# rpng/open_vins

Measured on NVIDIA H100. Metric: msckf_updates_per_sec, higher is better.
Workload: dtype f64

## Files before the change

### open_vins_b200/csrc/chol_tiles.cuh

```cuda
#pragma once
#include "chol.cuh"
#ifdef CQ_PROBE
#include <cstdio>
#endif

#define CT_XP 12

__device__ __forceinline__ void ct_dmma(double &d0, double &d1, double a, double b) {
  asm volatile("mma.sync.aligned.m8n8k4.row.col.f64.f64.f64.f64 {%0,%1}, {%2}, {%3}, {%0,%1};" : "+d"(d0), "+d"(d1) : "d"(a), "d"(b));
}
__device__ __forceinline__ int ct_tri(int b) { return (b * (b + 1)) >> 1; }
__device__ __forceinline__ void ct_bar_group(int id, int nthreads) { asm volatile("bar.sync %0, %1;" ::"r"(id), "r"(nthreads) : "memory"); }
__device__ __forceinline__ size_t ct_idx(int i, int j) { return (size_t)(ct_tri(i >> 3) + (j >> 3)) * 64 + (i & 7) * 8 + (j & 7); }

struct CtView {
  double *T, *Xp0, *Xp1, *invd, *Linv0, *Linv1, *dummyT, *dummyX;
  int *flag;
};
__host__ __device__ inline size_t ct_view_doubles(int NRB) {
  return (size_t)((NRB * (NRB + 1)) / 2) * 64 + 2 * (size_t)NRB * 8 * CT_XP + (size_t)NRB * 8 + 128 + 64 + 2 * CT_XP;
}
__device__ __forceinline__ CtView ct_view_carve(double *base, int NRB, int *flag_word) {
  CtView v;
  v.T = base;
  v.Xp0 = v.T + (size_t)((NRB * (NRB + 1)) / 2) * 64;
  v.Xp1 = v.Xp0 + (size_t)NRB * 8 * CT_XP;
  v.invd = v.Xp1 + (size_t)NRB * 8 * CT_XP;
  v.Linv0 = v.invd + (size_t)NRB * 8;
  v.Linv1 = v.Linv0 + 64;
  v.dummyT = v.Linv1 + 64;
  v.dummyX = v.dummyT + 64;
  v.flag = flag_word;
  return v;
}

__device__ __forceinline__ void ct_diag8_frag(double &d0, double &d1, int nbk, double *invd, bool strict, double floor_d, int *flag) {
  const unsigned full = 0xffffffffu;
  const int lane = threadIdx.x & 31, g = lane >> 2, q = lane & 3;
  bool bad = false;
  double myinv = 0.0;
  const double inv_floor = (floor_d > 0.0) ? fast_rsqrt(floor_d) : 0.0;
  double pj = __shfl_sync(full, d0, 0);
#pragma unroll
  for (int j = 0; j < 8; j++) {
    const int jq = j >> 1;
    const double cur = (j & 1) ? d1 : d0;
    const double ag = __shfl_sync(full, cur, 4 * g + jq);
    const double ac0 = __shfl_sync(full, cur, 8 * q + jq);
    const double ac1 = __shfl_sync(full, cur, 8 * q + 4 + jq);
    double an = 0.0, dn = 0.0;
    if (j < 7) {
      an = __shfl_sync(full, cur, 4 * (j + 1) + jq);
      dn = __shfl_sync(full, ((j + 1) & 1) ? d1 : d0, 4 * (j + 1) + ((j + 1) >> 1));
    }
    const double y = fast_rsqrt(pj);
    const bool in = j < nbk;
    double d, iv;
    if (strict) {
      const bool pos = pj > 0.0;
      bad = bad || (in && !pos);
      d = pj;
      iv = (in && pos) ? y : 0.0;
    } else {
      const bool above = pj > floor_d;
      d = above ? pj : floor_d;
      iv = in ? (above ? y : inv_floor) : 0.0;
    }
    if (j < 7) {
      const double ln = an * iv;
      pj = fma(-ln, ln, dn);
    }
    if (lane == j)
      myinv = iv;
    if (q == jq) {
      if (j & 1)
        d1 = (g == j) ? d * iv : d1 * iv;
      else
        d0 = (g == j) ? d * iv : d0 * iv;
    }
    const double lg = ag * iv, lc0 = ac0 * iv, lc1 = ac1 * iv;
    if (2 * q > j)
      d0 = fma(-lg, lc0, d0);
    if (2 * q + 1 > j)
      d1 = fma(-lg, lc1, d1);
  }
  if (lane < 8)
    invd[lane] = myinv;
  if (bad && lane == 0)
    *flag = 1;
}

__device__ __forceinline__ void ct_linv8(const double *Lt, const double *invd, double *Linv) {
  const int lane = threadIdx.x & 31, cc = lane & 7;
  double mc[8];
#pragma unroll
  for (int j = 0; j < 8; j++) {
    double s0 = (j == cc) ? 1.0 : 0.0, s1 = 0.0;
#pragma unroll
    for (int t = 0; t < j; t++) {
      if (t & 1)
        s1 = fma(-Lt[j * 8 + t], mc[t], s1);
      else
        s0 = fma(-Lt[j * 8 + t], mc[t], s0);
    }
    mc[j] = (s0 + s1) * invd[j];
  }
  if (lane < 8) {
#pragma unroll
    for (int i = 0; i < 8; i++)
      Linv[i * 8 + cc] = (i >= cc) ? mc[i] : 0.0;
  }
}

__device__ __forceinline__ void ct_panel_tile(const CtView &sm, int i, int k, const double *Linv, double *Xb) {
  const int lane = threadIdx.x & 31, g = lane >> 2, q = lane & 3;
  double *t = sm.T + (size_t)(ct_tri(i) + k) * 64;
  const double a0 = t[g * 8 + q], a1 = t[g * 8 + q + 4];
  const double b0 = Linv[g * 8 + q], b1 = Linv[g * 8 + q + 4];
  double2 d = make_double2(0.0, 0.0);
  ct_dmma(d.x, d.y, a0, b0);
  ct_dmma(d.x, d.y, a1, b1);
  *reinterpret_cast<double2 *>(t + 2 * lane) = d;
  *reinterpret_cast<double2 *>(Xb + (size_t)(8 * i + g) * CT_XP + 2 * q) = d;
}

__device__ __forceinline__ void ct_panel_rows(double *T, double *Xp, const double *invd, int i0, int stride, int nrows, int k, int nbk) {
  if (i0 >= nrows)
    return;
  const double *Lk = T + (size_t)(ct_tri(k) + k) * 64;
  double L[8][8], iv[8];
#pragma unroll
  for (int c = 0; c < 8; c++) {
    iv[c] = (c < nbk) ? invd[8 * k + c] : 0.0;
#pragma unroll
    for (int t2 = 0; t2 < 4; t2++) {
      if (2 * t2 < c) {
        const double2 v = *reinterpret_cast<const double2 *>(Lk + c * 8 + 2 * t2);
        L[c][2 * t2] = v.x;
        L[c][2 * t2 + 1] = v.y;
      }
    }
  }
  for (int i = i0; i < nrows; i += stride) {
    double *src = T + (size_t)(ct_tri(i >> 3) + k) * 64 + (i & 7) * 8;
    double v[8], x[8];
    {
      const double2 v01 = *reinterpret_cast<const double2 *>(src), v23 = *reinterpret_cast<const double2 *>(src + 2);
      const double2 v45 = *reinterpret_cast<const double2 *>(src + 4), v67 = *reinterpret_cast<const double2 *>(src + 6);
      v[0] = v01.x, v[1] = v01.y, v[2] = v23.x, v[3] = v23.y, v[4] = v45.x, v[5] = v45.y, v[6] = v67.x, v[7] = v67.y;
    }
#pragma unroll
    for (int c = 0; c < 8; c++) {
      x[c] = (c < nbk) ? v[c] * iv[c] : 0.0;
#pragma unroll
      for (int t = c + 1; t < 8; t++)
        v[t] = fma(-x[c], L[t][c], v[t]);
    }
    if (nbk == 8) {
      *reinterpret_cast<double2 *>(src) = make_double2(x[0], x[1]);
      *reinterpret_cast<double2 *>(src + 2) = make_double2(x[2], x[3]);
      *reinterpret_cast<double2 *>(src + 4) = make_double2(x[4], x[5]);
      *reinterpret_cast<double2 *>(src + 6) = make_double2(x[6], x[7]);
    } else {
#pragma unroll
      for (int c = 0; c < 8; c++)
        if (c < nbk)
          src[c] = x[c];
    }
    double *xp = Xp + (size_t)i * CT_XP;
    *reinterpret_cast<double2 *>(xp) = make_double2(x[0], x[1]);
    *reinterpret_cast<double2 *>(xp + 2) = make_double2(x[2], x[3]);
    *reinterpret_cast<double2 *>(xp + 4) = make_double2(x[4], x[5]);
    *reinterpret_cast<double2 *>(xp + 6) = make_double2(x[6], x[7]);
  }
}

struct CtTileOps {
  double a0, a1, b0, b1;
  double2 c;
  double2 *cp;
};
__device__ __forceinline__ void ct_tile_load(CtTileOps &o, const CtView &sm, const double *Xp, int bi, int bj, int lane, bool valid) {
  const int g = lane >> 2, q = lane & 3;
  const double *xa = valid ? Xp + (size_t)(8 * bi + g) * CT_XP + q : sm.dummyX + q;
  const double *xb = valid ? Xp + (size_t)(8 * bj + g) * CT_XP + q : sm.dummyX + q;
  o.cp = reinterpret_cast<double2 *>((valid ? sm.T + (size_t)(ct_tri(bi) + bj) * 64 : sm.dummyT) + 2 * lane);
  o.a0 = -xa[0];
  o.a1 = -xa[4];
  o.b0 = xb[0];
  o.b1 = xb[4];
  o.c = *o.cp;
}
__device__ __forceinline__ void ct_tile_mma(CtTileOps &o) {
  ct_dmma(o.c.x, o.c.y, o.a0, o.b0);
  ct_dmma(o.c.x, o.c.y, o.a1, o.b1);
}
__device__ __forceinline__ void ct_tile_mma_store(CtTileOps &o) {
  ct_tile_mma(o);
  *o.cp = o.c;
}

#ifdef CQ_PROBE
#define CT_PROBE_T(v) v = clock64()
#else
#define CT_PROBE_T(v) do { } while (0)
#endif

__device__ __forceinline__ void ct_trail_row(const CtView &sm, const double *Xk, int bi, int j0, int jmax, int lane) {
  const int g = lane >> 2, q = lane & 3;
  const double *xa = Xk + (size_t)(8 * bi + g) * CT_XP + q;
  const double a0 = -xa[0], a1 = -xa[4];
  double *trow = sm.T + (size_t)ct_tri(bi) * 64 + 2 * lane;
  for (int bj = j0; bj <= jmax; bj += 2) {
    const bool two = bj + 1 <= jmax;
    const double *xb0 = Xk + (size_t)(8 * bj + g) * CT_XP + q;
    const double *xb1 = two ? xb0 + 8 * CT_XP : sm.dummyX + q;
    double2 *c0p = reinterpret_cast<double2 *>(trow + (size_t)bj * 64);
    double2 *c1p = two ? c0p + 32 : reinterpret_cast<double2 *>(sm.dummyT + 2 * lane);
    const double b00 = xb0[0], b01 = xb0[4], b10 = xb1[0], b11 = xb1[4];
    double2 c0 = *c0p, c1 = *c1p;
    ct_dmma(c0.x, c0.y, a0, b00);
    ct_dmma(c1.x, c1.y, a0, b10);
    ct_dmma(c0.x, c0.y, a1, b01);
    ct_dmma(c1.x, c1.y, a1, b11);
    *c0p = c0;
    *c1p = c1;
  }
}

template <int THREADS>
__device__ __forceinline__ void ct_chol_tiles(const CtView &sm, int n, int nrows, bool strict, double floor_d) {
  const int tid = threadIdx.x, lane = tid & 31, wid = tid >> 5;
  constexpr int NW = THREADS / 32, NH = NW - (NW + 3) / 4;
  static_assert(NH >= 1, "need at least one helper warp");
  const bool helper = (wid & 3) != 0;
  const int hr = wid - 1 - (wid >> 2);
  constexpr bool LINV = NW >= 8;
#ifdef CQ_PROBE
  long long p0 = 0, p1 = 0, p2 = 0, p3 = 0, p4 = 0, p5 = 0, acc[6] = {0, 0, 0, 0, 0, 0};
#endif
  const int NB = (n + 7) >> 3, NRB = (nrows + 7) >> 3;
  if (wid == 0) {
    double2 c = *reinterpret_cast<const double2 *>(sm.T + 2 * lane);
    ct_diag8_frag(c.x, c.y, min(8, n), sm.invd, strict, floor_d, sm.flag);
    *reinterpret_cast<double2 *>(sm.T + 2 * lane) = c;
    __syncwarp();
    if (LINV)
      asm volatile("bar.arrive 3, 64;" ::: "memory");
    ct_panel_rows(sm.T, sm.Xp0, sm.invd, lane < 8 ? 8 + lane : nrows, 1 << 30, nrows, 0, min(8, n));
  } else if (LINV && wid == 4) {
    asm volatile("bar.sync 3, 64;" ::: "memory");
    ct_linv8(sm.T, sm.invd, sm.Linv0);
  }
  __syncthreads();
  for (int k = 0; k < NB; k++) {
    const int par = k & 1;
    double *Xk = par ? sm.Xp1 : sm.Xp0, *Xn = par ? sm.Xp0 : sm.Xp1;
    const bool more = k + 1 < NB;
    CT_PROBE_T(p0);
#ifdef CQ_PROBE
    p1 = p2 = p3 = p4 = p0;
#endif
    if (wid == 0) {
      if (more) {
        const int k1 = k + 1, nbk1 = min(8, n - 8 * k1);
        CtTileOps o;
        ct_tile_load(o, sm, Xk, k1, k1, lane, true);
        ct_tile_mma(o);
        CT_PROBE_T(p1);
        ct_diag8_frag(o.c.x, o.c.y, nbk1, sm.invd + 8 * k1, strict, floor_d, sm.flag);
        *o.cp = o.c;
        __syncwarp();
        if (LINV)
          asm volatile("bar.arrive 3, 64;" ::: "memory");
        CT_PROBE_T(p2);
        asm volatile("bar.sync 2, %0;" ::"r"((NH + 1) * 32) : "memory");
        CT_PROBE_T(p3);
        ct_panel_rows(sm.T, Xn, sm.invd, lane < 8 ? 8 * (k + 2) + lane : nrows, 1 << 30, nrows, k1, nbk1);
        CT_PROBE_T(p4);
      }
    } else if (LINV && wid == 4) {
      if (more) {
        asm volatile("bar.sync 3, 64;" ::: "memory");
        ct_linv8(sm.T + (size_t)(ct_tri(k + 1) + k + 1) * 64, sm.invd + 8 * (k + 1), par ? sm.Linv0 : sm.Linv1);
      }
    } else if (helper) {
      if (LINV) {
        const double *Lk = par ? sm.Linv1 : sm.Linv0;
        for (int i = k + 2 + hr; i < NRB; i += NH)
          ct_panel_tile(sm, i, k, Lk, Xk);
      } else {
        ct_panel_rows(sm.T, Xk, sm.invd, 8 * (k + 2) + hr * 32 + lane, NH * 32, nrows, k, min(8, n - 8 * k));
      }
      if (NH > 1)
        ct_bar_group(1, NH * 32);
      else
        __syncwarp();
      CT_PROBE_T(p1);
      if (more) {
        for (int i = k + 2 + hr; i < NRB; i += 2 * NH) {
          CtTileOps o0, o1;
          ct_tile_load(o0, sm, Xk, i, k + 1, lane, true);
          ct_tile_load(o1, sm, Xk, i + NH, k + 1, lane, i + NH < NRB);
          ct_tile_mma_store(o0);
          ct_tile_mma_store(o1);
        }
        asm volatile("bar.arrive 2, %0;" ::"r"((NH + 1) * 32) : "memory");
        CT_PROBE_T(p2);
        const int R = NRB - (k + 2), jmaxc = NB - 1;
        for (int pr = hr; 2 * pr < R; pr += NH) {
          const int rb = R - 1 - pr;
          ct_trail_row(sm, Xk, k + 2 + rb, k + 2, min(k + 2 + rb, jmaxc), lane);
          if (rb != pr)
            ct_trail_row(sm, Xk, k + 2 + pr, k + 2, min(k + 2 + pr, jmaxc), lane);
        }
      }
      CT_PROBE_T(p3);
    }
    __syncthreads();
    CT_PROBE_T(p5);
#ifdef CQ_PROBE
    if (wid == 0) {
      acc[0] += p1 - p0, acc[1] += p2 - p1, acc[2] += p3 - p2, acc[3] += p4 - p3, acc[4] += p5 - p4;
    } else {
      acc[0] += p1 - p0, acc[1] += p2 - p1, acc[2] += p3 - p2, acc[3] += p5 - p3;
    }
    acc[5] += p5 - p0;
#endif
  }
#ifdef CQ_PROBE
  if (tid == 0)
    printf("chol n=%d W0 (cycles over %d steps): diag update %lld pivots %lld wait %lld rows below %lld step tail %lld | %lld\n", n, NB, acc[0], acc[1], acc[2], acc[3],
           acc[4], acc[5]);
  if (tid == 32 || tid == THREADS - 32)
    printf("chol n=%d helper warp %d: panel rows %lld column k+1 %lld trailing %lld wait %lld | %lld\n", n, wid, acc[0], acc[1], acc[2], acc[3], acc[5]);
#endif
}
```

### open_vins_b200/csrc/k_cholqr.cu

```cuda
#include "chol.cuh"
#include "chol_tiles.cuh"
#include "ovb_internal.cuh"
#include <math.h>
#include <cstdio>

#define CQ_MAXN 160
#define CQ_MAXB 20
#define CQ_MAXRB 22
#define CQ_GRAM_T 512
#define CQ_KB 32
#ifndef CQ_CHOL_T
#define CQ_CHOL_T 384
#endif
#define CQ_XP CT_XP
#define CQ_TRSM_T 640

namespace {

__device__ __forceinline__ void dmma(double &d0, double &d1, double a, double b) {
  asm volatile("mma.sync.aligned.m8n8k4.row.col.f64.f64.f64.f64 {%0,%1}, {%2}, {%3}, {%0,%1};" : "+d"(d0), "+d"(d1) : "d"(a), "d"(b));
}
__device__ __forceinline__ unsigned s_u32(const void *p) { return (unsigned)__cvta_generic_to_shared(p); }
__device__ __forceinline__ void cpa16(unsigned dst, const void *src, unsigned bytes) {
  asm volatile("cp.async.cg.shared.global [%0], [%1], 16, %2;" ::"r"(dst), "l"(src), "r"(bytes) : "memory");
}
__device__ __forceinline__ void cpa8(unsigned dst, const void *src, unsigned bytes) {
  asm volatile("cp.async.ca.shared.global [%0], [%1], 8, %2;" ::"r"(dst), "l"(src), "r"(bytes) : "memory");
}
__device__ __forceinline__ void cpa_commit() { asm volatile("cp.async.commit_group;" ::: "memory"); }
template <int N> __device__ __forceinline__ void cpa_wait() { asm volatile("cp.async.wait_group %0;" ::"n"(N) : "memory"); }
__device__ __forceinline__ void bar_group(int id, int nthreads) { asm volatile("bar.sync %0, %1;" ::"r"(id), "r"(nthreads) : "memory"); }
__device__ __forceinline__ int tri(int b) { return (b * (b + 1)) >> 1; }

__device__ __forceinline__ bool cq_tile_origin(int blk, int w, int BW, int nblk_side, int &ci, int &cj, int &offI, int &offJ, bool &diag) {
  int bI = 0, t = blk;
  while (t >= nblk_side - bI) {
    t -= nblk_side - bI;
    bI++;
  }
  const int bJ = bI + t;
  diag = (bI == bJ);
  int a, b;
  if (diag) {
    a = 0;
    int u = w;
    while (a < BW && u >= BW - a) {
      u -= BW - a;
      a++;
    }
    if (a >= BW)
      return false;
    b = a + u;
  } else {
    if (w >= BW * BW)
      return false;
    a = w / BW;
    b = w % BW;
  }
  offI = a * 32;
  offJ = (diag ? 0 : BW * 32) + b * 32;
  ci = (bI * BW + a) * 32;
  cj = (bJ * BW + b) * 32;
  return true;
}

template <int NT>
__device__ __forceinline__ void cq_issue_rows(double *buf, int pitch, const double *__restrict__ A, int ldA, int rc, int nrows, int r1, int nt, int cI0, int cJ0,
                                              int WI, int nrng) {
  const int units_per_row = nrng * WI / 2;
  for (int e = threadIdx.x; e < nrows * units_per_row; e += NT) {
    const int k = e / units_per_row, u = e - k * units_per_row;
    const int r = rc + k;
    const int dcol = 2 * u, col = (dcol < WI) ? cI0 + dcol : cJ0 + (dcol - WI);
    unsigned bytes = 0;
    if (r < r1)
      bytes = (col + 1 < nt) ? 16u : (col < nt ? 8u : 0u);
    const double *src = bytes ? (A + (size_t)r * ldA + col) : A;
    cpa16(s_u32(buf + (size_t)k * pitch + dcol), src, bytes);
  }
  cpa_commit();
}

__device__ __forceinline__ void cq_gram_kstep(double (&acc)[4][4][2], const double *row0, int pitch, int offI, int offJ, bool same, int g, int q) {
  const double *row = row0 + (size_t)q * pitch + g;
  double fa[4], fb[4];
#pragma unroll
  for (int b = 0; b < 4; b++)
    fa[b] = row[offI + 8 * b];
  if (same) {
#pragma unroll
    for (int b = 0; b < 4; b++)
      fb[b] = fa[b];
  } else {
#pragma unroll
    for (int b = 0; b < 4; b++)
      fb[b] = row[offJ + 8 * b];
  }
#pragma unroll
  for (int a = 0; a < 4; a++)
#pragma unroll
    for (int b = 0; b < 4; b++)
      dmma(acc[a][b][0], acc[a][b][1], fa[a], fb[b]);
}

}

__global__ void __launch_bounds__(CQ_GRAM_T) k_cq_gram(const double *__restrict__ A, int ldA, int m, int nt, int slab_rows, int BW, int nblk_side,
                                                      double *__restrict__ Gpart, int cs) {
  OVB_PDL_ENTER();
  extern __shared__ __align__(16) double gsm[];
  const int tid = threadIdx.x, lane = tid & 31, wid = tid >> 5, g = lane >> 2, q = lane & 3;
  int ci, cj, offI, offJ;
  bool diag;
  const bool active = cq_tile_origin(blockIdx.x, wid, BW, nblk_side, ci, cj, offI, offJ, diag);
  int bI = 0, tt = blockIdx.x;
  while (tt >= nblk_side - bI) {
    tt -= nblk_side - bI;
    bI++;
  }
  const int bJ = bI + tt;
  const int WI = BW * 32;
  const int nrng = (bI == bJ) ? 1 : 2;
  const int pitch = nrng * WI + 4;
  const int cI0 = bI * WI, cJ0 = bJ * WI;
  const int r0 = blockIdx.y * slab_rows, r1 = min(m, r0 + slab_rows);
  const int nchunks = (r1 > r0) ? (r1 - r0 + CQ_KB - 1) / CQ_KB : 0;
  double acc[4][4][2];
#pragma unroll
  for (int a = 0; a < 4; a++)
#pragma unroll
    for (int b = 0; b < 4; b++)
      acc[a][b][0] = acc[a][b][1] = 0.0;

  auto issue = [&](int c) { cq_issue_rows<CQ_GRAM_T>(gsm + (size_t)(c & 1) * CQ_KB * pitch, pitch, A, ldA, r0 + c * CQ_KB, CQ_KB, r1, nt, cI0, cJ0, WI, nrng); };
  if (nchunks > 0)
    issue(0);
  for (int c = 0; c < nchunks; c++) {
    if (c + 1 < nchunks) {
      issue(c + 1);
      cpa_wait<1>();
    } else {
      cpa_wait<0>();
    }
    __syncthreads();
    if (active) {
      const double *buf = gsm + (size_t)(c & 1) * CQ_KB * pitch;
#pragma unroll
      for (int ks = 0; ks < CQ_KB / 4; ks++)
        cq_gram_kstep(acc, buf + (size_t)4 * ks * pitch, pitch, offI, offJ, diag && offI == offJ, g, q);
    }
    __syncthreads();
  }
  if (cs <= 1) {
    if (active) {
      double *dst = Gpart + (((size_t)blockIdx.y * gridDim.x + blockIdx.x) * 16 + wid) * 1024;
#pragma unroll
      for (int a = 0; a < 4; a++)
#pragma unroll
        for (int b = 0; b < 4; b++)
          *reinterpret_cast<double2 *>(dst + (8 * a + g) * 32 + 8 * b + 2 * q) = make_double2(acc[a][b][0], acc[a][b][1]);
    }
    return;
  }
  double *stage = gsm;
  if (active) {
    double *dst = stage + (size_t)wid * 1024;
#pragma unroll
    for (int a = 0; a < 4; a++)
#pragma unroll
      for (int b = 0; b < 4; b++)
        *reinterpret_cast<double2 *>(dst + (8 * a + g) * 32 + 8 * b + 2 * q) = make_double2(acc[a][b][0], acc[a][b][1]);
  }
  asm volatile("barrier.cluster.arrive.release.aligned;" ::: "memory");
  asm volatile("barrier.cluster.wait.acquire.aligned;" ::: "memory");
  unsigned rank;
  asm volatile("mov.u32 %0, %%cluster_ctarank;" : "=r"(rank));
  if (active) {
    const int per = 1024 / cs;
    double *dst = Gpart + ((((size_t)blockIdx.y / cs) * gridDim.x + blockIdx.x) * 16 + wid) * 1024 + (size_t)rank * per;
    const unsigned base = s_u32(stage + (size_t)wid * 1024 + (size_t)rank * per);
    for (int e = lane; e < per; e += 32) {
      double sum = 0.0;
      for (int r = 0; r < cs; r++) {
        unsigned ra;
        double v;
        asm volatile("mapa.shared::cluster.u32 %0, %1, %2;" : "=r"(ra) : "r"(base + 8u * (unsigned)e), "r"((unsigned)r));
        asm volatile("ld.shared::cluster.f64 %0, [%1];" : "=d"(v) : "r"(ra) : "memory");
        sum += v;
      }
      dst[e] = sum;
    }
  }
  asm volatile("barrier.cluster.arrive.release.aligned;" ::: "memory");
  asm volatile("barrier.cluster.wait.acquire.aligned;" ::: "memory");
}

#define CQ_RED_T 1024
#define CQ_RED_CH 8
#define CQ_RED_GX (16 * CQ_RED_CH)
__global__ void __launch_bounds__(CQ_RED_T) k_cq_reduce(const double *__restrict__ Gpart, int nslab, int nblk, int BW, int nblk_side, int nt,
                                                       double *__restrict__ G, int ldG, int tiled) {
  OVB_PDL_ENTER();
  __shared__ double red[8][128];
  int ci, cj, offI, offJ;
  bool diag;
  const int w = blockIdx.x / CQ_RED_CH, ch = blockIdx.x % CQ_RED_CH, blk = blockIdx.y;
  if (!cq_tile_origin(blk, w, BW, nblk_side, ci, cj, offI, offJ, diag))
    return;
  if (ci >= nt || cj >= nt)
    return;
  const int el = threadIdx.x & 127, sg = threadIdx.x >> 7;
  const int e = ch * 128 + el;
  const double *src = Gpart + ((size_t)blk * 16 + w) * 1024 + e;
  const size_t stride = (size_t)nblk * 16 * 1024;
  double s0 = 0.0, s1 = 0.0;
  int sl = sg;
  for (; sl + 8 < nslab; sl += 16) {
    s0 += src[(size_t)sl * stride];
    s1 += src[(size_t)(sl + 8) * stride];
  }
  if (sl < nslab)
    s0 += src[(size_t)sl * stride];
  red[sg][el] = s0 + s1;
  __syncthreads();
  if (sg == 0) {
    const int i = ci + (e >> 5), j = cj + (e & 31);
    if (i < nt && j < nt && i <= j) {
      const double s = ((red[0][el] + red[1][el]) + (red[2][el] + red[3][el])) + ((red[4][el] + red[5][el]) + (red[6][el] + red[7][el]));
      if (tiled) {
        G[ct_idx(j, i)] = s;
        if ((i >> 3) == (j >> 3))
          G[(size_t)(tri(j >> 3) + (j >> 3)) * 64 + (i & 7) * 8 + (j & 7)] = s;
      } else {
        G[(size_t)i * ldG + j] = s;
        G[(size_t)j * ldG + i] = s;
      }
    }
  }
}

struct CqCholSmem {
  double T[(CQ_MAXRB * (CQ_MAXRB + 1) / 2) * 64];
  double Xp[2][CQ_MAXRB * 8 * CQ_XP];
  double invd[CQ_MAXRB * 8];
  double Linv[2][64];
  double red[32];
  double dummyT[64];
  double dummyX[2 * CQ_XP];
  int flag;
};

#define CQ_PK_INV ((CQ_MAXB * (CQ_MAXB + 1) / 2) * 64)
#define CQ_PK_DOUBLES (CQ_PK_INV + CQ_MAXB * 8)

namespace {

__device__ __forceinline__ void cq_chol_tiles(CqCholSmem &sm, int n, int nrows, bool strict, double floor_d) {
  CtView v;
  v.T = sm.T;
  v.Xp0 = sm.Xp[0];
  v.Xp1 = sm.Xp[1];
  v.invd = sm.invd;
  v.Linv0 = sm.Linv[0];
  v.Linv1 = sm.Linv[1];
  v.dummyT = sm.dummyT;
  v.dummyX = sm.dummyX;
  v.flag = &sm.flag;
  ct_chol_tiles<CQ_CHOL_T>(v, n, nrows, strict, floor_d);
}

__device__ void cq_load_tiles(CqCholSmem &sm, const double *__restrict__ G, size_t ldG, int n, int nrows, const double *__restrict__ rhs, int ld_rhs) {
  const int tid = threadIdx.x, lane = tid & 31, wid = tid >> 5;
  const int NB = (n + 7) >> 3, NRB = (nrows + 7) >> 3;
  for (int i = wid; i < 8 * NRB; i += CQ_CHOL_T / 32) {
    const double *row = (i >= n && rhs != nullptr) ? rhs + (size_t)(i - n) * ld_rhs : G + (size_t)i * ldG;
    const int jmax = min(i | 7, 8 * NB - 1);
    double *dst = sm.T + (size_t)tri(i >> 3) * 64 + (i & 7) * 8;
    for (int j = 2 * lane; j <= jmax; j += 64) {
      unsigned bytes = 0;
      if (i < nrows)
        bytes = (j + 1 < n) ? 16u : (j < n ? 8u : 0u);
      cpa16(s_u32(dst + (size_t)(j >> 3) * 64 + (j & 7)), bytes ? (const void *)(row + j) : (const void *)G, bytes);
    }
  }
  cpa_commit();
  for (int e = tid; e < 2 * CQ_MAXRB * 8 * CQ_XP; e += CQ_CHOL_T)
    (&sm.Xp[0][0])[e] = 0.0;
  if (tid < 64)
    sm.dummyT[tid] = 0.0;
  if (tid < 2 * CQ_XP)
    sm.dummyX[tid] = 0.0;
  if (tid == 0)
    sm.flag = 0;
  cpa_wait<0>();
}

__device__ __forceinline__ double cq_el(const double *T, int i, int j) { return T[(size_t)(tri(i >> 3) + (j >> 3)) * 64 + (i & 7) * 8 + (j & 7)]; }

}

__global__ void __launch_bounds__(CQ_CHOL_T) k_cq_chol_gram(const double *__restrict__ G, int ldG, int n, double shift_rel, double *__restrict__ Lpk, int tiled) {
  OVB_PDL_ENTER();
  extern __shared__ __align__(16) unsigned char cq_raw[];
  CqCholSmem &sm = *reinterpret_cast<CqCholSmem *>(cq_raw);
  const int tid = threadIdx.x, lane = tid & 31, wid = tid >> 5;
#ifdef CQ_PROBE
  const long long q0 = clock64();
#endif
  if (tiled) {
    __shared__ __align__(8) unsigned long long g_bar;
    const unsigned bar = s_u32(&g_bar);
    const int NB = (n + 7) >> 3;
    if (tid == 0) {
      asm volatile("mbarrier.init.shared::cta.b64 [%0], 1;" ::"r"(bar) : "memory");
      asm volatile("fence.mbarrier_init.release.cluster;" ::: "memory");
    }
    __syncthreads();
    if (tid == 0) {
      const unsigned bytes = (unsigned)(tri(NB) * 64 * sizeof(double));
      asm volatile("mbarrier.arrive.expect_tx.shared::cta.b64 _, [%0], %1;" ::"r"(bar), "r"(bytes) : "memory");
      asm volatile("cp.async.bulk.shared::cluster.global.mbarrier::complete_tx::bytes [%0], [%1], %2, [%3];" ::"r"(s_u32(sm.T)), "l"(G), "r"(bytes), "r"(bar)
                   : "memory");
    }
    for (int e = tid; e < 2 * CQ_MAXRB * 8 * CQ_XP; e += CQ_CHOL_T)
      (&sm.Xp[0][0])[e] = 0.0;
    if (tid < 64)
      sm.dummyT[tid] = 0.0;
    if (tid < 2 * CQ_XP)
      sm.dummyX[tid] = 0.0;
    if (tid == 0)
      sm.flag = 0;
    asm volatile("{\n\t.reg .pred p;\n\tCQ_GWAIT:\n\tmbarrier.try_wait.parity.shared::cta.b64 p, [%0], 0;\n\t@p bra CQ_GDONE;\n\tbra CQ_GWAIT;\n\tCQ_GDONE:\n\t}" ::"r"(bar)
                 : "memory");
    const int r0 = n - 8 * (NB - 1);
    if (r0 < 8) {
      double *last = sm.T + (size_t)tri(NB - 1) * 64;
      for (int e = tid; e < NB * 64; e += CQ_CHOL_T)
        if (((e >> 3) & 7) >= r0)
          last[e] = 0.0;
    }
  } else {
    cq_load_tiles(sm, G, (size_t)ldG, n, n, nullptr, 0);
  }
  __syncthreads();
  double mx = 0.0;
  for (int i = tid; i < n; i += CQ_CHOL_T) {
    const double d = sm.T[(size_t)(tri(i >> 3) + (i >> 3)) * 64 + (i & 7) * 9];
    mx = (d > mx) ? d : mx;
  }
#pragma unroll
  for (int o = 16; o > 0; o >>= 1) {
    const double y = __shfl_xor_sync(0xffffffffu, mx, o);
    mx = (y > mx) ? y : mx;
  }
  if (lane == 0)
    sm.red[wid] = mx;
  __syncthreads();
  mx = 0.0;
  for (int w = 0; w < CQ_CHOL_T / 32; w++)
    mx = (sm.red[w] > mx) ? sm.red[w] : mx;
  const double shift = shift_rel * mx;
  for (int i = tid; i < n; i += CQ_CHOL_T)
    sm.T[(size_t)(tri(i >> 3) + (i >> 3)) * 64 + (i & 7) * 9] += shift;
  __syncthreads();
#ifdef CQ_PROBE
  const long long q1 = clock64();
#endif
  cq_chol_tiles(sm, n, n, false, 0.25 * shift);
#ifdef CQ_PROBE
  const long long q2 = clock64();
#endif
  const int NB = (n + 7) >> 3;
  for (int e = 2 * tid; e < tri(NB) * 64; e += 2 * CQ_CHOL_T)
    *reinterpret_cast<double2 *>(Lpk + e) = *reinterpret_cast<const double2 *>(sm.T + e);
  for (int e = tid; e < CQ_MAXB * 8; e += CQ_CHOL_T)
    Lpk[CQ_PK_INV + e] = (e < n) ? sm.invd[e] : 1.0;
#ifdef CQ_PROBE
  if (tid == 0)
    printf("chol_gram n=%d: load %lld factor %lld store %lld cycles\n", n, q1 - q0, q2 - q1, clock64() - q2);
#endif
}

__global__ void __launch_bounds__(CQ_CHOL_T) k_cq_chol_ekf(double *__restrict__ S, int ldS, int r, const double *__restrict__ res, double *__restrict__ w,
                                                          double *__restrict__ invdiag, DevUpdateInfo *__restrict__ info, double *__restrict__ Lpk,
                                                          const double *__restrict__ floor_dev) {
  OVB_PDL_ENTER();
  extern __shared__ __align__(16) unsigned char cq_raw[];
  CqCholSmem &sm = *reinterpret_cast<CqCholSmem *>(cq_raw);
  const int tid = threadIdx.x, lane = tid & 31, wid = tid >> 5;
  const int nrows = r + (res != nullptr ? 1 : 0);
  cq_load_tiles(sm, S, (size_t)ldS, r, nrows, res, 0);
  __syncthreads();
  if (floor_dev != nullptr)
    cq_chol_tiles(sm, r, nrows, false, *floor_dev);
  else
    cq_chol_tiles(sm, r, nrows, true, 0.0);
  for (int i = wid; i < r; i += CQ_CHOL_T / 32)
    for (int j = lane; j <= i; j += 32)
      S[(size_t)i * ldS + j] = cq_el(sm.T, i, j);
  if (res != nullptr)
    for (int j = tid; j < r; j += CQ_CHOL_T)
      w[j] = cq_el(sm.T, r, j);
  if (invdiag != nullptr)
    for (int j = tid; j < r; j += CQ_CHOL_T)
      invdiag[j] = sm.invd[j];
  if (Lpk != nullptr) {
    const int NB = (r + 7) >> 3;
    for (int e = 2 * tid; e < tri(NB) * 64; e += 2 * CQ_CHOL_T)
      *reinterpret_cast<double2 *>(Lpk + e) = *reinterpret_cast<const double2 *>(sm.T + e);
    for (int e = tid; e < CQ_MAXB * 8; e += CQ_CHOL_T)
      Lpk[CQ_PK_INV + e] = (e < r) ? sm.invd[e] : 1.0;
  }
  if (tid == 0 && sm.flag && info != nullptr)
    info->not_spd = 1;
}

#define CQ_TRSM_NH 10
#define CQ_TRSM_SMEM (sizeof(double) * ((size_t)CQ_PK_DOUBLES + (size_t)(CQ_TRSM_T / 32) * CQ_TRSM_NH * 2 * 32))
template <int NH>
__device__ __forceinline__ void cq_trsm_half(double (&acc)[NH][2], int b0, const double *Lt, const double *Ri, double *xs, int lane) {
  const int g = lane >> 2, q = lane & 3;
#pragma unroll
  for (int jb = 0; jb < NH; jb++) {
    const int B = b0 + jb;
    const double *Ld = Lt + (size_t)(tri(B) + B) * 64;
    const double *ri = Ri + B * 8;
    double x[8];
#pragma unroll
    for (int qq = 0; qq < 4; qq++) {
      x[2 * qq] = __shfl_sync(0xffffffffu, acc[jb][0], (lane & ~3) | qq);
      x[2 * qq + 1] = __shfl_sync(0xffffffffu, acc[jb][1], (lane & ~3) | qq);
    }
#pragma unroll
    for (int c = 0; c < 8; c++) {
      x[c] *= ri[c];
#pragma unroll
      for (int c2 = c + 1; c2 < 8; c2++)
        x[c2] -= x[c] * Ld[c2 * 8 + c];
    }
    acc[jb][0] = (q == 0) ? x[0] : (q == 1) ? x[2] : (q == 2) ? x[4] : x[6];
    acc[jb][1] = (q == 0) ? x[1] : (q == 1) ? x[3] : (q == 2) ? x[5] : x[7];
    const double af0 = -((q == 0) ? x[0] : (q == 1) ? x[1] : (q == 2) ? x[2] : x[3]);
    const double af1 = -((q == 0) ? x[4] : (q == 1) ? x[5] : (q == 2) ? x[6] : x[7]);
    if (xs != nullptr) {
      xs[(2 * jb) * 32 + lane] = af0;
      xs[(2 * jb + 1) * 32 + lane] = af1;
    }
#pragma unroll
    for (int j = jb + 1; j < NH; j++) {
      const double *lf = Lt + (size_t)(tri(b0 + j) + B) * 64 + g * 8 + q;
      dmma(acc[j][0], acc[j][1], af0, lf[0]);
      dmma(acc[j][0], acc[j][1], af1, lf[4]);
    }
  }
}

template <int NH>
__device__ __forceinline__ void cq_trsm_load(double (&acc)[NH][2], const double *arow, bool row_ok, int b0, int nt, int q) {
#pragma unroll
  for (int jb = 0; jb < NH; jb++) {
    const int col = 8 * (b0 + jb) + 2 * q;
    acc[jb][0] = acc[jb][1] = 0.0;
    if (row_ok) {
      if (col + 1 < nt) {
        const double2 v = *reinterpret_cast<const double2 *>(arow + col);
        acc[jb][0] = v.x;
        acc[jb][1] = v.y;
      } else if (col < nt) {
        acc[jb][0] = arow[col];
      }
    }
  }
}
template <int NH>
__device__ __forceinline__ void cq_trsm_store(const double (&acc)[NH][2], double *arow, bool row_ok, int b0, int nt, int q) {
  if (!row_ok)
    return;
#pragma unroll
  for (int jb = 0; jb < NH; jb++) {
    const int col = 8 * (b0 + jb) + 2 * q;
    if (col + 1 < nt)
      *reinterpret_cast<double2 *>(arow + col) = make_double2(acc[jb][0], acc[jb][1]);
    else if (col < nt)
      arow[col] = acc[jb][0];
  }
}

template <int NBP, int NT>
__device__ __forceinline__ void cq_fetch_factor(double *Lt, double *Ri, const double *__restrict__ Lpk, int NB) {
  const int tid = threadIdx.x;
  __shared__ __align__(8) unsigned long long l_bar;
  const unsigned bar = s_u32(&l_bar);
  if (tid == 0) {
    asm volatile("mbarrier.init.shared::cta.b64 [%0], 1;" ::"r"(bar) : "memory");
    asm volatile("fence.mbarrier_init.release.cluster;" ::: "memory");
  }
  __syncthreads();
  if (tid == 0) {
    const unsigned bytesL = (unsigned)(tri(NB) * 64 * sizeof(double)), bytesR = (unsigned)(NB * 8 * sizeof(double));
    asm volatile("mbarrier.arrive.expect_tx.shared::cta.b64 _, [%0], %1;" ::"r"(bar), "r"(bytesL + bytesR) : "memory");
    asm volatile("cp.async.bulk.shared::cluster.global.mbarrier::complete_tx::bytes [%0], [%1], %2, [%3];" ::"r"(s_u32(Lt)), "l"(Lpk), "r"(bytesL), "r"(bar)
                 : "memory");
    asm volatile("cp.async.bulk.shared::cluster.global.mbarrier::complete_tx::bytes [%0], [%1], %2, [%3];" ::"r"(s_u32(Ri)), "l"(Lpk + CQ_PK_INV), "r"(bytesR),
                 "r"(bar)
                 : "memory");
  }
  for (int e = tri(NB) * 64 + tid; e < tri(NBP) * 64; e += NT)
    Lt[e] = 0.0;
  for (int e = NB * 8 + tid; e < NBP * 8; e += NT)
    Ri[e] = 1.0;
  asm volatile("{\n\t.reg .pred p;\n\tCQ_LWAIT:\n\tmbarrier.try_wait.parity.shared::cta.b64 p, [%0], 0;\n\t@p bra CQ_LDONE;\n\tbra CQ_LWAIT;\n\tCQ_LDONE:\n\t}" ::"r"(bar)
               : "memory");
  __syncthreads();
}

template <int NH1, int NH2>
__global__ void __launch_bounds__(CQ_TRSM_T) k_cq_trsm(double *__restrict__ A, int ldA, int m, int nt, const double *__restrict__ Lpk) {
  OVB_PDL_ENTER();
  extern __shared__ __align__(16) double tsm[];
  double *Lt = tsm;
  double *Ri = tsm + CQ_PK_INV;
  double *Xs = tsm + CQ_PK_DOUBLES;
  const int tid = threadIdx.x, lane = tid & 31, wid = tid >> 5, g = lane >> 2, q = lane & 3;
  cq_fetch_factor<NH1 + NH2, CQ_TRSM_T>(Lt, Ri, Lpk, (nt + 7) >> 3);
  double *xs = Xs + (size_t)wid * (CQ_TRSM_NH * 2 * 32);
  const int ngroups = (m + 7) >> 3;
  for (int rg = blockIdx.x + gridDim.x * wid; rg < ngroups; rg += gridDim.x * (CQ_TRSM_T / 32)) {
    const int row = 8 * rg + g;
    const bool row_ok = row < m;
    double *arow = A + (size_t)row * ldA;
#ifdef CQ_PROBE
    long long t0 = clock64(), t1, t2, t3 = 0, t4 = 0;
#endif
    {
      double acc[NH1][2];
      cq_trsm_load<NH1>(acc, arow, row_ok, 0, nt, q);
#ifdef CQ_PROBE
      t1 = clock64();
#endif
      cq_trsm_half<NH1>(acc, 0, Lt, Ri, NH2 > 0 ? xs : nullptr, lane);
#ifdef CQ_PROBE
      t2 = clock64();
#endif
      cq_trsm_store<NH1>(acc, arow, row_ok, 0, nt, q);
    }
    if constexpr (NH2 > 0) {
      double acc[NH2][2];
      cq_trsm_load<NH2>(acc, arow, row_ok, NH1, nt, q);
      __syncwarp();
#pragma unroll 2
      for (int jb = 0; jb < NH1; jb++) {
        const double af0 = xs[(2 * jb) * 32 + lane], af1 = xs[(2 * jb + 1) * 32 + lane];
#pragma unroll
        for (int j = 0; j < NH2; j++) {
          const double *lf = Lt + (size_t)(tri(NH1 + j) + jb) * 64 + g * 8 + q;
          dmma(acc[j][0], acc[j][1], af0, lf[0]);
          dmma(acc[j][0], acc[j][1], af1, lf[4]);
        }
      }
#ifdef CQ_PROBE
      t3 = clock64();
#endif
      cq_trsm_half<NH2>(acc, NH1, Lt, Ri, nullptr, lane);
#ifdef CQ_PROBE
      t4 = clock64();
#endif
      cq_trsm_store<NH2>(acc, arow, row_ok, NH1, nt, q);
      __syncwarp();
    }
#ifdef CQ_PROBE
    if (blockIdx.x == 0 && (tid == 0 || tid == 32 * 7) && rg < 40)
      printf("trsm rg=%d tid=%d: load %lld half1 %lld gemm+load %lld half2 %lld total %lld\n", rg, tid, t1 - t0, t2 - t1, t3 - t2, t4 - t3, clock64() - t0);
#endif
  }
}

static void cq_launch_trsm(ovb_ctx *ctx, int ctas, double *A, int ldA, int m, int nt, const double *Lpk) {
  const int NB = (nt + 7) / 8;
  const size_t smem = CQ_TRSM_SMEM;
  if (NB <= 5)
    ovb_launch(ctx, k_cq_trsm<5, 0>, dim3(ctas), dim3(CQ_TRSM_T), smem, A, ldA, m, nt, Lpk);
  else if (NB <= 10)
    ovb_launch(ctx, k_cq_trsm<10, 0>, dim3(ctas), dim3(CQ_TRSM_T), smem, A, ldA, m, nt, Lpk);
  else if (NB <= 15)
    ovb_launch(ctx, k_cq_trsm<10, 5>, dim3(ctas), dim3(CQ_TRSM_T), smem, A, ldA, m, nt, Lpk);
  else
    ovb_launch(ctx, k_cq_trsm<10, 10>, dim3(ctas), dim3(CQ_TRSM_T), smem, A, ldA, m, nt, Lpk);
}

#define CQ_SG_SMEM (226 * 1024)

__host__ __device__ __forceinline__ int cq_sg_pitch(int BW, int NBP) {
  const int w = (8 * NBP > 32 * BW) ? 8 * NBP : 32 * BW;
  return ((w + 15) & ~15) + 4;
}

template <int NH1, int NH2>
__device__ __forceinline__ void cq_solve_group(double *xrow, bool row_ok, const double *Lt, const double *Ri, int lane) {
  constexpr int NBP = NH1 + NH2;
  const int g = lane >> 2, q = lane & 3;
  {
    double acc[NH1][2];
    cq_trsm_load<NH1>(acc, xrow, row_ok, 0, 8 * NBP, q);
    cq_trsm_half<NH1>(acc, 0, Lt, Ri, nullptr, lane);
    cq_trsm_store<NH1>(acc, xrow, row_ok, 0, 8 * NBP, q);
  }
  if constexpr (NH2 > 0) {
    double acc[NH2][2];
    __syncwarp();
    cq_trsm_load<NH2>(acc, xrow, row_ok, NH1, 8 * NBP, q);
#pragma unroll 2
    for (int jb = 0; jb < NH1; jb++) {
      const double af0 = -xrow[8 * jb + q], af1 = -xrow[8 * jb + 4 + q];
#pragma unroll
      for (int j = 0; j < NH2; j++) {
        const double *lf = Lt + (size_t)(tri(NH1 + j) + jb) * 64 + g * 8 + q;
        dmma(acc[j][0], acc[j][1], af0, lf[0]);
        dmma(acc[j][0], acc[j][1], af1, lf[4]);
      }
    }
    cq_trsm_half<NH2>(acc, NH1, Lt, Ri, nullptr, lane);
    cq_trsm_store<NH2>(acc, xrow, row_ok, NH1, 8 * NBP, q);
  }
}

template <int NH1, int NH2>
__global__ void __launch_bounds__(CQ_GRAM_T) k_cq_solve_gram(const double *__restrict__ A, int ldA, int m, int nt, const double *__restrict__ Lpk, int slab_rows,
                                                            int cb, int ntail_max, int BW, double *__restrict__ Gpart, double *__restrict__ Qtail) {
  OVB_PDL_ENTER();
  extern __shared__ __align__(16) double ssm[];
  double *Lt = ssm;
  double *Ri = ssm + CQ_PK_INV;
  double *X = ssm + CQ_PK_DOUBLES;
  constexpr int NBP = NH1 + NH2;
  const int pitch = cq_sg_pitch(BW, NBP);
  const int r0 = blockIdx.x * slab_rows, r1 = min(m, r0 + slab_rows);
  double *tail = Qtail + (size_t)blockIdx.x * ntail_max * pitch;
  auto split_at = [&](int rc) { return r1 - rc > cb && r1 - rc <= 8 * (CQ_GRAM_T / 32); };
  auto nbuf_at = [&](int rc) { return split_at(rc) ? cb & ~7 : min(cb, (r1 - rc + 3) & ~3); };
  if (r0 < r1)
    cq_issue_rows<CQ_GRAM_T>(X, pitch, A, ldA, r0, nbuf_at(r0), r1, nt, 0, 0, pitch - 4, 1);
  cq_fetch_factor<NBP, CQ_GRAM_T>(Lt, Ri, Lpk, (nt + 7) >> 3);
  for (int rc = r0, nbuf = nbuf_at(r0), ntail = 0; rc < r1; rc += nbuf + ntail, nbuf = nbuf_at(rc)) {
    ntail = split_at(rc) ? (r1 - rc - nbuf + 3) & ~3 : 0;
    const int nact = nbuf + ntail;
    if (rc > r0)
      cq_issue_rows<CQ_GRAM_T>(X, pitch, A, ldA, rc, nbuf, r1, nt, 0, 0, pitch - 4, 1);
    for (int e = threadIdx.x; e < ntail * (pitch - 4); e += CQ_GRAM_T) {
      const int k = e / (pitch - 4), col = e - k * (pitch - 4), r = rc + nbuf + k;
      tail[(size_t)k * pitch + col] = (r < r1 && col < nt) ? A[(size_t)r * ldA + col] : 0.0;
    }
    cpa_wait<0>();
    __syncthreads();
    const int lane = threadIdx.x & 31, wid = threadIdx.x >> 5, g = lane >> 2, q = lane & 3, lr = 8 * wid + g;
    if (8 * wid < nbuf)
      cq_solve_group<NH1, NH2>(X + (size_t)min(lr, nbuf - 1) * pitch, lr < nbuf, Lt, Ri, lane);
    else if (8 * wid < nact)
      cq_solve_group<NH1, NH2>(tail + (size_t)min(lr - nbuf, ntail - 1) * pitch, lr < nact, Lt, Ri, lane);
    __syncthreads();
    int ci, cj, offI, offJ;
    bool diag;
    const bool active = cq_tile_origin(0, wid, BW, 1, ci, cj, offI, offJ, diag);
    double *part = Gpart + ((size_t)blockIdx.x * 16 + wid) * 1024 + g * 32 + 2 * q;
    if (active) {
      double acc[4][4][2];
#pragma unroll
      for (int a = 0; a < 4; a++)
#pragma unroll
        for (int b = 0; b < 4; b++) {
          const double2 v = rc > r0 ? *reinterpret_cast<const double2 *>(part + a * 256 + 8 * b) : make_double2(0.0, 0.0);
          acc[a][b][0] = v.x;
          acc[a][b][1] = v.y;
        }
#pragma unroll 1
      for (int k = 0; k < nact; k += 4)
        cq_gram_kstep(acc, k < nbuf ? X + (size_t)k * pitch : tail + (size_t)(k - nbuf) * pitch, pitch, offI, offJ, offI == offJ, g, q);
#pragma unroll
      for (int a = 0; a < 4; a++)
#pragma unroll
        for (int b = 0; b < 4; b++)
          *reinterpret_cast<double2 *>(part + a * 256 + 8 * b) = make_double2(acc[a][b][0], acc[a][b][1]);
    }
    __syncthreads();
  }
}

struct CqSgShape {
  int pitch, cb, ntail;
};
static CqSgShape cq_sg_shape(int nt, int BW, int slab_rows) {
  const int NB = (nt + 7) / 8, NBP = NB <= 5 ? 5 : NB <= 10 ? 10 : NB <= 15 ? 15 : 20;
  CqSgShape s;
  s.pitch = cq_sg_pitch(BW, NBP);
  const int round = slab_rows < 8 * (CQ_GRAM_T / 32) ? slab_rows : 8 * (CQ_GRAM_T / 32);
  const int fit = (int)((CQ_SG_SMEM - sizeof(double) * CQ_PK_DOUBLES) / (sizeof(double) * s.pitch)) & ~3;
  s.cb = fit < round ? fit : round;
  s.ntail = slab_rows > s.cb ? round - (s.cb & ~7) : 0;
  return s;
}
static size_t cq_solve_gram_scratch(int nslab, int nt, int BW, int slab_rows) {
  const CqSgShape s = cq_sg_shape(nt, BW, slab_rows);
  return (size_t)nslab * s.ntail * s.pitch;
}

template <int NH1, int NH2>
static void cq_launch_solve_gram_t(ovb_ctx *ctx, int nslab, const double *A, int ldA, int m, int nt, const double *Lpk, int slab_rows, int BW, double *Gpart,
                                   double *Qtail) {
  const CqSgShape s = cq_sg_shape(nt, BW, slab_rows);
  const size_t smem = sizeof(double) * (CQ_PK_DOUBLES + (size_t)s.cb * s.pitch);
  ovb_launch(ctx, k_cq_solve_gram<NH1, NH2>, dim3(nslab), dim3(CQ_GRAM_T), smem, A, ldA, m, nt, Lpk, slab_rows, s.cb, s.ntail, BW, Gpart, Qtail);
}
static void cq_launch_solve_gram(ovb_ctx *ctx, int nslab, const double *A, int ldA, int m, int nt, const double *Lpk, int slab_rows, int BW, double *Gpart,
                                 double *Qtail) {
  const int NB = (nt + 7) / 8;
  if (NB <= 5)
    cq_launch_solve_gram_t<5, 0>(ctx, nslab, A, ldA, m, nt, Lpk, slab_rows, BW, Gpart, Qtail);
  else if (NB <= 10)
    cq_launch_solve_gram_t<10, 0>(ctx, nslab, A, ldA, m, nt, Lpk, slab_rows, BW, Gpart, Qtail);
  else if (NB <= 15)
    cq_launch_solve_gram_t<10, 5>(ctx, nslab, A, ldA, m, nt, Lpk, slab_rows, BW, Gpart, Qtail);
  else
    cq_launch_solve_gram_t<10, 10>(ctx, nslab, A, ldA, m, nt, Lpk, slab_rows, BW, Gpart, Qtail);
}

__global__ void __launch_bounds__(256) k_cq_trmm(const double *__restrict__ L2, const double *__restrict__ L1, int nt, double *__restrict__ Rout, int ldR) {
  OVB_PDL_ENTER();
  __shared__ double As[16][CQ_MAXN + 1];
  __shared__ double Bs[CQ_MAXN][17];
  const int ti = blockIdx.y, tj = blockIdx.x;
  const int tid = threadIdx.x, tx = tid & 15, ty = tid >> 4;
  const int n = nt - 1;
  const int i = ti * 16 + ty, j = tj * 16 + tx;
  double acc = 0.0;
  if (tj >= ti) {
    const int k0 = ti * 16, k1 = min(nt, tj * 16 + 16);
    const int K = k1 - k0;
    for (int e = tid; e < 16 * K; e += 256) {
      const int a = e / K, k = e - a * K;
      const int ii = ti * 16 + a, kk = k0 + k;
      As[a][k] = (ii < nt && kk >= ii) ? L2[(size_t)(tri(kk >> 3) + (ii >> 3)) * 64 + (kk & 7) * 8 + (ii & 7)] : 0.0;
    }
    for (int e = tid; e < 16 * K; e += 256) {
      const int k = e >> 4, b = e & 15;
      const int kk = k0 + k, jj = tj * 16 + b;
      Bs[k][b] = (jj < nt && jj >= kk) ? L1[(size_t)(tri(jj >> 3) + (kk >> 3)) * 64 + (jj & 7) * 8 + (kk & 7)] : 0.0;
    }
    __syncthreads();
    double a0 = 0.0, a1 = 0.0, a2 = 0.0, a3 = 0.0;
    int k = 0;
    for (; k + 3 < K; k += 4) {
      a0 += As[ty][k] * Bs[k][tx];
      a1 += As[ty][k + 1] * Bs[k + 1][tx];
      a2 += As[ty][k + 2] * Bs[k + 2][tx];
      a3 += As[ty][k + 3] * Bs[k + 3][tx];
    }
    for (; k < K; k++)
      a0 += As[ty][k] * Bs[k][tx];
    acc = (a0 + a1) + (a2 + a3);
  }
  if (i < n && j < nt)
    Rout[(size_t)i * ldR + j] = (j >= i) ? acc : 0.0;
}

#define CQ_GN_T 256
__global__ void __launch_bounds__(CQ_GN_T) k_cq_gemm_nt(double *__restrict__ C, int ldc, const double *__restrict__ A, int lda, const double *__restrict__ B,
                                                       int ldb, int M, int N, int K, int lower_only) {
  OVB_PDL_ENTER();
  __shared__ __align__(16) double As[64][36];
  __shared__ __align__(16) double Bs[64][36];
  const int m0 = blockIdx.y * 64, n0 = blockIdx.x * 64;
  if (lower_only && n0 > m0 + 63)
    return;
  const int tid = threadIdx.x, lane = tid & 31, wid = tid >> 5, g = lane >> 2, q = lane & 3;
  const int wm = (wid >> 2) * 32, wn = (wid & 3) * 16;
  double acc[4][2][2];
#pragma unroll
  for (int a = 0; a < 4; a++)
#pragma unroll
    for (int b = 0; b < 2; b++)
      acc[a][b][0] = acc[a][b][1] = 0.0;
  for (int k0 = 0; k0 < K; k0 += 32) {
    for (int e = tid; e < 64 * 16; e += CQ_GN_T) {
      const int r = e >> 4, u = e & 15, k = k0 + 2 * u;
      unsigned ba = 0, bb = 0;
      if (m0 + r < M)
        ba = (k + 1 < K) ? 16u : (k < K ? 8u : 0u);
      if (n0 + r < N)
        bb = (k + 1 < K) ? 16u : (k < K ? 8u : 0u);
      cpa16(s_u32(&As[r][2 * u]), ba ? (const void *)(A + (size_t)(m0 + r) * lda + k) : (const void *)A, ba);
      cpa16(s_u32(&Bs[r][2 * u]), bb ? (const void *)(B + (size_t)(n0 + r) * ldb + k) : (const void *)B, bb);
    }
    cpa_commit();
    cpa_wait<0>();
    __syncthreads();
#pragma unroll
    for (int ks = 0; ks < 8; ks++) {
      double fa[4], fb[2];
#pragma unroll
      for (int a = 0; a < 4; a++)
        fa[a] = As[wm + 8 * a + g][4 * ks + q];
#pragma unroll
      for (int b = 0; b < 2; b++)
        fb[b] = Bs[wn + 8 * b + g][4 * ks + q];
#pragma unroll
      for (int a = 0; a < 4; a++)
#pragma unroll
        for (int b = 0; b < 2; b++)
          dmma(acc[a][b][0], acc[a][b][1], fa[a], fb[b]);
    }
    __syncthreads();
  }
#pragma unroll
  for (int a = 0; a < 4; a++)
#pragma unroll
    for (int b = 0; b < 2; b++) {
      const int i = m0 + wm + 8 * a + g, j = n0 + wn + 8 * b + 2 * q;
      if (i < M) {
        double *c = C + (size_t)i * ldc + j;
        if (j + 1 < N) {
          double2 v = *reinterpret_cast<double2 *>(c);
          v.x -= acc[a][b][0];
          v.y -= acc[a][b][1];
          *reinterpret_cast<double2 *>(c) = v;
        } else if (j < N) {
          c[0] -= acc[a][b][0];
        }
      }
    }
}

__global__ void __launch_bounds__(256) k_cq_shift(double *__restrict__ G, int ldG, int n, double shift_rel, double *__restrict__ floor_out) {
  OVB_PDL_ENTER();
  __shared__ double red[8];
  double mx = 0.0;
  for (int i = threadIdx.x; i < n; i += 256) {
    const double d = G[(size_t)i * ldG + i];
    mx = (d > mx) ? d : mx;
  }
#pragma unroll
  for (int o = 16; o > 0; o >>= 1) {
    const double y = __shfl_xor_sync(0xffffffffu, mx, o);
    mx = (y > mx) ? y : mx;
  }
  if ((threadIdx.x & 31) == 0)
    red[threadIdx.x >> 5] = mx;
  __syncthreads();
  mx = 0.0;
  for (int w = 0; w < 8; w++)
    mx = (red[w] > mx) ? red[w] : mx;
  const double shift = shift_rel * mx;
  for (int i = threadIdx.x; i < n; i += 256)
    G[(size_t)i * ldG + i] += shift;
  if (threadIdx.x == 0)
    *floor_out = 0.25 * shift;
}

__global__ void __launch_bounds__(256) k_cq_trmm_wide(const double *__restrict__ L2, const double *__restrict__ L1, int ldL, int nt, double *__restrict__ Rout,
                                                     int ldR) {
  OVB_PDL_ENTER();
  __shared__ double As[32][33];
  __shared__ double Bs[32][33];
  const int ti = blockIdx.y, tj = blockIdx.x;
  const int tid = threadIdx.x, tx = tid & 31, ty = tid >> 5;
  const int n = nt - 1;
  double acc[4] = {0, 0, 0, 0};
  if (tj >= ti) {
    for (int tk = ti; tk <= tj; tk++) {
      for (int e = tid; e < 1024; e += 256) {
        const int a = e >> 5, b = e & 31;
        const int k = tk * 32 + a, i = ti * 32 + b;
        As[a][b] = (k < nt && i < nt && k >= i) ? L2[(size_t)k * ldL + i] : 0.0;
        const int j = tj * 32 + a, k2 = tk * 32 + b;
        Bs[a][b] = (j < nt && k2 < nt && j >= k2) ? L1[(size_t)j * ldL + k2] : 0.0;
      }
      __syncthreads();
#pragma unroll 8
      for (int kk = 0; kk < 32; kk++) {
        const double b = Bs[tx][kk];
#pragma unroll
        for (int u = 0; u < 4; u++)
          acc[u] += As[kk][ty + 8 * u] * b;
      }
      __syncthreads();
    }
  }
#pragma unroll
  for (int u = 0; u < 4; u++) {
    const int i = ti * 32 + ty + 8 * u, j = tj * 32 + tx;
    if (i < n && j < nt)
      Rout[(size_t)i * ldR + j] = (j >= i) ? acc[u] : 0.0;
  }
}

#define CQ_GRAM_CS 4
static void cq_launch_gram(ovb_ctx *ctx, int nblk, int nslab_padded, size_t smem, const double *A, int ldA, int m, int nt, int slab_rows, int BW, int nblk_side,
                           double *Gpart, int cs) {
  cudaLaunchConfig_t cfg = {};
  cfg.gridDim = dim3(nblk, nslab_padded);
  cfg.blockDim = dim3(CQ_GRAM_T);
  cfg.dynamicSmemBytes = smem;
  cfg.stream = ctx->stream;
  cudaLaunchAttribute at[2];
  int na = 0;
  if (ctx->tsqr_pdl && !ctx->prof_on) {
    at[na].id = cudaLaunchAttributeProgrammaticStreamSerialization;
    at[na].val.programmaticStreamSerializationAllowed = 1;
    na++;
  }
  if (cs > 1) {
    at[na].id = cudaLaunchAttributeClusterDimension;
    at[na].val.clusterDim.x = 1;
    at[na].val.clusterDim.y = cs;
    at[na].val.clusterDim.z = 1;
    na++;
  }
  cfg.attrs = at;
  cfg.numAttrs = na;
  const bool prof = ctx->prof_on && ctx->prof_n < 96 && ctx->prof_ev[0] != nullptr;
  if (prof)
    cudaEventRecord(ctx->prof_ev[2 * ctx->prof_n], ctx->stream);
  cudaLaunchKernelEx(&cfg, k_cq_gram, A, ldA, m, nt, slab_rows, BW, nblk_side, Gpart, cs);
  if (prof) {
    cudaEventRecord(ctx->prof_ev[2 * ctx->prof_n + 1], ctx->stream);
    ctx->prof_fn[ctx->prof_n++] = (const void *)k_cq_gram;
  }
}

static bool cq_attrs(ovb_ctx *ctx) {
  if (!ctx->attr_done[4]) {
    cudaFuncSetAttribute(k_cq_gram, cudaFuncAttributeMaxDynamicSharedMemorySize, 160 * 1024);
    cudaFuncSetAttribute(k_cq_chol_gram, cudaFuncAttributeMaxDynamicSharedMemorySize, (int)sizeof(CqCholSmem));
    cudaFuncSetAttribute(k_cq_chol_ekf, cudaFuncAttributeMaxDynamicSharedMemorySize, (int)sizeof(CqCholSmem));
    cudaFuncSetAttribute(k_cq_trsm<5, 0>, cudaFuncAttributeMaxDynamicSharedMemorySize, (int)CQ_TRSM_SMEM);
    cudaFuncSetAttribute(k_cq_trsm<10, 0>, cudaFuncAttributeMaxDynamicSharedMemorySize, (int)CQ_TRSM_SMEM);
    cudaFuncSetAttribute(k_cq_trsm<10, 5>, cudaFuncAttributeMaxDynamicSharedMemorySize, (int)CQ_TRSM_SMEM);
    cudaFuncSetAttribute(k_cq_trsm<10, 10>, cudaFuncAttributeMaxDynamicSharedMemorySize, (int)CQ_TRSM_SMEM);
    cudaFuncSetAttribute(k_cq_solve_gram<5, 0>, cudaFuncAttributeMaxDynamicSharedMemorySize, CQ_SG_SMEM);
    cudaFuncSetAttribute(k_cq_solve_gram<10, 0>, cudaFuncAttributeMaxDynamicSharedMemorySize, CQ_SG_SMEM);
    cudaFuncSetAttribute(k_cq_solve_gram<10, 5>, cudaFuncAttributeMaxDynamicSharedMemorySize, CQ_SG_SMEM);
    cudaFuncSetAttribute(k_cq_solve_gram<10, 10>, cudaFuncAttributeMaxDynamicSharedMemorySize, CQ_SG_SMEM);
    ctx->attr_done[4] = 1;
  }
  return true;
}

int ovb_cholqr_max_cols(void) { return CQ_MAXN; }

static bool cq_ensure_G(ovb_ctx *ctx) {
  const int ldW = CQ_MAXN + 8;
  const size_t need_G = (size_t)4 * ldW * ldW;
  if (need_G > ctx->G_cap) {
    if (ctx->d_G)
      cudaFree(ctx->d_G);
    ctx->d_G = nullptr;
    if (cudaMalloc(&ctx->d_G, sizeof(double) * need_G) != cudaSuccess)
      return false;
    cudaMemsetAsync(ctx->d_G, 0, sizeof(double) * need_G, ctx->stream);
    ctx->G_cap = need_G;
  }
  return true;
}

bool launch_chol_ekf_dmma(ovb_ctx *ctx, double *S, int ldS, int r, const double *res, double *w, double *invdiag, double **Lpk_out) {
  if (Lpk_out)
    *Lpk_out = nullptr;
  if (r + 1 > CQ_MAXRB * 8 || r > CQ_MAXN || (ldS & 1))
    return false;
  cq_attrs(ctx);
  double *Lpk = nullptr;
  if (cq_ensure_G(ctx)) {
    const int ldW = CQ_MAXN + 8;
    Lpk = ctx->d_G + (size_t)3 * ldW * ldW;
  }
  ovb_launch(ctx, k_cq_chol_ekf, dim3(1), dim3(CQ_CHOL_T), sizeof(CqCholSmem), S, ldS, r, res, w, invdiag, ctx->d_info, Lpk, (const double *)nullptr);
  if (Lpk_out)
    *Lpk_out = Lpk;
  return true;
}

bool launch_trsm_rows(ovb_ctx *ctx, double *A, int ldA, int m, int nt, const double *Lpk) {
  if (nt > CQ_MAXN || (ldA & 1) || m < 1 || Lpk == nullptr)
    return false;
  cq_attrs(ctx);
  const int ngroups = (m + 7) / 8;
  int ctas = ngroups;
  if (ctas > ctx->sm_count)
    ctas = ctx->sm_count;
  cq_launch_trsm(ctx, ctas, A, ldA, m, nt, Lpk);
  return true;
}

#define CQ_WB 128
#define CQ_WMAX 520
#define CQ_WBLOCKS ((CQ_WMAX + CQ_WB - 1) / CQ_WB)
static bool cq_ensure_wide(ovb_ctx *ctx) {
  const size_t need = (size_t)2 * CQ_WMAX * CQ_WMAX + (size_t)2 * CQ_WBLOCKS * CQ_PK_DOUBLES + 64;
  if (need > ctx->cqw_cap) {
    if (ctx->d_cqw)
      cudaFree(ctx->d_cqw);
    ctx->d_cqw = nullptr;
    if (cudaMalloc(&ctx->d_cqw, sizeof(double) * need) != cudaSuccess)
      return false;
    ctx->cqw_cap = need;
  }
  return true;
}
static void cq_gemm_nt(ovb_ctx *ctx, double *C, int ldc, const double *A, int lda, const double *B, int ldb, int M, int N, int K, int lower_only) {
  if (M <= 0 || N <= 0 || K <= 0)
    return;
  ovb_launch(ctx, k_cq_gemm_nt, dim3((N + 63) / 64, (M + 63) / 64), dim3(CQ_GN_T), (size_t)0, C, ldc, A, lda, B, ldb, M, N, K, lower_only);
}
static void cq_trsm_any(ovb_ctx *ctx, double *A, int ldA, int m, int nt, const double *Lpk) {
  const int ngroups = (m + 7) / 8;
  int ctas = (ngroups + CQ_TRSM_T / 32 - 1) / (CQ_TRSM_T / 32);
  if (ngroups <= ctx->sm_count)
    ctas = ngroups;
  if (ctas > ctx->sm_count)
    ctas = ctx->sm_count;
  cq_launch_trsm(ctx, ctas, A, ldA, m, nt, Lpk);
}
static void cq_chol_blocked(ovb_ctx *ctx, double *S, int ld, int n, int extra, double *Lpk, const double *floor_dev, DevUpdateInfo *info) {
  for (int J = 0, b = 0; J < n; J += CQ_WB, b++) {
    const int nb = (n - J < CQ_WB) ? n - J : CQ_WB;
    double *Lb = Lpk + (size_t)b * CQ_PK_DOUBLES;
    ovb_launch(ctx, k_cq_chol_ekf, dim3(1), dim3(CQ_CHOL_T), sizeof(CqCholSmem), S + (size_t)J * ld + J, ld, nb, (const double *)nullptr, (double *)nullptr,
               (double *)nullptr, info, Lb, floor_dev);
    const int mrem = n + extra - (J + nb);
    if (mrem > 0) {
      double *panel = S + (size_t)(J + nb) * ld + J;
      cq_trsm_any(ctx, panel, ld, mrem, nb, Lb);
      const int ncols = n - (J + nb);
      cq_gemm_nt(ctx, S + (size_t)(J + nb) * ld + (J + nb), ld, panel, ld, panel, ld, mrem, ncols, nb, 1);
    }
  }
}
static void cq_trsm_blocked(ovb_ctx *ctx, double *X, int ldx, int m, int n, const double *S, int ld, const double *Lpk) {
  for (int J = 0, b = 0; J < n; J += CQ_WB, b++) {
    const int nb = (n - J < CQ_WB) ? n - J : CQ_WB;
    if (J > 0)
      cq_gemm_nt(ctx, X + J, ldx, X, ldx, S + (size_t)J * ld, ld, m, nb, J, 0);
    cq_trsm_any(ctx, X + J, ldx, m, nb, Lpk + (size_t)b * CQ_PK_DOUBLES);
  }
}

__global__ void k_cq_copy_row(const double *__restrict__ src, double *__restrict__ dst, int n) {
  OVB_PDL_ENTER();
  const int i = blockIdx.x * blockDim.x + threadIdx.x;
  if (i < n)
    dst[i] = src[i];
}
__global__ void k_cq_inv_diag(const double *__restrict__ S, int ld, int n, double *__restrict__ inv) {
  OVB_PDL_ENTER();
  const int i = blockIdx.x * blockDim.x + threadIdx.x;
  if (i < n) {
    const double d = S[(size_t)i * ld + i];
    inv[i] = d != 0.0 ? 1.0 / d : 0.0;
  }
}

bool launch_chol_solve_wide(ovb_ctx *ctx, double *S, int ldS, int r, double *w, double *invdiag, double *M, int ldM, int N, bool gate_only) {
  if (r > CQ_WMAX - 8 || (ldS & 1) || (ldM & 1) || r + 1 > ctx->cfg.max_state + 1)
    return false;
  cq_attrs(ctx);
  if (!cq_ensure_wide(ctx))
    return false;
  double *Lpk = ctx->d_cqw + (size_t)2 * CQ_WMAX * CQ_WMAX;
  ovb_launch(ctx, k_cq_copy_row, dim3((r + 127) / 128), dim3(128), (size_t)0, (const double *)w, S + (size_t)r * ldS, r);
  cq_chol_blocked(ctx, S, ldS, r, 1, Lpk, nullptr, ctx->d_info);
  ovb_launch(ctx, k_cq_copy_row, dim3((r + 127) / 128), dim3(128), (size_t)0, (const double *)(S + (size_t)r * ldS), w, r);
  ovb_launch(ctx, k_cq_inv_diag, dim3((r + 127) / 128), dim3(128), (size_t)0, (const double *)S, ldS, r, invdiag);
  if (!gate_only)
    cq_trsm_blocked(ctx, M, ldM, N, r, S, ldS, Lpk);
  return true;
}

static int cq_compress_wide(ovb_ctx *ctx, double *A, int m, int n, int ldA, double *Rout, int ldR) {
  const int nt = n + 1;
  if (nt > CQ_WMAX - 7 || !cq_ensure_wide(ctx))
    return -1;
  const int nT = (nt + 31) / 32, BW = 4, nblk_side = (nT + BW - 1) / BW, nblk = nblk_side * (nblk_side + 1) / 2;
  int nslab = ctx->sm_count / nblk;
  if (nslab < 1)
    nslab = 1;
  const int max_slabs = (m + CQ_KB - 1) / CQ_KB;
  if (nslab > max_slabs)
    nslab = max_slabs;
  int slab_rows = (((m + nslab - 1) / nslab) + 3) & ~3;
  nslab = (m + slab_rows - 1) / slab_rows;
  const size_t need_part = (size_t)nslab * nblk * 16 * 1024;
  if (need_part > ctx->Gpart_cap) {
    if (ctx->d_Gpart)
      cudaFree(ctx->d_Gpart);
    ctx->d_Gpart = nullptr;
    if (cudaMalloc(&ctx->d_Gpart, sizeof(double) * need_part) != cudaSuccess)
      return -1;
    ctx->Gpart_cap = need_part;
  }
  double *G1 = ctx->d_cqw, *G2 = G1 + (size_t)CQ_WMAX * CQ_WMAX, *Lpk1 = G2 + (size_t)CQ_WMAX * CQ_WMAX, *Lpk2 = Lpk1 + (size_t)CQ_WBLOCKS * CQ_PK_DOUBLES;
  double *floor_dev = Lpk2 + (size_t)CQ_WBLOCKS * CQ_PK_DOUBLES;
  const size_t gram_smem = sizeof(double) * 2 * CQ_KB * (size_t)(2 * BW * 32 + 4);
  int launches = 0;
  for (int pass = 0; pass < 2; pass++) {
    double *G = pass == 0 ? G1 : G2;
    cq_launch_gram(ctx, nblk, nslab, gram_smem, (const double *)A, ldA, m, nt, slab_rows, BW, nblk_side, ctx->d_Gpart, 1);
    ovb_launch(ctx, k_cq_reduce, dim3(CQ_RED_GX, nblk), dim3(CQ_RED_T), (size_t)0, (const double *)ctx->d_Gpart, nslab, nblk, BW, nblk_side, nt, G, (int)CQ_WMAX, 0);
    ovb_launch(ctx, k_cq_shift, dim3(1), dim3(256), (size_t)0, G, (int)CQ_WMAX, nt, pass == 0 ? 1e-11 : 1e-13, floor_dev + pass);
    cq_chol_blocked(ctx, G, CQ_WMAX, nt, 0, pass == 0 ? Lpk1 : Lpk2, floor_dev + pass, (DevUpdateInfo *)nullptr);
    if (pass == 0)
      cq_trsm_blocked(ctx, A, ldA, m, nt, G1, CQ_WMAX, Lpk1);
    launches += 3 + 3 * ((nt + CQ_WB - 1) / CQ_WB);
  }
  const int nT32 = (nt + 31) / 32;
  ovb_launch(ctx, k_cq_trmm_wide, dim3(nT32, nT32), dim3(256), (size_t)0, (const double *)G2, (const double *)G1, (int)CQ_WMAX, nt, Rout, ldR);
  ctx->n_launch += launches + 1;
  return launches + 1;
}

int launch_compress_cholqr2(ovb_ctx *ctx, double *A, int m, int n, int ldA, double *Rout, int ldR) {
  const int nt = n + 1;
  if ((ldA & 1) || m < 1)
    return -1;
  cq_attrs(ctx);
  if (nt > CQ_MAXN)
    return cq_compress_wide(ctx, A, m, n, ldA, Rout, ldR);
  const int nT = (nt + 31) / 32;
  const int BW = nT, nblk_side = 1, nblk = 1;
  int nslab = ctx->sm_count;
  const int max_slabs = (m + CQ_KB - 1) / CQ_KB;
  if (nslab > max_slabs)
    nslab = max_slabs;
  int slab_rows = (m + nslab - 1) / nslab;
  slab_rows = (slab_rows + 3) & ~3;
  nslab = (m + slab_rows - 1) / slab_rows;
  const int cs = (ctx->gram_cluster && nslab >= 2 * CQ_GRAM_CS) ? CQ_GRAM_CS : 1;
  const int nslab_pad = (nslab + cs - 1) / cs * cs, npart = nslab_pad / cs;
  const size_t part_doubles = (size_t)nslab_pad * nblk * 16 * 1024;
  const size_t need_part = part_doubles + cq_solve_gram_scratch(nslab, nt, BW, slab_rows);
  const int ldW = CQ_MAXN + 8;
  if (!cq_ensure_G(ctx))
    return -1;
  if (need_part > ctx->Gpart_cap) {
    const size_t cap = need_part + need_part / 2;
    if (ctx->d_Gpart)
      cudaFree(ctx->d_Gpart);
    ctx->d_Gpart = nullptr;
    ctx->Gpart_cap = 0;
    if (cudaMalloc(&ctx->d_Gpart, sizeof(double) * cap) != cudaSuccess)
      return -1;
    ctx->Gpart_cap = cap;
  }
  double *G = ctx->d_G, *L1 = G + (size_t)ldW * ldW, *L2 = L1 + (size_t)ldW * ldW;
  static_assert(CQ_PK_DOUBLES <= (CQ_MAXN + 8) * (CQ_MAXN + 8), "packed factor must fit its slot");
  size_t gram_smem = sizeof(double) * 2 * CQ_KB * (size_t)(BW * 32 + 4);
  if (cs > 1 && gram_smem < sizeof(double) * 16 * 1024)
    gram_smem = sizeof(double) * 16 * 1024;
  cq_launch_gram(ctx, nblk, nslab_pad, gram_smem, (const double *)A, ldA, m, nt, slab_rows, BW, nblk_side, ctx->d_Gpart, cs);
  ovb_launch(ctx, k_cq_reduce, dim3(CQ_RED_GX, nblk), dim3(CQ_RED_T), (size_t)0, (const double *)ctx->d_Gpart, npart, nblk, BW, nblk_side, nt, G, ldW, 1);
  ovb_launch(ctx, k_cq_chol_gram, dim3(1), dim3(CQ_CHOL_T), sizeof(CqCholSmem), (const double *)G, ldW, nt, 1e-11, L1, 1);
  cq_launch_solve_gram(ctx, nslab, (const double *)A, ldA, m, nt, (const double *)L1, slab_rows, BW, ctx->d_Gpart, ctx->d_Gpart + part_doubles);
  ovb_launch(ctx, k_cq_reduce, dim3(CQ_RED_GX, nblk), dim3(CQ_RED_T), (size_t)0, (const double *)ctx->d_Gpart, nslab, nblk, BW, nblk_side, nt, G, ldW, 1);
  ovb_launch(ctx, k_cq_chol_gram, dim3(1), dim3(CQ_CHOL_T), sizeof(CqCholSmem), (const double *)G, ldW, nt, 1e-13, L2, 1);
  const int nT16 = (nt + 15) / 16;
  ovb_launch(ctx, k_cq_trmm, dim3(nT16, nT16), dim3(256), (size_t)0, (const double *)L2, (const double *)L1, nt, Rout, ldR);
  ctx->n_launch += 7;
  return 7;
}
```

### open_vins_b200/csrc/k_ekf.cu

```cuda
#include "chol.cuh"
#include "ovb_internal.cuh"

#define EK_T 32

__global__ void __launch_bounds__(256) k_ekf_gemm(int mode, const double *__restrict__ P, int ldP, const double *__restrict__ H, int ldH,
                                                  const double *__restrict__ Min, int ldM, const DevUpdateInfo *__restrict__ info, int X, int Y,
                                                  int K, double *__restrict__ Cout, int ldC, double sigma2, const double *__restrict__ Rdiag) {
  OVB_PDL_ENTER();
  __shared__ double As[EK_T][EK_T + 1];
  __shared__ double Bs[EK_T][EK_T + 1];
  const int x0 = blockIdx.x * EK_T, y0 = blockIdx.y * EK_T;
  if (mode == 1 && y0 > x0 + EK_T - 1)
    return;
  const int tid = threadIdx.x, tx = tid & 31, ty = tid >> 5;
  double acc[4] = {0, 0, 0, 0};
  const int *cs = info->col_state;
  for (int j0 = 0; j0 < K; j0 += EK_T) {
    for (int e = tid; e < EK_T * EK_T; e += 256) {
      int jj = e >> 5, q = e & 31;
      int j = j0 + jj;
      double av = 0.0, bv = 0.0;
      if (j < K) {
        if (mode == 0) {
          int a = x0 + q;
// ... 79 lines not shown
                                                           int L_in_smem, const DevUpdateInfo *__restrict__ info) {
  OVB_PDL_ENTER();
  extern __shared__ __align__(16) double tsm[];
  const int lane = threadIdx.x & 31, wid = threadIdx.x >> 5;
  if (info->not_spd)
    return;
  const int ldl = r | 1;
  double *inv_s = tsm + (size_t)TR_ROWS * r;
  double *Ls = inv_s + r;
  for (int e = threadIdx.x; e < r; e += 32 * TR_ROWS)
    inv_s[e] = invdiag[e];
  if (L_in_smem)
    stage_lower_async<32 * TR_ROWS>(Ls, ldl, L, (size_t)ldL, r, r);
  else
    __syncthreads();
  const double *Lp = L_in_smem ? Ls : L;
  const int lp = L_in_smem ? ldl : ldL;
  const int a = blockIdx.x * TR_ROWS + wid;
  if (a >= N)
    return;
  double *y = tsm + (size_t)wid * r;
  for (int t = lane; t < r; t += 32)
    y[t] = M[(size_t)a * ldM + t];
  __syncwarp();
  for (int kb = 0; kb < r; kb += 8) {
    const int nbk = min(8, r - kb);
    double s[8];
#pragma unroll
    for (int c = 0; c < 8; c++)
      s[c] = 0.0;
    for (int t = lane; t < kb; t += 32) {
      const double yt = y[t];
#pragma unroll
      for (int c = 0; c < 8; c++)
        if (c < nbk)
          s[c] += Lp[(size_t)(kb + c) * lp + t] * yt;
    }
#pragma unroll
    for (int o = 16; o > 0; o >>= 1) {
#pragma unroll
      for (int c = 0; c < 8; c++)
        s[c] += __shfl_xor_sync(0xffffffffu, s[c], o);
    }
    double yn[8];
#pragma unroll
    for (int c = 0; c < 8; c++) {
      if (c < nbk) {
        const double *Lr = Lp + (size_t)(kb + c) * lp + kb;
        double v = y[kb + c] - s[c];
#pragma unroll
        for (int t = 0; t < 8; t++)
          if (t + 1 < c)
            v -= Lr[t] * yn[t];
        if (c > 0)
          v -= Lr[c - 1] * yn[c - 1];
        yn[c] = v * inv_s[kb + c];
      }
    }
    __syncwarp();
    if (lane < nbk) {
      double v = yn[0];
#pragma unroll
      for (int c = 1; c < 8; c++)
        v = (lane == c) ? yn[c] : v;
      y[kb + lane] = v;
    }
    __syncwarp();
  }
  for (int t = lane; t < r; t += 32)
    Yout[(size_t)a * ldY + t] = y[t];
}

__global__ void __launch_bounds__(256) k_ekf_downdate(double *__restrict__ P, int ldP, const double *__restrict__ Yin, int ldY, int N, int r,
                                                      const double *__restrict__ w, double *__restrict__ dx, DevUpdateInfo *__restrict__ info) {
  OVB_PDL_ENTER();
  __shared__ double As[EK_T][EK_T + 1];
  __shared__ double Bs[EK_T][EK_T + 1];
  const int a0 = blockIdx.x * EK_T, b0 = blockIdx.y * EK_T;
  if (b0 < a0)
    return;
  const int tid = threadIdx.x, tx = tid & 31, ty = tid >> 5;
  if (info->not_spd) {
    if (a0 == b0 && tid < EK_T && a0 + tid < N)
      dx[a0 + tid] = 0.0;
    return;
  }
  double acc[4] = {0, 0, 0, 0};
  double dxa = 0.0;
  for (int k0 = 0; k0 < r; k0 += EK_T) {
    for (int e = tid; e < EK_T * EK_T; e += 256) {
      int q = e >> 5, kk = e & 31;
      int k = k0 + kk;
      As[kk][q] = (k < r && a0 + q < N) ? Yin[(size_t)(a0 + q) * ldY + k] : 0.0;
      Bs[kk][q] = (k < r && b0 + q < N) ? Yin[(size_t)(b0 + q) * ldY + k] : 0.0;
    }
    __syncthreads();
#pragma unroll 8
    for (int kk = 0; kk < EK_T; kk++) {
      double b = Bs[kk][tx];
#pragma unroll
      for (int u = 0; u < 4; u++)
        acc[u] += As[kk][ty + 8 * u] * b;
    }
    if (a0 == b0 && tid < EK_T) {
      for (int kk = 0; kk < EK_T; kk++)
        if (k0 + kk < r)
          dxa += As[kk][tid] * w[k0 + kk];
    }
    __syncthreads();
  }
#pragma unroll
  for (int u = 0; u < 4; u++) {
    int a = a0 + ty + 8 * u, b = b0 + tx;
    if (a < N && b < N && b >= a) {
      double v = P[(size_t)a * ldP + b] - acc[u];
      P[(size_t)a * ldP + b] = v;
      P[(size_t)b * ldP + a] = v;
      if (a == b && v < 0.0)
        atomicMin(&info->neg_diag_index, a);
      if (!isfinite(v))
        info->nonfinite = 1;
    }
  }
  if (a0 == b0 && tid < EK_T && a0 + tid < N)
    dx[a0 + tid] = dxa;
}

#define EK1_KMAX 160
__device__ __forceinline__ void ek_cpa8(double *dst_smem, const double *src) {
  asm volatile("cp.async.ca.shared.global [%0], [%1], 8;" ::"r"((unsigned)__cvta_generic_to_shared(dst_smem)), "l"(src) : "memory");
}
__global__ void __launch_bounds__(256) k_ekf_gemm1(int mode, const double *__restrict__ P, int ldP, const double *__restrict__ H, int ldH,
                                                   const double *__restrict__ Min, int ldM, const DevUpdateInfo *__restrict__ info, int X, int Y,
                                                   int K, double *__restrict__ Cout, int ldC, double sigma2, const double *__restrict__ Rdiag) {
  OVB_PDL_ENTER();
  extern __shared__ __align__(16) double g1[];
  const int x0 = blockIdx.x * EK_T, y0 = blockIdx.y * EK_T;
  if (mode == 1 && y0 > x0 + EK_T - 1)
    return;
  const int tid = threadIdx.x, tx = tid & 31, ty = tid >> 5;
  const int *cs = info->col_state;
  const int pk = K | 1;
  double *Gs = g1, *Hs = g1 + (size_t)K * 33;
  const double *Gsrc = (mode == 0) ? P : Min;
  const int ldG = (mode == 0) ? ldP : ldM;
  const int g0 = (mode == 0) ? x0 : y0, gmax = (mode == 0) ? X : Y;
  const int h0 = (mode == 0) ? y0 : x0, hmax = (mode == 0) ? Y : X;
  __shared__ int cs_s[EK1_KMAX];
  for (int j = tid; j < K; j += 256)
    cs_s[j] = cs[j];
  __syncthreads();
  for (int e = tid; e < K * 32; e += 256) {
    const int j = e >> 5, a = e & 31;
    if (g0 + a < gmax)
      ek_cpa8(&Gs[j * 33 + a], &Gsrc[(size_t)cs_s[j] * ldG + g0 + a]);
    else
      Gs[j * 33 + a] = 0.0;
  }
  for (int i = ty; i < 32; i += 8)
    for (int j = tx; j < K; j += 32) {
      if (h0 + i < hmax)
        ek_cpa8(&Hs[i * pk + j], &H[(size_t)(h0 + i) * ldH + j]);
      else
        Hs[i * pk + j] = 0.0;
    }
  asm volatile("cp.async.commit_group;" ::: "memory");
  asm volatile("cp.async.wait_group 0;" ::: "memory");
  __syncthreads();
  double acc[4] = {0, 0, 0, 0};
  if (mode == 0) {
    for (int j = 0; j < K; j++) {
      const double gv = Gs[j * 33 + tx];
#pragma unroll
      for (int u = 0; u < 4; u++)
        acc[u] += gv * Hs[(ty + 8 * u) * pk + j];
    }
#pragma unroll
    for (int u = 0; u < 4; u++) {
      const int a = x0 + tx, i = y0 + ty + 8 * u;
      if (a < X && i < Y)
        Cout[(size_t)a * ldC + i] = acc[u];
    }
  } else {
    for (int j = 0; j < K; j++) {
      const double gv = Gs[j * 33 + tx];
#pragma unroll
      for (int u = 0; u < 4; u++)
        acc[u] += Hs[(ty + 8 * u) * pk + j] * gv;
    }
#pragma unroll
    for (int u = 0; u < 4; u++) {
      const int i = x0 + ty + 8 * u, k = y0 + tx;
      if (i < X && k < Y) {
        double v = acc[u];
        if (i == k)
          v += Rdiag ? Rdiag[i] : sigma2;
        Cout[(size_t)i * ldC + k] = v;
      }
    }
  }
}

__global__ void __launch_bounds__(256) k_ekf_downdate1(double *__restrict__ P, int ldP, const double *__restrict__ Yin, int ldY, int N, int r,
                                                       const double *__restrict__ w, double *__restrict__ dx, DevUpdateInfo *__restrict__ info) {
  OVB_PDL_ENTER();
  extern __shared__ __align__(16) double d1[];
  const int a0 = blockIdx.x * EK_T, b0 = blockIdx.y * EK_T;
  if (b0 < a0)
    return;
  const int tid = threadIdx.x, tx = tid & 31, ty = tid >> 5;
  if (info->not_spd) {
    if (a0 == b0 && tid < EK_T && a0 + tid < N)
      dx[a0 + tid] = 0.0;
    return;
  }
  const int pk = r | 1;
  double *As = d1, *Bs = d1 + (size_t)32 * pk, *ws = Bs + (size_t)32 * pk;
  for (int i = ty; i < 32; i += 8)
    for (int k = tx; k < r; k += 32) {
      if (a0 + i < N)
        ek_cpa8(&As[i * pk + k], &Yin[(size_t)(a0 + i) * ldY + k]);
      else
        As[i * pk + k] = 0.0;
      if (b0 + i < N)
        ek_cpa8(&Bs[i * pk + k], &Yin[(size_t)(b0 + i) * ldY + k]);
      else
        Bs[i * pk + k] = 0.0;
    }
  for (int k = tid; k < r; k += 256)
    ek_cpa8(&ws[k], &w[k]);
  asm volatile("cp.async.commit_group;" ::: "memory");
  asm volatile("cp.async.wait_group 0;" ::: "memory");
  __syncthreads();
  double acc[4] = {0, 0, 0, 0};
  for (int k = 0; k < r; k++) {
    const double bv = Bs[tx * pk + k];
#pragma unroll
    for (int u = 0; u < 4; u++)
      acc[u] += As[(ty + 8 * u) * pk + k] * bv;
  }
#pragma unroll
  for (int u = 0; u < 4; u++) {
    const int a = a0 + ty + 8 * u, b = b0 + tx;
    if (a < N && b < N && b >= a) {
      const double v = P[(size_t)a * ldP + b] - acc[u];
      P[(size_t)a * ldP + b] = v;
      P[(size_t)b * ldP + a] = v;
      if (a == b && v < 0.0)
        atomicMin(&info->neg_diag_index, a);
      if (!isfinite(v))
        info->nonfinite = 1;
    }
  }
  if (a0 == b0 && tid < EK_T && a0 + tid < N) {
    double s0 = 0.0, s1 = 0.0;
    int k = 0;
    for (; k + 1 < r; k += 2) {
      s0 += As[tid * pk + k] * ws[k];
      s1 += As[tid * pk + k + 1] * ws[k + 1];
    }
    if (k < r)
      s0 += As[tid * pk + k] * ws[k];
    dx[a0 + tid] = s0 + s1;
  }
}

__global__ void k_ekf_prep(DevUpdateInfo *info, const int *skip) {
  OVB_PDL_ENTER();
  info->neg_diag_index = 0x7fffffff;
  info->not_spd = (skip && *skip) ? 1 : 0;
  info->nonfinite = 0;
}

void launch_ekf_update(ovb_ctx *ctx, const double *H, int ldHm, int r, int n, bool gate_only, double sigma2, const double *Rdiag_dev,
                       const int *skip_dev) {
  const int N = ctx->N;
  const int ld = ctx->ldP;
  double *P = ctx->P[ctx->cur];
  ovb_launch(ctx, k_ekf_prep, dim3(1), dim3(1), (size_t)(0), ctx->d_info, skip_dev);
  if (r <= 0 || n <= 0)
    return;
  if (!ctx->attr_done[2]) {
    cudaFuncSetAttribute(k_ekf_chol, cudaFuncAttributeMaxDynamicSharedMemorySize, 200 * 1024);
    cudaFuncSetAttribute(k_ekf_trsm, cudaFuncAttributeMaxDynamicSharedMemorySize, 200 * 1024);
    cudaFuncSetAttribute(k_ekf_gemm1, cudaFuncAttributeMaxDynamicSharedMemorySize, 100 * 1024);
    cudaFuncSetAttribute(k_ekf_downdate1, cudaFuncAttributeMaxDynamicSharedMemorySize, 100 * 1024);
    ctx->attr_done[2] = 1;
  }
  const bool one_shot = ctx->ekf_chol_dmma && n <= EK1_KMAX && r <= EK1_KMAX;
  dim3 g0((N + EK_T - 1) / EK_T, (r + EK_T - 1) / EK_T);
  dim3 g1((r + EK_T - 1) / EK_T, (r + EK_T - 1) / EK_T);
  if (one_shot) {
    const size_t sm01 = sizeof(double) * ((size_t)n * 33 + (size_t)32 * (n | 1));
    ovb_launch(ctx, k_ekf_gemm1, dim3(g0), dim3(256), sm01, 0, P, ld, H, ldHm, nullptr, 0, ctx->d_info, N, r, n, ctx->d_M, ld, 0.0, nullptr);
    ovb_launch(ctx, k_ekf_gemm1, dim3(g1), dim3(256), sm01, 1, P, ld, H, ldHm, ctx->d_M, ld, ctx->d_info, r, r, n, ctx->d_S, ld, sigma2, Rdiag_dev);
  } else {
    ovb_launch(ctx, k_ekf_gemm, dim3(g0), dim3(256), (size_t)(0), 0, P, ld, H, ldHm, nullptr, 0, ctx->d_info, N, r, n, ctx->d_M, ld, 0.0, nullptr);
    ovb_launch(ctx, k_ekf_gemm, dim3(g1), dim3(256), (size_t)(0), 1, P, ld, H, ldHm, ctx->d_M, ld, ctx->d_info, r, r, n, ctx->d_S, ld, sigma2, Rdiag_dev);
  }
  size_t chol_bytes = sizeof(double) * (size_t)(r + 1) * (size_t)(r | 1);
  int use_smem = chol_bytes <= 200 * 1024;
  double *invdiag = ctx->d_w + ctx->cfg.max_state;
  double *Lpk = nullptr;
  const bool dmma_chol = ctx->ekf_chol_dmma && launch_chol_ekf_dmma(ctx, ctx->d_S, ld, r, ctx->d_w, ctx->d_w, invdiag, &Lpk);
  const bool wide = !dmma_chol && ctx->ekf_chol_dmma && r < ld && launch_chol_solve_wide(ctx, ctx->d_S, ld, r, ctx->d_w, invdiag, ctx->d_M, ld, N, gate_only);
  if (wide) {
    if (gate_only)
      return;
    dim3 g2w((N + EK_T - 1) / EK_T, (N + EK_T - 1) / EK_T);
    ovb_launch(ctx, k_ekf_downdate, dim3(g2w), dim3(256), (size_t)(0), P, ld, (const double *)ctx->d_M, ld, N, r, ctx->d_w, ctx->d_dx, ctx->d_info);
    return;
  }
  if (!dmma_chol)
    ovb_launch(ctx, k_ekf_chol, dim3(1), dim3(EKC_THREADS), (size_t)(use_smem ? chol_bytes : 0), ctx->d_S, ld, r, ctx->d_w, ctx->d_w, invdiag, ctx->d_info, use_smem);
  if (gate_only)
    return;
  const double *Yd = ctx->d_Y;
  if (dmma_chol && Lpk != nullptr && launch_trsm_rows(ctx, ctx->d_M, ld, N, r, Lpk)) {
    Yd = ctx->d_M;
  } else {
    size_t trsm_small = sizeof(double) * ((size_t)TR_ROWS * r + r);
    size_t trsm_full = trsm_small + sizeof(double) * (size_t)r * (size_t)(r | 1);
    int L_in_smem = trsm_full <= 200 * 1024;
    ovb_launch(ctx, k_ekf_trsm, dim3((N + TR_ROWS - 1) / TR_ROWS), dim3(32 * TR_ROWS), (size_t)(L_in_smem ? trsm_full : trsm_small), ctx->d_M, ld, ctx->d_S, ld, invdiag, N,
               r, ctx->d_Y, ld, L_in_smem, ctx->d_info);
  }
  dim3 g2((N + EK_T - 1) / EK_T, (N + EK_T - 1) / EK_T);
  if (one_shot) {
    const size_t smd = sizeof(double) * ((size_t)64 * (r | 1) + r);
    ovb_launch(ctx, k_ekf_downdate1, dim3(g2), dim3(256), smd, P, ld, Yd, ld, N, r, ctx->d_w, ctx->d_dx, ctx->d_info);
  } else {
    ovb_launch(ctx, k_ekf_downdate, dim3(g2), dim3(256), (size_t)(0), P, ld, Yd, ld, N, r, ctx->d_w, ctx->d_dx, ctx->d_info);
  }
}


__global__ void k_cov_init_augment(double *__restrict__ P, int ld, int N, int k, int n, const DevUpdateInfo *__restrict__ info,
                                   const double *__restrict__ Hx, const double *__restrict__ Hinv, double sigma2, const int *__restrict__ skip) {
  extern __shared__ double ism[];
  double *m = ism, *M = ism + (size_t)N * k;
  const int tid = threadIdx.x;
  if (skip && *skip)
    return;
  for (int a = tid; a < N; a += blockDim.x) {
    for (int i = 0; i < k; i++) {
      double acc = 0.0;
      for (int j = 0; j < n; j++)
        acc += P[(size_t)a * ld + info->col_state[j]] * Hx[i * n + j];
      m[a * k + i] = acc;
    }
  }
  __syncthreads();
  if (tid < k * k) {
    const int i = tid / k, i2 = tid % k;
    double acc = 0.0;
    for (int j = 0; j < n; j++)
      acc += Hx[i * n + j] * m[info->col_state[j] * k + i2];
    M[i * k + i2] = acc + (i == i2 ? sigma2 : 0.0);
  }
  __syncthreads();
  if (tid < k * k) {
    const int i = tid / k, i2 = tid % k;
    if (i2 < i)
      M[i * k + i2] = M[i2 * k + i];
  }
  __syncthreads();
  for (int a = tid; a < N; a += blockDim.x) {
    for (int q = 0; q < k; q++) {
      double acc = 0.0;
      for (int i = 0; i < k; i++)
        acc += m[a * k + i] * Hinv[q * k + i];
      P[(size_t)a * ld + N + q] = -acc;
      P[(size_t)(N + q) * ld + a] = -acc;
    }
  }
  if (tid < k * k) {
    const int q = tid / k, q2 = tid % k;
    double acc = 0.0;
    for (int i = 0; i < k; i++)
      for (int i2 = 0; i2 < k; i2++)
        acc += Hinv[q * k + i] * M[i * k + i2] * Hinv[q2 * k + i2];
    if (q <= q2) {
      P[(size_t)(N + q) * ld + N + q2] = acc;
      P[(size_t)(N + q2) * ld + N + q] = acc;
    }
  }
}

bool launch_cov_init_augment(ovb_ctx *ctx, int k, int n, const double *Hx_dev, const double *Hinv_dev, double sigma2, const int *skip_dev) {
  const int N = ctx->N;
  size_t smem = sizeof(double) * ((size_t)N * k + (size_t)k * k);
  if (smem > 200 * 1024)
    return false;
  if (!ctx->attr_done[5]) {
    cudaFuncSetAttribute(k_cov_init_augment, cudaFuncAttributeMaxDynamicSharedMemorySize, 200 * 1024);
    ctx->attr_done[5] = 1;
  }
  k_cov_init_augment<<<1, 256, smem, ctx->stream>>>(ctx->P[ctx->cur], ctx->ldP, N, k, n, ctx->d_info, Hx_dev, Hinv_dev, sigma2, skip_dev);
  return cudaGetLastError() == cudaSuccess;
}

__global__ void k_init_prep(const DevFeat *__restrict__ feat, DevInitSys *__restrict__ sys, DevUpdateInfo *__restrict__ info, int k, int n) {
  const int tid = threadIdx.x;
  const bool ok = feat->status == OVB_FEAT_OK;
  if (ok)
    for (int j = tid; j < n; j += blockDim.x)
      info->col_state[j] = sys->col_state[j];
  if (tid != 0)
    return;
  sys->status = feat->status;
  sys->chi2 = feat->chi2;
  int fail = sys->n != n ? 2 : 0;
  const int o = 3 - k;
  double A[9], Inv[9];
  for (int i = 0; i < k; i++)
    for (int j = 0; j < k; j++) {
      A[i * k + j] = sys->HL[(o + i) * 3 + o + j];
      Inv[i * k + j] = (i == j) ? 1.0 : 0.0;
    }
  for (int c0 = 0; c0 < k && !fail; c0++) {
    int piv = c0;
    for (int i = c0 + 1; i < k; i++)
      if (fabs(A[i * k + c0]) > fabs(A[piv * k + c0]))
        piv = i;
    if (!(fabs(A[piv * k + c0]) > 0.0)) {
      fail = 1;
      break;
    }
    if (piv != c0)
      for (int j = 0; j < k; j++) {
        double t = A[c0 * k + j];
        A[c0 * k + j] = A[piv * k + j];
        A[piv * k + j] = t;
        t = Inv[c0 * k + j];
        Inv[c0 * k + j] = Inv[piv * k + j];
        Inv[piv * k + j] = t;
      }
    const double d = A[c0 * k + c0];
    for (int j = 0; j < k; j++) {
      A[c0 * k + j] /= d;
      Inv[c0 * k + j] /= d;
    }
    for (int i = 0; i < k; i++) {
      if (i == c0)
        continue;
      const double f = A[i * k + c0];
      for (int j = 0; j < k; j++) {
        A[i * k + j] -= f * A[c0 * k + j];
        Inv[i * k + j] -= f * Inv[c0 * k + j];
      }
    }
  }
  for (int q = 0; q < 3; q++) {
    double acc = 0.0;
    if (q < k)
      for (int i = 0; i < k; i++)
        acc += Inv[q * k + i] * sys->res[o + i];
    sys->dx_new[q] = acc;
  }
  for (int i = 0; i < k * k; i++)
    sys->Hinv[i] = Inv[i];
  sys->fail = ok ? fail : 0;
  sys->skip = (!ok || fail) ? 1 : 0;
}

void launch_init_prep(ovb_ctx *ctx, int feat, int k, int n) {
  k_init_prep<<<1, 256, 0, ctx->stream>>>(ctx->d_feat + feat, ctx->d_init, ctx->d_info, k, n);
}

__global__ void k_cov_clone(double *P, int ld, int N, int old_off, int size, const int *neg_diag) {
  int idx = blockIdx.x * blockDim.x + threadIdx.x;
  int N2 = N + size;
  if (idx >= N2 * size || (neg_diag && *neg_diag != 0x7fffffff))
    return;
  int i = idx / size, j = idx % size;
  double v;
  if (i < N)
    v = P[(size_t)i * ld + old_off + j];
  else
    v = P[(size_t)(old_off + (i - N)) * ld + old_off + j];
  double vr = (i < N) ? P[(size_t)(old_off + j) * ld + i] : v;
  P[(size_t)i * ld + N + j] = v;
  if (i < N)
    P[(size_t)(N + j) * ld + i] = vr;
}
__global__ void k_cov_dt_cols(double *P, int ld, int N2, int new_off, int size, int dt_off, const double *dnc, const int *neg_diag) {
  int idx = blockIdx.x * blockDim.x + threadIdx.x;
  if (idx >= N2 * size || (neg_diag && *neg_diag != 0x7fffffff))
    return;
  int i = idx / size, j = idx % size;
  P[(size_t)i * ld + new_off + j] += P[(size_t)i * ld + dt_off] * dnc[j];
}
__global__ void k_cov_dt_rows(double *P, int ld, int N2, int new_off, int size, int dt_off, const double *dnc, const int *neg_diag) {
  int idx = blockIdx.x * blockDim.x + threadIdx.x;
  if (idx >= N2 * size || (neg_diag && *neg_diag != 0x7fffffff))
    return;
  int i = idx / N2, j = idx % N2;
  P[(size_t)(new_off + i) * ld + j] += dnc[i] * P[(size_t)dt_off * ld + j];
}

void launch_cov_clone(ovb_ctx *ctx, int old_off, int size, const double *dnc_dt_dev, int dt_off, const int *neg_diag_dev) {
  double *P = ctx->P[ctx->cur];
  int N = ctx->N, N2 = N + size;
  int tot = N2 * size;
  k_cov_clone<<<(tot + 255) / 256, 256, 0, ctx->stream>>>(P, ctx->ldP, N, old_off, size, neg_diag_dev);
  if (dnc_dt_dev) {
    k_cov_dt_cols<<<(tot + 255) / 256, 256, 0, ctx->stream>>>(P, ctx->ldP, N2, N, size, dt_off, dnc_dt_dev, neg_diag_dev);
    k_cov_dt_rows<<<(tot + 255) / 256, 256, 0, ctx->stream>>>(P, ctx->ldP, N2, N, size, dt_off, dnc_dt_dev, neg_diag_dev);
  }
}

__global__ void k_cov_marg(const double *Pin, double *Pout, int ld, int N, int off, int size) {
  int N2 = N - size;
  int i = blockIdx.y * blockDim.y + threadIdx.y, j = blockIdx.x * blockDim.x + threadIdx.x;
  if (i >= N2 || j >= N2)
    return;
  int si = i < off ? i : i + size, sj = j < off ? j : j + size;
  double v = (i >= off && j < off) ? Pin[(size_t)sj * ld + si] : Pin[(size_t)si * ld + sj];
  Pout[(size_t)i * ld + j] = v;
}

void launch_cov_marginalize(ovb_ctx *ctx, int off, int size) {
  int N2 = ctx->N - size;
  dim3 b(32, 8), g((N2 + 31) / 32, (N2 + 7) / 8);
  k_cov_marg<<<g, b, 0, ctx->stream>>>(ctx->P[ctx->cur], ctx->P[ctx->cur ^ 1], ctx->ldP, ctx->N, off, size);
}

__global__ void k_prop_C(const double *P, int ld, int N, int p, int q, const int *old_idx, const double *Phi, double *Cbuf, int ldC) {
  int idx = blockIdx.x * blockDim.x + threadIdx.x;
  if (idx >= N * p)
    return;
  int a = idx / p, j = idx % p;
  double acc = 0.0;
  for (int k = 0; k < q; k++)
    acc += P[(size_t)a * ld + old_idx[k]] * Phi[(size_t)j * q + k];
  Cbuf[(size_t)a * ldC + j] = acc;
}
__global__ void k_prop_PCP(const double *Cbuf, int ldC, int p, int q, const int *old_idx, const double *Phi, const double *Q, double *Sbuf,
                           int ldS) {
  int idx = blockIdx.x * blockDim.x + threadIdx.x;
  if (idx >= p * p)
    return;
  int i = idx / p, j = idx % p;
  double acc = (i <= j) ? Q[(size_t)i * p + j] : Q[(size_t)j * p + i];
  for (int k = 0; k < q; k++)
    acc += Phi[(size_t)i * q + k] * Cbuf[(size_t)old_idx[k] * ldC + j];
  Sbuf[(size_t)i * ldS + j] = acc;
}
__global__ void k_prop_write(double *P, int ld, int N, int new_off, int p, const double *Cbuf, int ldC, const double *Sbuf, int ldS,
                             DevUpdateInfo *info) {
  int idx = blockIdx.x * blockDim.x + threadIdx.x;
  if (idx >= N * p)
    return;
  int a = idx / p, j = idx % p;
  if (a >= new_off && a < new_off + p) {
    double v = Sbuf[(size_t)(a - new_off) * ldS + j];
    P[(size_t)a * ld + new_off + j] = v;
    if (a - new_off == j && v < 0.0)
      atomicMin(&info->neg_diag_index, a);
  } else {
    double v = Cbuf[(size_t)a * ldC + j];
    P[(size_t)a * ld + new_off + j] = v;
    P[(size_t)(new_off + j) * ld + a] = v;
  }
}

void launch_cov_propagate(ovb_ctx *ctx, int new_off, int p, int q, const int *old_idx_dev, const double *Phi_dev, const double *Q_dev) {
  double *P = ctx->P[ctx->cur];
  int N = ctx->N, ld = ctx->ldP;
  ovb_launch(ctx, k_ekf_prep, dim3(1), dim3(1), (size_t)(0), ctx->d_info, (const int *)nullptr);
  k_prop_C<<<(N * p + 255) / 256, 256, 0, ctx->stream>>>(P, ld, N, p, q, old_idx_dev, Phi_dev, ctx->d_M, ld);
  k_prop_PCP<<<(p * p + 255) / 256, 256, 0, ctx->stream>>>(ctx->d_M, ld, p, q, old_idx_dev, Phi_dev, Q_dev, ctx->d_S, ld);
  k_prop_write<<<(N * p + 255) / 256, 256, 0, ctx->stream>>>(P, ld, N, new_off, p, ctx->d_M, ld, ctx->d_S, ld, ctx->d_info);
}

#define PA_THREADS 1024

__device__ __forceinline__ void pa_stage(double *dst, const double *src, int count, int tid) {
  for (int e = tid; e < count; e += PA_THREADS) {
    const unsigned d = (unsigned)__cvta_generic_to_shared(dst + e);
    asm volatile("cp.async.ca.shared.global [%0], [%1], 8;" ::"r"(d), "l"(src + e) : "memory");
  }
}

__global__ void __launch_bounds__(PA_THREADS) k_prop_accumulate(int n, int steps, const double *__restrict__ F, const double *__restrict__ G,
                                                                const double *__restrict__ qc, double *__restrict__ Phi_out,
                                                                double *__restrict__ Q_out) {
  extern __shared__ double pa_sm[];
  const int tid = threadIdx.x, nn = n * n, rec = nn + 12 * n + 4, npairs = n * (n + 1) / 2;
  double *Phi = pa_sm, *Phi2 = Phi + nn, *Q = Phi2 + nn, *T = Q + nn, *stg = T + nn;
  unsigned char *pi = (unsigned char *)(stg + 2 * rec), *pj = pi + npairs;
  for (int e = tid; e < nn; e += PA_THREADS) {
    Phi[e] = (e / n == e % n) ? 1.0 : 0.0;
    Q[e] = 0.0;
  }
  if (tid < n)
    for (int j = tid, t = tid * n - tid * (tid - 1) / 2; j < n; j++, t++)
      pi[t] = (unsigned char)tid, pj[t] = (unsigned char)j;
  auto stage = [&](int s) {
    double *r = stg + (s & 1) * rec;
    pa_stage(r, F + (size_t)s * nn, nn, tid);
    pa_stage(r + nn, G + (size_t)s * 12 * n, 12 * n, tid);
    pa_stage(r + nn + 12 * n, qc + (size_t)s * 4, 4, tid);
    asm volatile("cp.async.commit_group;" ::: "memory");
  };
  if (steps > 0)
    stage(0);
  for (int s = 0; s < steps; s++) {
    asm volatile("cp.async.wait_all;" ::: "memory");
    __syncthreads();
    if (s + 1 < steps)
      stage(s + 1);
    const double *f = stg + (s & 1) * rec, *g = f + nn, *w = g + 12 * n;
    for (int e = tid; e < 2 * nn; e += PA_THREADS) {
      const bool phi = e >= nn;
      const int ee = phi ? e - nn : e, i = ee / n, j = ee % n;
      const double *B = phi ? Phi : Q;
      double acc = 0.0;
      for (int k = 0; k < n; k++)
        acc = __dadd_rn(acc, __dmul_rn(f[i * n + k], B[k * n + j]));
      (phi ? Phi2 : T)[ee] = acc;
// ... 45 lines not shown
```

### open_vins_b200/csrc/ovb_api.cu

```cuda
#include "ovb_internal.cuh"
#include <chrono>
#include <algorithm>
#include <cmath>
#include <cstdio>
#include <cstdlib>
#include <cstring>
#include <new>
#include <vector>

static const double g_chi2_table[OVB_CHI2_TABLE_LEN] = {
#include "chi2_table.inc"
};

unsigned char *ovb_feat_order_ptr(ovb_ctx *ctx) { return ctx->d_feat_order; }

static size_t align_up(size_t v, size_t a) { return (v + a - 1) / a * a; }

extern "C" {

static ovb_status ensure_stage(ovb_ctx *ctx, size_t doubles);

int ovb_abi_version(void) { return OVB_ABI_VERSION; }

double ovb_chi2_quantile95(int dof) {
  if (dof < 1)
    return 0.0;
  if (dof >= OVB_CHI2_TABLE_LEN)
    dof = OVB_CHI2_TABLE_LEN - 1;
  return g_chi2_table[dof];
}

void ovb_opts_default(ovb_opts *o) {
  memset(o, 0, sizeof(*o));
  o->triangulate_1d = 0;
  o->refine_features = 1;
  o->max_runs = 5;
  o->init_lamda = 1e-3;
  o->max_lamda = 1e10;
  o->min_dx = 1e-6;
  o->min_dcost = 1e-6;
  o->lam_mult = 10;
  o->min_dist = 0.10;
  o->max_dist = 60;
  o->max_baseline = 40;
  o->max_cond_number = 10000;
  o->sigma_pix = 1;
  o->chi2_multipler = 5;
  o->do_fej = 1;
  o->feat_rep = OVB_REP_GLOBAL_3D;
  o->do_calib_camera_pose = 0;
  o->do_calib_camera_intrinsics = 0;
  o->col_order = OVB_COLS_CANONICAL;
  o->compress = OVB_COMPRESS_CHOLQR2;
}

const char *ovb_last_error(const ovb_ctx *ctx) { return ctx ? ctx->err : "null context"; }

ovb_status ovb_create(const ovb_config *cfg, ovb_ctx **out) {
  if (!cfg || !out)
    return OVB_ERR_ARG;
  *out = nullptr;
  ovb_ctx *ctx = new (std::nothrow) ovb_ctx();
  if (!ctx)
    return OVB_ERR_CAPACITY;
  memset(ctx, 0, sizeof(*ctx));
  ctx->cfg = *cfg;
  if (ctx->cfg.max_state < 32)
    ctx->cfg.max_state = 32;
  if (ctx->cfg.max_feats < 1)
    ctx->cfg.max_feats = 1;
  if (ctx->cfg.max_meas < 2)
    ctx->cfg.max_meas = 2;
  ctx->device = cfg->device;
  int ndev = 0;
  if (cudaGetDeviceCount(&ndev) != cudaSuccess || ndev <= 0 || cfg->device >= ndev) {
    delete ctx;
    return OVB_ERR_CUDA;
  }
#define CK(call)                                                                                                      \
  do {                                                                                                                \
    cudaError_t e_ = (call);                                                                                          \
    if (e_ != cudaSuccess) {                                                                                          \
      fprintf(stderr, "ovb_create: %s failed: %s\n", #call, cudaGetErrorString(e_));                                  \
      ovb_destroy(ctx);                                                                                               \
      return OVB_ERR_CUDA;                                                                                            \
    }                                                                                                                 \
  } while (0)
  CK(cudaSetDevice(ctx->device));
  cudaDeviceProp prop;
  CK(cudaGetDeviceProperties(&prop, ctx->device));
  ctx->sm_count = prop.multiProcessorCount;
  {
    const char *e = getenv("OVB_TSQR_CLUSTER");
    ctx->tsqr_cluster = e ? atoi(e) : 1;
    const char *e2 = getenv("OVB_TSQR_PDL");
    ctx->tsqr_pdl = e2 ? atoi(e2) : 1;
    const char *e3 = getenv("OVB_FEAT_CLASSES");
    ctx->feat_classes = e3 ? atoi(e3) : 1;
    const char *e4 = getenv("OVB_EKF_CHOL_DMMA");
    ctx->ekf_chol_dmma = e4 ? atoi(e4) : 1;
    const char *e5 = getenv("OVB_GRAM_CLUSTER");
    ctx->gram_cluster = e5 ? atoi(e5) : 0;
  }
  CK(cudaStreamCreateWithFlags(&ctx->stream, cudaStreamNonBlocking));
  ctx->own_stream = 1;
  CK(cudaStreamCreateWithFlags(&ctx->side_stream, cudaStreamNonBlocking));
  CK(cudaStreamCreateWithFlags(&ctx->side_stream2, cudaStreamNonBlocking));
  CK(cudaEventCreateWithFlags(&ctx->ev_join2, cudaEventDisableTiming));
  CK(cudaEventCreateWithFlags(&ctx->ev_fork, cudaEventDisableTiming));
  CK(cudaEventCreateWithFlags(&ctx->ev_join, cudaEventDisableTiming));
  for (int i = 0; i < 8; i++)
    CK(cudaEventCreate(&ctx->ev[i]));
  const int ms = ctx->cfg.max_state;
  ctx->ldP = ms;
  ctx->N = 0;
  ctx->cur = 0;
  CK(cudaMalloc(&ctx->P[0], sizeof(double) * (size_t)ms * ms));
  CK(cudaMalloc(&ctx->P[1], sizeof(double) * (size_t)ms * ms));
  CK(cudaMemset(ctx->P[0], 0, sizeof(double) * (size_t)ms * ms));
  CK(cudaMemset(ctx->P[1], 0, sizeof(double) * (size_t)ms * ms));
  ctx->off_opts = align_up(sizeof(DevFrame), 256);
  ctx->off_feat = ctx->off_opts + align_up(sizeof(DevOpts), 256);
  ctx->off_blob = ctx->off_feat + align_up(sizeof(DevFeat) * (size_t)ctx->cfg.max_feats, 256);
  ctx->blob_cap = align_up((size_t)ctx->cfg.max_meas * (1 + 2 + 8 + 8) + (size_t)ctx->cfg.max_feats * OVB_MAX_CAMS + 64, 256);
  ctx->arena_bytes = ctx->off_blob + ctx->blob_cap;
  CK(cudaMalloc(&ctx->d_arena, ctx->arena_bytes));
  CK(cudaMallocHost(&ctx->h_arena, ctx->arena_bytes));
  ctx->d_frame = (DevFrame *)ctx->d_arena;
  ctx->d_opts = (DevOpts *)(ctx->d_arena + ctx->off_opts);
  ctx->d_feat = (DevFeat *)(ctx->d_arena + ctx->off_feat);
  ctx->d_blob = ctx->d_arena + ctx->off_blob;
  ctx->h_frame = (DevFrame *)ctx->h_arena;
  ctx->h_opts = (DevOpts *)(ctx->h_arena + ctx->off_opts);
  ctx->h_feat = (DevFeat *)(ctx->h_arena + ctx->off_feat);
  ctx->h_blob = ctx->h_arena + ctx->off_blob;
  CK(cudaMalloc(&ctx->d_cc, sizeof(DevCamPoses)));
  CK(cudaMalloc(&ctx->d_feat_order, (size_t)ctx->cfg.max_feats * (OVB_MAX_VARS + 1)));
  ctx->info_bytes = align_up(sizeof(DevUpdateInfo), 256);
  CK(cudaMalloc(&ctx->d_info, ctx->info_bytes + sizeof(double) * (size_t)ms));
  ctx->d_dx = (double *)((char *)ctx->d_info + ctx->info_bytes);
  CK(cudaMallocHost(&ctx->h_info, ctx->info_bytes + sizeof(double) * (size_t)ms));
  ctx->h_dx = (double *)((char *)ctx->h_info + ctx->info_bytes);
  CK(cudaMalloc(&ctx->d_chi2_table, sizeof(g_chi2_table)));
  CK(cudaMemcpy(ctx->d_chi2_table, g_chi2_table, sizeof(g_chi2_table), cudaMemcpyHostToDevice));
  ctx->max_rows = ctx->cfg.max_rows > 0 ? ctx->cfg.max_rows : 2 * ctx->cfg.max_meas;
  if (ctx->max_rows < 2 * ctx->cfg.max_meas)
    ctx->max_rows = 2 * ctx->cfg.max_meas;
  int ldcap = std::min(OVB_MAX_COLS, ms) + 8;
  ctx->Hs_cap = (size_t)ctx->max_rows * ldcap;
  CK(cudaMalloc(&ctx->d_Hs, sizeof(double) * ctx->Hs_cap));
  ctx->h_stage = nullptr;
  ctx->stage_cap = 0;
  ctx->W_cap = ((size_t)ctx->max_rows / OVB_CR + 2 + (size_t)ctx->sm_count) * OVB_NB * OVB_NB + 4096;
  CK(cudaMalloc(&ctx->d_W[0], sizeof(double) * ctx->W_cap));
  CK(cudaMalloc(&ctx->d_W[1], sizeof(double) * ctx->W_cap));
  size_t rsz = (size_t)(ms + 8) * (ms + 8);
  CK(cudaMalloc(&ctx->d_R, sizeof(double) * rsz));
  CK(cudaMalloc(&ctx->d_R2, sizeof(double) * rsz));
  CK(cudaMalloc(&ctx->d_M, sizeof(double) * (size_t)ms * ms));
  CK(cudaMalloc(&ctx->d_S, sizeof(double) * (size_t)(ms + 1) * ms));
  CK(cudaMalloc(&ctx->d_Y, sizeof(double) * (size_t)ms * ms));
  CK(cudaMalloc(&ctx->d_w, sizeof(double) * (size_t)ms * 4));
  ctx->scratch_per_cta = (size_t)(2 * OVB_BIG_MAX_MEAS + 1) * (2 * OVB_BIG_MAX_MEAS + 1);
  ctx->scratch_ctas = 2 * ctx->sm_count;
  CK(cudaMalloc(&ctx->d_scratch, sizeof(double) * ctx->scratch_per_cta * ctx->scratch_ctas));
  ctx->dump_cap = 0;
  ctx->d_dump = nullptr;
  ctx->imu_cap = (size_t)OVB_PROP_STEPS_RESERVE * (39 * 39 + 12 * 39 + 4) + 64 + 39;
  CK(cudaMalloc(&ctx->d_imu, sizeof(double) * ctx->imu_cap));
  CK(cudaMallocHost(&ctx->h_imu, sizeof(double) * ctx->imu_cap));
#undef CK
  *out = ctx;
  return OVB_OK;
}

void ovb_destroy(ovb_ctx *ctx) {
  if (ctx)
    for (int i = 0; i < 2 * 96; i++)
      if (ctx->prof_ev[i])
        cudaEventDestroy(ctx->prof_ev[i]);
  if (!ctx)
    return;
  cudaSetDevice(ctx->device);
  if (ctx->stream)
    cudaStreamSynchronize(ctx->stream);
  void *dev[] = {ctx->P[0],   ctx->P[1], ctx->d_arena, ctx->d_cc, ctx->d_feat_order, ctx->d_info, ctx->d_chi2_table, ctx->d_Hs, ctx->d_W[0],
                 ctx->d_W[1], ctx->d_R,  ctx->d_R2,    ctx->d_M,  ctx->d_S,          ctx->d_Y,    ctx->d_w,          ctx->d_scratch,
                 ctx->d_long, ctx->d_dump, ctx->P_snap, ctx->d_flush, ctx->d_Gpart, ctx->d_G, ctx->d_cqw, ctx->d_grp, ctx->d_grp_acc, ctx->d_init, ctx->d_imu};
  for (void *p : dev)
    if (p)
      cudaFree(p);
  void *host[] = {ctx->h_arena, ctx->h_info, ctx->h_stage, ctx->h_grp, ctx->h_init, ctx->h_imu};
  for (void *p : host)
    if (p)
      cudaFreeHost(p);
  for (int i = 0; i < 8; i++)
    if (ctx->ev[i])
      cudaEventDestroy(ctx->ev[i]);
  if (ctx->ev_fork)
    cudaEventDestroy(ctx->ev_fork);
  if (ctx->ev_join)
    cudaEventDestroy(ctx->ev_join);
  if (ctx->ev_join2)
    cudaEventDestroy(ctx->ev_join2);
  if (ctx->side_stream2)
    cudaStreamDestroy(ctx->side_stream2);
  if (ctx->side_stream)
    cudaStreamDestroy(ctx->side_stream);
  if (ctx->stream && ctx->own_stream)
    cudaStreamDestroy(ctx->stream);
  delete ctx;
}

int ovb_cov_dim(const ovb_ctx *ctx) { return ctx ? ctx->N : 0; }

ovb_status ovb_cov_set(ovb_ctx *ctx, const double *P, int N) {
  if (!ctx || !P || N < 1)
    return OVB_ERR_ARG;
  if (N > ctx->cfg.max_state) {
    snprintf(ctx->err, sizeof(ctx->err), "ovb_cov_set: N=%d exceeds max_state=%d", N, ctx->cfg.max_state);
    return OVB_ERR_CAPACITY;
  }
  OVB_CUDA_CHECK(ctx, cudaSetDevice(ctx->device));
  OVB_CUDA_CHECK(ctx, cudaMemcpy2DAsync(ctx->P[ctx->cur], sizeof(double) * ctx->ldP, P, sizeof(double) * N, sizeof(double) * N, N,
                                        cudaMemcpyHostToDevice, ctx->stream));
  OVB_CUDA_CHECK(ctx, cudaStreamSynchronize(ctx->stream));
  ctx->N = N;
  return OVB_OK;
}

ovb_status ovb_cov_get(ovb_ctx *ctx, double *P, int N) {
  if (!ctx || !P || N != ctx->N)
    return OVB_ERR_ARG;
  OVB_CUDA_CHECK(ctx, cudaSetDevice(ctx->device));
  OVB_CUDA_CHECK(ctx, cudaMemcpy2DAsync(P, sizeof(double) * N, ctx->P[ctx->cur], sizeof(double) * ctx->ldP, sizeof(double) * N, N,
                                        cudaMemcpyDeviceToHost, ctx->stream));
  OVB_CUDA_CHECK(ctx, cudaStreamSynchronize(ctx->stream));
  return OVB_OK;
}

ovb_status ovb_cov_get_marginal(ovb_ctx *ctx, const int *off, const int *sz, int nvar, double *out) {
  if (!ctx || !off || !sz || !out || nvar < 1)
    return OVB_ERR_ARG;
  int n = 0;
  for (int i = 0; i < nvar; i++) {
    if (off[i] < 0 || sz[i] < 1 || off[i] + sz[i] > ctx->N)
      return OVB_ERR_ARG;
    n += sz[i];
  }
  OVB_CUDA_CHECK(ctx, cudaSetDevice(ctx->device));
  int ii = 0;
  for (int i = 0; i < nvar; i++) {
    int kk = 0;
    for (int k = 0; k < nvar; k++) {
      OVB_CUDA_CHECK(ctx, cudaMemcpy2DAsync(out + (size_t)ii * n + kk, sizeof(double) * n,
                                            ctx->P[ctx->cur] + (size_t)off[i] * ctx->ldP + off[k], sizeof(double) * ctx->ldP,
                                            sizeof(double) * sz[k], sz[i], cudaMemcpyDeviceToHost, ctx->stream));
      kk += sz[k];
    }
    ii += sz[i];
  }
  OVB_CUDA_CHECK(ctx, cudaStreamSynchronize(ctx->stream));
  return OVB_OK;
}

ovb_status ovb_cov_clone(ovb_ctx *ctx, int old_off, int size, const double *dnc_dt, int dt_off) {
  if (!ctx || size < 1 || old_off < 0 || old_off + size > ctx->N)
    return OVB_ERR_ARG;
  if (ctx->N + size > ctx->cfg.max_state) {
    snprintf(ctx->err, sizeof(ctx->err), "ovb_cov_clone: N+size=%d exceeds max_state=%d", ctx->N + size, ctx->cfg.max_state);
    return OVB_ERR_CAPACITY;
  }
  if (dnc_dt && (dt_off < 0 || dt_off >= ctx->N || size > 64))
    return OVB_ERR_ARG;
  OVB_CUDA_CHECK(ctx, cudaSetDevice(ctx->device));
  const double *dnc_dev = nullptr;
  if (dnc_dt) {
    memcpy(ctx->h_dx, dnc_dt, sizeof(double) * size);
    OVB_CUDA_CHECK(ctx, cudaMemcpyAsync(ctx->d_w, ctx->h_dx, sizeof(double) * size, cudaMemcpyHostToDevice, ctx->stream));
    dnc_dev = ctx->d_w;
  }
  launch_cov_clone(ctx, old_off, size, dnc_dev, dt_off);
  OVB_CUDA_CHECK(ctx, cudaGetLastError());
  OVB_CUDA_CHECK(ctx, cudaStreamSynchronize(ctx->stream));
  ctx->N += size;
  return OVB_OK;
}

ovb_status ovb_cov_marginalize(ovb_ctx *ctx, int off, int size) {
  if (!ctx || size < 1 || off < 0 || off + size > ctx->N)
    return OVB_ERR_ARG;
  OVB_CUDA_CHECK(ctx, cudaSetDevice(ctx->device));
  launch_cov_marginalize(ctx, off, size);
  OVB_CUDA_CHECK(ctx, cudaGetLastError());
  OVB_CUDA_CHECK(ctx, cudaStreamSynchronize(ctx->stream));
  ctx->cur ^= 1;
  ctx->N -= size;
  return OVB_OK;
}

ovb_status ovb_cov_propagate(ovb_ctx *ctx, int new_off, int p, const int *old_off, const int *old_sz, int nold, const double *Phi,
                             const double *Q) {
  if (!ctx || !old_off || !old_sz || !Phi || !Q || p < 1 || nold < 1 || new_off < 0 || new_off + p > ctx->N)
    return OVB_ERR_ARG;
  int q = 0;
  for (int i = 0; i < nold; i++) {
    if (old_off[i] < 0 || old_sz[i] < 1 || old_off[i] + old_sz[i] > ctx->N)
      return OVB_ERR_ARG;
    q += old_sz[i];
  }
  if (q > ctx->cfg.max_state || p > ctx->cfg.max_state || (size_t)p * q + (size_t)p * p > ctx->Hs_cap)
    return OVB_ERR_CAPACITY;
  OVB_CUDA_CHECK(ctx, cudaSetDevice(ctx->device));
  {
    ovb_status es = ensure_stage(ctx, (size_t)p * q + (size_t)p * p + (size_t)q + 16);
    if (es != OVB_OK)
      return es;
  }
  double *hs = ctx->h_stage;
  memcpy(hs, Phi, sizeof(double) * (size_t)p * q);
  memcpy(hs + (size_t)p * q, Q, sizeof(double) * (size_t)p * p);
  int *hidx = (int *)(hs + (size_t)p * q + (size_t)p * p);
  int c = 0;
  for (int i = 0; i < nold; i++)
    for (int k = 0; k < old_sz[i]; k++)
      hidx[c++] = old_off[i] + k;
  size_t bytes = sizeof(double) * ((size_t)p * q + (size_t)p * p) + sizeof(int) * q;
  OVB_CUDA_CHECK(ctx, cudaMemcpyAsync(ctx->d_Hs, hs, bytes, cudaMemcpyHostToDevice, ctx->stream));
  const double *Phi_dev = ctx->d_Hs;
  const double *Q_dev = ctx->d_Hs + (size_t)p * q;
  const int *idx_dev = (const int *)(ctx->d_Hs + (size_t)p * q + (size_t)p * p);
  launch_cov_propagate(ctx, new_off, p, q, idx_dev, Phi_dev, Q_dev);
  OVB_CUDA_CHECK(ctx, cudaGetLastError());
  OVB_CUDA_CHECK(ctx, cudaMemcpyAsync(ctx->h_info, ctx->d_info, sizeof(DevUpdateInfo), cudaMemcpyDeviceToHost, ctx->stream));
  OVB_CUDA_CHECK(ctx, cudaStreamSynchronize(ctx->stream));
  if (ctx->h_info->neg_diag_index != 0x7fffffff) {
    snprintf(ctx->err, sizeof(ctx->err), "EKFPropagation: diagonal at %d is negative", ctx->h_info->neg_diag_index);
    return OVB_ERR_NEG_DIAG;
  }
  return OVB_OK;
}

ovb_status ovb_cov_propagate_imu(ovb_ctx *ctx, int n, int steps, const double *F, const double *G, const double *qc, int new_off, const int *old_off,
                                 const int *old_sz, int nold, int clone_off, int clone_size, const double *dnc_dt, int dt_off, double *Phi_out,
                                 double *Q_out) {
  if (!ctx)
    return OVB_ERR_ARG;
  if (n > OVB_PROP_MAX_N) {
    snprintf(ctx->err, sizeof(ctx->err), "ovb_cov_propagate_imu: n=%d exceeds %d", n, OVB_PROP_MAX_N);
    return OVB_ERR_CAPACITY;
  }
  if (n < 1 || steps < 0 || (steps > 0 && (!F || !G || !qc)) || !old_off || !old_sz || nold < 1 || new_off < 0 || new_off + n > ctx->N)
    return OVB_ERR_ARG;
  int q = 0;
  for (int i = 0; i < nold; i++) {
    if (old_off[i] < 0 || old_sz[i] < 1 || old_off[i] + old_sz[i] > ctx->N)
      return OVB_ERR_ARG;
    q += old_sz[i];
  }
  if (q != n)
    return OVB_ERR_ARG;
  if (clone_size < 1 || clone_off < 0 || clone_off + clone_size > ctx->N || (dnc_dt && (dt_off < 0 || dt_off >= ctx->N || clone_size > 64)))
    return OVB_ERR_ARG;
  if (ctx->N + clone_size > ctx->cfg.max_state) {
    snprintf(ctx->err, sizeof(ctx->err), "ovb_cov_propagate_imu: N+clone_size=%d exceeds max_state=%d", ctx->N + clone_size, ctx->cfg.max_state);
    return OVB_ERR_CAPACITY;
  }
  const size_t nn = (size_t)n * n;
  if (2 * nn > ctx->Hs_cap)
    return OVB_ERR_CAPACITY;
  OVB_CUDA_CHECK(ctx, cudaSetDevice(ctx->device));
  const size_t oF = 0, oG = oF + (size_t)steps * nn, oq = oG + (size_t)steps * 12 * n, od = oq + (size_t)steps * 4,
               oi = od + (dnc_dt ? (size_t)clone_size : 0), in_doubles = oi + ((size_t)n + 1) / 2;
  const size_t need = std::max(in_doubles, 2 * nn);
  if (need > ctx->imu_cap) {
    const size_t cap = need + need / 2;
    cudaFree(ctx->d_imu);
    cudaFreeHost(ctx->h_imu);
    ctx->d_imu = nullptr, ctx->h_imu = nullptr, ctx->imu_cap = 0;
    OVB_CUDA_CHECK(ctx, cudaMalloc(&ctx->d_imu, sizeof(double) * cap));
    OVB_CUDA_CHECK(ctx, cudaMallocHost(&ctx->h_imu, sizeof(double) * cap));
    ctx->imu_cap = cap;
  }
  double *hs = ctx->h_imu;
  if (steps > 0) {
    memcpy(hs + oF, F, sizeof(double) * (size_t)steps * nn);
    memcpy(hs + oG, G, sizeof(double) * (size_t)steps * 12 * n);
    memcpy(hs + oq, qc, sizeof(double) * (size_t)steps * 4);
  }
  if (dnc_dt)
    memcpy(hs + od, dnc_dt, sizeof(double) * clone_size);
  int *hidx = (int *)(hs + oi);
  for (int i = 0, c = 0; i < nold; i++)
    for (int k = 0; k < old_sz[i]; k++)
      hidx[c++] = old_off[i] + k;
  OVB_CUDA_CHECK(ctx, cudaMemcpyAsync(ctx->d_imu, hs, sizeof(double) * in_doubles, cudaMemcpyHostToDevice, ctx->stream));
  double *Phi_dev = ctx->d_Hs, *Q_dev = ctx->d_Hs + nn;
  if (!launch_prop_accumulate(ctx, n, steps, ctx->d_imu + oF, ctx->d_imu + oG, ctx->d_imu + oq, Phi_dev, Q_dev)) {
    snprintf(ctx->err, sizeof(ctx->err), "ovb_cov_propagate_imu: k_prop_accumulate launch failed: %s", cudaGetErrorString(cudaGetLastError()));
    OVB_CUDA_CHECK(ctx, cudaStreamSynchronize(ctx->stream));
    return OVB_ERR_CUDA;
  }
  launch_cov_propagate(ctx, new_off, n, n, (const int *)(ctx->d_imu + oi), Phi_dev, Q_dev);
  launch_cov_clone(ctx, clone_off, clone_size, dnc_dt ? ctx->d_imu + od : nullptr, dt_off, &ctx->d_info->neg_diag_index);
  OVB_CUDA_CHECK(ctx, cudaGetLastError());
  OVB_CUDA_CHECK(ctx, cudaMemcpyAsync(&ctx->h_info->neg_diag_index, &ctx->d_info->neg_diag_index, sizeof(int), cudaMemcpyDeviceToHost, ctx->stream));
  if (Phi_out || Q_out)
    OVB_CUDA_CHECK(ctx, cudaMemcpyAsync(hs, Phi_dev, sizeof(double) * 2 * nn, cudaMemcpyDeviceToHost, ctx->stream));
  OVB_CUDA_CHECK(ctx, cudaStreamSynchronize(ctx->stream));
  if (Phi_out)
    memcpy(Phi_out, hs, sizeof(double) * nn);
  if (Q_out)
    memcpy(Q_out, hs + nn, sizeof(double) * nn);
  if (ctx->h_info->neg_diag_index != 0x7fffffff) {
    snprintf(ctx->err, sizeof(ctx->err), "EKFPropagation: diagonal at %d is negative", ctx->h_info->neg_diag_index);
    return OVB_ERR_NEG_DIAG;
  }
  ctx->N += clone_size;
  return OVB_OK;
}

struct Packed {
  int n_feats, n_meas, m_total, ldH, n_all;
  int n_groups;
  BlobView bv;
};

static ovb_status ensure_groups(ovb_ctx *ctx, int n) {
  if (n > 1) {
    if (!ctx->P_snap)
      OVB_CUDA_CHECK(ctx, cudaMalloc(&ctx->P_snap, sizeof(double) * (size_t)ctx->ldP * ctx->ldP));
    if (!ctx->d_grp_acc)
      OVB_CUDA_CHECK(ctx, cudaMalloc(&ctx->d_grp_acc, sizeof(double) * ((size_t)ctx->cfg.max_state + 4)));
  }
  if (n <= ctx->grp_cap)
    return OVB_OK;
  if (ctx->d_grp)
    cudaFree(ctx->d_grp);
  if (ctx->h_grp)
    cudaFreeHost(ctx->h_grp);
  ctx->d_grp = nullptr;
  ctx->h_grp = nullptr;
  ctx->grp_cap = 0;
  const int cap = std::max(n, 4);
  OVB_CUDA_CHECK(ctx, cudaMalloc(&ctx->d_grp, sizeof(DevGroup) * (size_t)cap));
  OVB_CUDA_CHECK(ctx, cudaMallocHost(&ctx->h_grp, sizeof(DevGroup) * (size_t)cap));
  ctx->grp_cap = cap;
  return OVB_OK;
}

static int slam_lm_width(int rep) { return rep == OVB_REP_ANCHORED_INVERSE_DEPTH_SINGLE ? 1 : 3; }

static ovb_status build_groups(ovb_ctx *ctx, int F, int rows_total, Packed *pk) {
  const DevFrame *hf = ctx->h_frame;
  const int room = OVB_MAX_COLS - hf->n_all;
  std::vector<int> f0;
  for (int f = 0, acc = 0; f < F; f++) {
    const int w = slam_lm_width(ctx->h_feat[f].rep);
    if (f == 0 || acc + w > room) {
      f0.push_back(f);
      acc = 0;
    }
    acc += w;
  }
  const int G = (int)f0.size();
  f0.push_back(F);
  if (room < 3 || G > 0xffff) {
    snprintf(ctx->err, sizeof(ctx->err), "SLAM batch of %d landmarks: %d column groups", F, G);
    return OVB_ERR_CAPACITY;
  }
  ovb_status st = ensure_groups(ctx, G);
  if (st != OVB_OK)
    return st;
  int widest = 0;
  std::vector<std::pair<int, int>> lms;
  for (int g = 0; g < G; g++) {
    DevGroup &gr = ctx->h_grp[g];
    gr.f0 = f0[g];
    gr.f1 = f0[g + 1];
    gr.row0 = ctx->h_feat[gr.f0].row0;
    gr.rows = (gr.f1 < F ? ctx->h_feat[gr.f1].row0 : rows_total) - gr.row0;
    lms.clear();
    for (int f = gr.f0; f < gr.f1; f++)
      lms.push_back({ctx->h_feat[f].lm_off, f});
    std::sort(lms.begin(), lms.end());
    int col = 0, n_ent = 0;
    size_t l = 0;
    for (int s = 0; s < hf->n_slots || l < lms.size();) {
      if (l < lms.size() && (s == hf->n_slots || lms[l].first < hf->slot_off[s])) {
        const int f = lms[l++].second;
        gr.ent[n_ent++] = -1 - f;
// ... 1609 lines not shown
```

### open_vins_b200/csrc/ovb_internal.cuh

```cuda
#pragma once
#include "../../include/ovb200.h"
#include <cuda_runtime.h>
#include <stdint.h>

#define OVB_BIG_MAX_MEAS 128
#define OVB_MAX_COLS 512
#define OVB_NB 16
#define OVB_CR 256
#define OVB_PROP_MAX_N 64
#define OVB_PROP_STEPS_RESERVE 64

struct DevFrame {
  int n_clones, n_cams;
  int n_slots;
  int n_all;
  double clone_R[OVB_MAX_CLONES][9];
  double clone_p[OVB_MAX_CLONES][3];
  double clone_R_fej[OVB_MAX_CLONES][9];
  double clone_p_fej[OVB_MAX_CLONES][3];
  double cam_R[OVB_MAX_CAMS][9];
  double cam_p[OVB_MAX_CAMS][3];
  double cam_intr[OVB_MAX_CAMS][8];
  int cam_model[OVB_MAX_CAMS];
  int slot_off[OVB_MAX_VARS];
  int slot_size[OVB_MAX_VARS];
  int slot_col[OVB_MAX_VARS];
  int clone_slot[OVB_MAX_CLONES];
  int cam_ext_slot[OVB_MAX_CAMS];
  int cam_intr_slot[OVB_MAX_CAMS];
  const struct DevGroup *groups;
  int lm_w;
};

struct DevGroup {
  int f0, f1;
  int row0, rows;
  int n_cols;
  int n_ent;
  int ent[OVB_MAX_VARS + OVB_MAX_COLS];
  int col_state[OVB_MAX_COLS];
  short col_frame[OVB_MAX_COLS];
};

struct DevCamPoses {
  double cc_R[OVB_MAX_CAMS][OVB_MAX_CLONES][9];
  double cc_p[OVB_MAX_CAMS][OVB_MAX_CLONES][3];
};

struct DevOpts {
  ovb_opts o;
  double sigma_pix_sq;
  int rep;
};

struct DevFeat {
  int m0, m1;
  int row0;
  int key0, key1;
  int status;
  int anchor_cam, anchor_clone;
  int sched;
  int rep;
  double p_FinA[3], p_FinG[3];
  double chi2;
  double p_FinG_fej[3];
  double sigma_sq;
  double chi2_mult;
  int lm_off;
  unsigned short lm_col, grp;
};

struct DevUpdateInfo {
  int n_used;
  int n_feats_used;
  int rows_stacked;
  int n_order;
  int order_slot[OVB_MAX_VARS];
  int col_state[OVB_MAX_COLS];
  int col_canon[OVB_MAX_COLS];
  int neg_diag_index;
  int not_spd;
  int nonfinite;
};

struct DevInitSys {
  int status;
  int skip;
  int fail;
  int pad;
  double chi2;
  double dx_new[3];
  int n;
  int col_state[OVB_MAX_COLS];
  double HL[9];
  double res[3];
  double HR[3 * OVB_MAX_COLS];
  double Hinv[9];
};
#define OVB_INIT_HEAD_BYTES (4 * sizeof(int) + 4 * sizeof(double))

struct BlobView {
  const uint8_t *cam;
  const uint16_t *clone;
  const float *uv;
  const float *uvn;
  const uint8_t *keys;
};

struct ovb_ctx {
  ovb_config cfg;
  int device;
  cudaStream_t stream;
  int own_stream;
  cudaStream_t side_stream;
  cudaStream_t side_stream2;
  cudaEvent_t ev_fork, ev_join, ev_join2;
  int feat_classes;
  cudaEvent_t ev[8];
  char err[256];
  int N, ldP;
  double *P[2];
  int cur;
  unsigned char *d_arena, *h_arena;
  size_t arena_bytes, off_opts, off_feat, off_blob;
  DevFrame *d_frame;
  DevOpts *d_opts;
  DevFeat *d_feat;
  unsigned char *d_blob;
  DevFrame *h_frame;
  DevOpts *h_opts;
  DevFeat *h_feat;
  unsigned char *h_blob;
  size_t blob_cap;
  DevCamPoses *d_cc;
  unsigned char *d_feat_order;
  DevUpdateInfo *d_info;
  DevUpdateInfo *h_info;
  double *h_dx;
  double *h_stage;
  size_t stage_cap;
  double *d_chi2_table;
  double *d_Hs;
  size_t Hs_cap;
  double *d_W[2];
  size_t W_cap;
  double *d_R;
  double *d_R2;
  double *d_M;
  double *d_S;
  double *d_Y;
  double *d_w;
  double *d_dx;
  double *d_scratch;
  size_t scratch_per_cta;
  int scratch_ctas;
  double *d_long;
  size_t long_cap;
  double *d_dump;
  size_t dump_cap;
  int dump_rows;
  int max_rows;
  int sm_count;
  size_t info_bytes;
  int attr_done[8];
  int tsqr_pdl;
  int tsqr_cluster;
  int gram_cluster;
  int ekf_chol_dmma;
  mutable float stage_ms[6];
  mutable int stage_pending;
  double host_us[4];
  int replay_enabled, last_pk_valid;
  int last_n_feats, last_m_total, last_ldH, last_n_all, last_col_order;
  BlobView last_bv;
  double *P_snap;
  void *d_flush;
  DevGroup *d_grp, *h_grp;
  int grp_cap;
  double *d_grp_acc;
  int slam_unbounded;
  int n_launch, n_launch_tsqr_level;
  double *d_Gpart, *d_G;
  size_t Gpart_cap, G_cap;
  double *d_cqw;
  size_t cqw_cap;
  size_t last_h2d_bytes, last_d2h_bytes;
  DevInitSys *d_init, *h_init;
  int64_t init_counters[4];
  double *d_imu, *h_imu;
  size_t imu_cap;
  int prof_on, prof_n;
  cudaEvent_t prof_ev[2 * 96];
  const void *prof_fn[96];
};

#define OVB_CUDA_CHECK(ctx, call)                                                                                     \
  do {                                                                                                                \
    cudaError_t e_ = (call);                                                                                          \
    if (e_ != cudaSuccess) {                                                                                          \
      snprintf((ctx)->err, sizeof((ctx)->err), "%s:%d %s: %s", __FILE__, __LINE__, #call, cudaGetErrorString(e_));    \
      return OVB_ERR_CUDA;                                                                                            \
    }                                                                                                                 \
  } while (0)

void launch_cam_poses(ovb_ctx *ctx);
void launch_triangulate(ovb_ctx *ctx, int n_feats, BlobView bv);
void launch_feature_system(ovb_ctx *ctx, int n_feats, BlobView bv, int ldH, int mode);
ovb_status feature_scratch_reserve(ovb_ctx *ctx, int n_feats, bool slam, bool init = false);
void launch_feature_init(ovb_ctx *ctx, int sched, BlobView bv, int ldH);
void launch_init_prep(ovb_ctx *ctx, int feat, int k, int n);
void launch_column_map(ovb_ctx *ctx, int n_feats, BlobView bv, int rows_drop = 3);
void launch_column_map_slam(ovb_ctx *ctx, int n_feats, bool full_map);
void launch_tsqr(ovb_ctx *ctx, double *A, int m, int n, int ldA, double *Rout, int ldR);
int launch_compress_gram(ovb_ctx *ctx, const double *A, int m, int n, int ldA, double *Rout, int ldR);
int launch_compress_cholqr2(ovb_ctx *ctx, double *A, int m, int n, int ldA, double *Rout, int ldR);
bool launch_chol_ekf_dmma(ovb_ctx *ctx, double *S, int ldS, int r, const double *res, double *w, double *invdiag, double **Lpk_out);
bool launch_trsm_rows(ovb_ctx *ctx, double *A, int ldA, int m, int nt, const double *Lpk);
bool launch_chol_solve_wide(ovb_ctx *ctx, double *S, int ldS, int r, double *w, double *invdiag, double *M, int ldM, int N, bool gate_only);
void launch_reorder_R(ovb_ctx *ctx, const double *Rin, int n_all, int ldRin, double *Rout, int ldRout);
void launch_ekf_update(ovb_ctx *ctx, const double *H, int ldHm, int r, int n, bool gate_only, double sigma2, const double *Rdiag_dev,
                       const int *skip_dev = nullptr);
bool launch_cov_init_augment(ovb_ctx *ctx, int k, int n, const double *Hx_dev, const double *Hinv_dev, double sigma2,
                             const int *skip_dev = nullptr);
void launch_cov_clone(ovb_ctx *ctx, int old_off, int size, const double *dnc_dt_dev, int dt_off, const int *neg_diag_dev = nullptr);
void launch_cov_marginalize(ovb_ctx *ctx, int off, int size);
void launch_cov_propagate(ovb_ctx *ctx, int new_off, int p, int q, const int *old_idx_dev, const double *Phi_dev, const double *Q_dev);
bool launch_prop_accumulate(ovb_ctx *ctx, int n, int steps, const double *F_dev, const double *G_dev, const double *qc_dev, double *Phi_dev,
                            double *Q_dev);

#define OVB_PDL_ENTER()                                                     \
  do {                                                                      \
    asm volatile("griddepcontrol.launch_dependents;" ::: "memory");         \
    asm volatile("griddepcontrol.wait;" ::: "memory");                      \
  } while (0)

#ifdef __CUDACC__
template <typename... KArgs, typename... Args>
static inline void ovb_launch(ovb_ctx *ctx, void (*kern)(KArgs...), dim3 grid, dim3 block, size_t smem, Args &&...args) {
  cudaLaunchConfig_t cfg = {};
  cfg.gridDim = grid;
  cfg.blockDim = block;
  cfg.dynamicSmemBytes = smem;
  cfg.stream = ctx->stream;
  cudaLaunchAttribute at[1];
  at[0].id = cudaLaunchAttributeProgrammaticStreamSerialization;
  at[0].val.programmaticStreamSerializationAllowed = 1;
  cfg.attrs = at;
  cfg.numAttrs = (ctx->tsqr_pdl && !ctx->prof_on) ? 1 : 0;
  const bool prof = ctx->prof_on && ctx->prof_n < 96 && ctx->prof_ev[0] != nullptr;
  if (prof)
    cudaEventRecord(ctx->prof_ev[2 * ctx->prof_n], ctx->stream);
  cudaLaunchKernelEx(&cfg, kern, static_cast<KArgs>(args)...);
  if (prof) {
    cudaEventRecord(ctx->prof_ev[2 * ctx->prof_n + 1], ctx->stream);
    ctx->prof_fn[ctx->prof_n++] = (const void *)kern;
  }
}
#endif
```

Baseline: 2328.

## Stream Cholesky factor columns to dependent TRSM kernels via global epoch counter

The single-CTA Cholesky kernels now publish each finished block column of the packed factor to global memory from a spare warp and bump an epoch-tagged release counter. The downstream TRSM and solve-gram kernels launch early through PDL, dedicate one warp to polling that counter, and issue bulk async copies into shared memory guarded by per-column mbarriers. Compute warps wait only on the column they need, so the triangular solve overlaps with the factorization instead of waiting for the whole kernel to finish. The cost is cross-kernel spin polling with a timeout fallback, one fewer compute warp in the consumer, extra global stores, and a risk of deadlock or ordering bugs if the producer and consumer are not co-resident.

```diff
diff --git a/open_vins_b200/csrc/chol_tiles.cuh b/open_vins_b200/csrc/chol_tiles.cuh
--- a/open_vins_b200/csrc/chol_tiles.cuh
+++ b/open_vins_b200/csrc/chol_tiles.cuh
@@ -228,8 +228,11 @@
   }
 }
 
-template <int THREADS>
-__device__ __forceinline__ void ct_chol_tiles(const CtView &sm, int n, int nrows, bool strict, double floor_d) {
+struct CtNoPublish {
+  __device__ __forceinline__ void column(const CtView &, int) const {}
+};
+template <int THREADS, typename PUB = CtNoPublish>
+__device__ __forceinline__ void ct_chol_tiles(const CtView &sm, int n, int nrows, bool strict, double floor_d, const PUB &pub = PUB()) {
   const int tid = threadIdx.x, lane = tid & 31, wid = tid >> 5;
   constexpr int NW = THREADS / 32, NH = NW - (NW + 3) / 4;
   static_assert(NH >= 1, "need at least one helper warp");
@@ -316,6 +319,8 @@
         }
       }
       CT_PROBE_T(p3);
+    } else if (wid == 8 && k > 0) {
+      pub.column(sm, k - 1);
     }
     __syncthreads();
     CT_PROBE_T(p5);
diff --git a/open_vins_b200/csrc/k_cholqr.cu b/open_vins_b200/csrc/k_cholqr.cu
--- a/open_vins_b200/csrc/k_cholqr.cu
+++ b/open_vins_b200/csrc/k_cholqr.cu
@@ -31,6 +31,21 @@
 template <int N> __device__ __forceinline__ void cpa_wait() { asm volatile("cp.async.wait_group %0;" ::"n"(N) : "memory"); }
 __device__ __forceinline__ void bar_group(int id, int nthreads) { asm volatile("bar.sync %0, %1;" ::"r"(id), "r"(nthreads) : "memory"); }
 __device__ __forceinline__ int tri(int b) { return (b * (b + 1)) >> 1; }
+
+__device__ __forceinline__ void cq_pub_store(unsigned long long *ctr, unsigned long long v) {
+  asm volatile("st.release.gpu.global.u64 [%0], %1;" ::"l"(ctr), "l"(v) : "memory");
+}
+__device__ __forceinline__ unsigned long long cq_pub_load(const unsigned long long *ctr) {
+  unsigned long long v;
+  asm volatile("ld.acquire.gpu.global.u64 %0, [%1];" : "=l"(v) : "l"(ctr) : "memory");
+  return v;
+}
+__device__ __forceinline__ void cq_fence_proxy() { asm volatile("fence.proxy.async.global;" ::: "memory"); }
+__device__ __forceinline__ void cq_mbar_init(unsigned bar) { asm volatile("mbarrier.init.shared::cta.b64 [%0], 1;" ::"r"(bar) : "memory"); }
+__device__ __forceinline__ void cq_mbar_arrive(unsigned bar) { asm volatile("mbarrier.arrive.shared::cta.b64 _, [%0];" ::"r"(bar) : "memory"); }
+__device__ __forceinline__ void cq_mbar_wait(unsigned bar) {
+  asm volatile("{\n\t.reg .pred p;\n\tCQ_MWAIT:\n\tmbarrier.try_wait.parity.shared::cta.b64 p, [%0], 0;\n\t@!p bra CQ_MWAIT;\n\t}" ::"r"(bar) : "memory");
+}
 
 __device__ __forceinline__ bool cq_tile_origin(int blk, int w, int BW, int nblk_side, int &ci, int &cj, int &offI, int &offJ, bool &diag) {
   int bI = 0, t = blk;
@@ -255,7 +270,40 @@
 
 namespace {
 
-__device__ __forceinline__ void cq_chol_tiles(CqCholSmem &sm, int n, int nrows, bool strict, double floor_d) {
+struct CqPublish {
+  double *Lpk;
+  unsigned long long *ctr, epoch;
+  int n;
+  __device__ __forceinline__ void column(const CtView &sm, int k) const {
+    if (ctr == nullptr)
+      return;
+    const int lane = threadIdx.x & 31, NB = (n + 7) >> 3;
+    for (int i = k; i < NB; i++) {
+      const size_t o = (size_t)(ct_tri(i) + k) * 64 + 2 * lane;
+      *reinterpret_cast<double2 *>(Lpk + o) = *reinterpret_cast<const double2 *>(sm.T + o);
+    }
+    if (lane < 8)
+      Lpk[CQ_PK_INV + 8 * k + lane] = (8 * k + lane < n) ? sm.invd[8 * k + lane] : 1.0;
+    cq_fence_proxy();
+    __threadfence();
+    __syncwarp();
+    if (lane == 0)
+      cq_pub_store(ctr, (epoch << 6) | (unsigned long long)(k + 2));
+  }
+  __device__ __forceinline__ int first_tile_el() const { return ctr ? (tri((n + 7) >> 3) - 1) * 64 : 0; }
+  __device__ __forceinline__ int first_pivot() const { return ctr ? 8 * (((n + 7) >> 3) - 1) : 0; }
+  __device__ __forceinline__ void finish() const {
+    if (ctr == nullptr)
+      return;
+    cq_fence_proxy();
+    __threadfence();
+    __syncthreads();
+    if (threadIdx.x == 0)
+      cq_pub_store(ctr, (epoch << 6) | (unsigned long long)(((n + 7) >> 3) + 1));
+  }
+};
+
+__device__ __forceinline__ void cq_chol_tiles(CqCholSmem &sm, int n, int nrows, bool strict, double floor_d, const CqPublish &pub) {
   CtView v;
   v.T = sm.T;
   v.Xp0 = sm.Xp[0];
@@ -266,7 +314,7 @@
   v.dummyT = sm.dummyT;
   v.dummyX = sm.dummyX;
   v.flag = &sm.flag;
-  ct_chol_tiles<CQ_CHOL_T>(v, n, nrows, strict, floor_d);
+  ct_chol_tiles<CQ_CHOL_T>(v, n, nrows, strict, floor_d, pub);
 }
 
 __device__ void cq_load_tiles(CqCholSmem &sm, const double *__restrict__ G, size_t ldG, int n, int nrows, const double *__restrict__ rhs, int ld_rhs) {
@@ -299,8 +347,12 @@
 
 }
 
-__global__ void __launch_bounds__(CQ_CHOL_T) k_cq_chol_gram(const double *__restrict__ G, int ldG, int n, double shift_rel, double *__restrict__ Lpk, int tiled) {
+__global__ void __launch_bounds__(CQ_CHOL_T) k_cq_chol_gram(const double *__restrict__ G, int ldG, int n, double shift_rel, double *__restrict__ Lpk, int tiled,
+                                                           unsigned long long *pub_ctr, unsigned long long epoch) {
   OVB_PDL_ENTER();
+  if (pub_ctr != nullptr && threadIdx.x == 0)
+    cq_pub_store(pub_ctr, (epoch << 6) | 1ull);
+  const CqPublish pub{Lpk, pub_ctr, epoch, n};
   extern __shared__ __align__(16) unsigned char cq_raw[];
   CqCholSmem &sm = *reinterpret_cast<CqCholSmem *>(cq_raw);
   const int tid = threadIdx.x, lane = tid & 31, wid = tid >> 5;
@@ -366,15 +418,16 @@
 #ifdef CQ_PROBE
   const long long q1 = clock64();
 #endif
-  cq_chol_tiles(sm, n, n, false, 0.25 * shift);
+  cq_chol_tiles(sm, n, n, false, 0.25 * shift, pub);
 #ifdef CQ_PROBE
   const long long q2 = clock64();
 #endif
   const int NB = (n + 7) >> 3;
-  for (int e = 2 * tid; e < tri(NB) * 64; e += 2 * CQ_CHOL_T)
+  for (int e = pub.first_tile_el() + 2 * tid; e < tri(NB) * 64; e += 2 * CQ_CHOL_T)
     *reinterpret_cast<double2 *>(Lpk + e) = *reinterpret_cast<const double2 *>(sm.T + e);
-  for (int e = tid; e < CQ_MAXB * 8; e += CQ_CHOL_T)
+  for (int e = pub.first_pivot() + tid; e < CQ_MAXB * 8; e += CQ_CHOL_T)
     Lpk[CQ_PK_INV + e] = (e < n) ? sm.invd[e] : 1.0;
+  pub.finish();
 #ifdef CQ_PROBE
   if (tid == 0)
     printf("chol_gram n=%d: load %lld factor %lld store %lld cycles\n", n, q1 - q0, q2 - q1, clock64() - q2);
@@ -383,8 +436,11 @@
 
 __global__ void __launch_bounds__(CQ_CHOL_T) k_cq_chol_ekf(double *__restrict__ S, int ldS, int r, const double *__restrict__ res, double *__restrict__ w,
                                                           double *__restrict__ invdiag, DevUpdateInfo *__restrict__ info, double *__restrict__ Lpk,
-                                                          const double *__restrict__ floor_dev) {
+                                                          const double *__restrict__ floor_dev, unsigned long long *pub_ctr, unsigned long long epoch) {
   OVB_PDL_ENTER();
+  if (pub_ctr != nullptr && threadIdx.x == 0)
+    cq_pub_store(pub_ctr, (epoch << 6) | 1ull);
+  const CqPublish pub{Lpk, pub_ctr, epoch, r};
   extern __shared__ __align__(16) unsigned char cq_raw[];
   CqCholSmem &sm = *reinterpret_cast<CqCholSmem *>(cq_raw);
   const int tid = threadIdx.x, lane = tid & 31, wid = tid >> 5;
@@ -392,9 +448,17 @@
   cq_load_tiles(sm, S, (size_t)ldS, r, nrows, res, 0);
   __syncthreads();
   if (floor_dev != nullptr)
-    cq_chol_tiles(sm, r, nrows, false, *floor_dev);
+    cq_chol_tiles(sm, r, nrows, false, *floor_dev, pub);
   else
-    cq_chol_tiles(sm, r, nrows, true, 0.0);
+    cq_chol_tiles(sm, r, nrows, true, 0.0, pub);
+  if (Lpk != nullptr) {
+    const int NB = (r + 7) >> 3;
+    for (int e = pub.first_tile_el() + 2 * tid; e < tri(NB) * 64; e += 2 * CQ_CHOL_T)
+      *reinterpret_cast<double2 *>(Lpk + e) = *reinterpret_cast<const double2 *>(sm.T + e);
+    for (int e = pub.first_pivot() + tid; e < CQ_MAXB * 8; e += CQ_CHOL_T)
+      Lpk[CQ_PK_INV + e] = (e < r) ? sm.invd[e] : 1.0;
+    pub.finish();
+  }
   for (int i = wid; i < r; i += CQ_CHOL_T / 32)
     for (int j = lane; j <= i; j += 32)
       S[(size_t)i * ldS + j] = cq_el(sm.T, i, j);
@@ -404,25 +468,20 @@
   if (invdiag != nullptr)
     for (int j = tid; j < r; j += CQ_CHOL_T)
       invdiag[j] = sm.invd[j];
-  if (Lpk != nullptr) {
-    const int NB = (r + 7) >> 3;
-    for (int e = 2 * tid; e < tri(NB) * 64; e += 2 * CQ_CHOL_T)
-      *reinterpret_cast<double2 *>(Lpk + e) = *reinterpret_cast<const double2 *>(sm.T + e);
-    for (int e = tid; e < CQ_MAXB * 8; e += CQ_CHOL_T)
-      Lpk[CQ_PK_INV + e] = (e < r) ? sm.invd[e] : 1.0;
-  }
   if (tid == 0 && sm.flag && info != nullptr)
     info->not_spd = 1;
 }
 
 #define CQ_TRSM_NH 10
 #define CQ_TRSM_SMEM (sizeof(double) * ((size_t)CQ_PK_DOUBLES + (size_t)(CQ_TRSM_T / 32) * CQ_TRSM_NH * 2 * 32))
-template <int NH>
-__device__ __forceinline__ void cq_trsm_half(double (&acc)[NH][2], int b0, const double *Lt, const double *Ri, double *xs, int lane) {
+template <int NH, bool WAIT = false>
+__device__ __forceinline__ void cq_trsm_half(double (&acc)[NH][2], int b0, const double *Lt, const double *Ri, double *xs, int lane, unsigned cbar = 0) {
   const int g = lane >> 2, q = lane & 3;
 #pragma unroll
   for (int jb = 0; jb < NH; jb++) {
     const int B = b0 + jb;
+    if constexpr (WAIT)
+      cq_mbar_wait(cbar + 8 * B);
     const double *Ld = Lt + (size_t)(tri(B) + B) * 64;
     const double *ri = Ri + B * 8;
     double x[8];
@@ -514,18 +573,91 @@
   __syncthreads();
 }
 
-template <int NH1, int NH2>
-__global__ void __launch_bounds__(CQ_TRSM_T) k_cq_trsm(double *__restrict__ A, int ldA, int m, int nt, const double *__restrict__ Lpk) {
-  OVB_PDL_ENTER();
+template <int NBP, int NT>
+__device__ __forceinline__ void cq_stream_init(unsigned long long *bars, double *Lt, double *Ri, int NB) {
+  const int tid = threadIdx.x;
+  if (tid == 0) {
+    for (int j = 0; j <= NBP; j++)
+      cq_mbar_init(s_u32(bars + j));
+    asm volatile("fence.mbarrier_init.release.cluster;" ::: "memory");
+  }
+  for (int e = tri(NB) * 64 + tid; e < tri(NBP) * 64; e += NT)
+    Lt[e] = 0.0;
+  for (int e = NB * 8 + tid; e < NBP * 8; e += NT)
+    Ri[e] = 1.0;
+  __syncthreads();
+}
+
+#define CQ_STREAM_POLL_NS 20000000ull
+
+__device__ void cq_stream_fetch(unsigned long long *bars, double *Lt, double *Ri, const double *__restrict__ Lpk, int NB, int NBP,
+                                const unsigned long long *ctr, unsigned long long epoch) {
+  const unsigned long long base = epoch << 6;
+  unsigned long long t0, t;
+  asm volatile("mov.u64 %0, %%globaltimer;" : "=l"(t0));
+  bool poll = true;
+  auto reach = [&](int s) {
+    while (poll && cq_pub_load(ctr) < (base | (unsigned long long)s)) {
+      asm volatile("mov.u64 %0, %%globaltimer;" : "=l"(t));
+      if (t - t0 > CQ_STREAM_POLL_NS) {
+        asm volatile("griddepcontrol.wait;" ::: "memory");
+        poll = false;
+      } else {
+        __nanosleep(64);
+      }
+    }
+  };
+  reach(1);
+  cq_mbar_arrive(s_u32(bars));
+  for (int j = NB; j < NBP; j++)
+    cq_mbar_arrive(s_u32(bars + 1 + j));
+  for (int j = 0; j < NB; j++) {
+    reach(j + 2);
+    cq_fence_proxy();
+    const unsigned bar = s_u32(bars + 1 + j);
+    asm volatile("mbarrier.arrive.expect_tx.shared::cta.b64 _, [%0], %1;" ::"r"(bar), "r"((unsigned)((NB - j) * 64 + 8) * 8u) : "memory");
+    for (int i = j; i < NB; i++) {
+      const size_t o = (size_t)(tri(i) + j) * 64;
+      asm volatile("cp.async.bulk.shared::cluster.global.mbarrier::complete_tx::bytes [%0], [%1], 512, [%2];" ::"r"(s_u32(Lt + o)), "l"(Lpk + o), "r"(bar)
+                   : "memory");
+    }
+    asm volatile("cp.async.bulk.shared::cluster.global.mbarrier::complete_tx::bytes [%0], [%1], 64, [%2];" ::"r"(s_u32(Ri + 8 * j)), "l"(Lpk + CQ_PK_INV + 8 * j),
+                 "r"(bar)
+                 : "memory");
+  }
+  asm volatile("griddepcontrol.wait;" ::: "memory");
+  for (int j = 0; j < NB; j++)
+    cq_mbar_wait(s_u32(bars + 1 + j));
+}
+
+template <int NH1, int NH2, bool STREAM>
+__device__ __forceinline__ void cq_trsm_rows(double *__restrict__ A, int ldA, int m, int nt, const double *__restrict__ Lpk,
+                                             const unsigned long long *__restrict__ pub_ctr, unsigned long long epoch) {
   extern __shared__ __align__(16) double tsm[];
   double *Lt = tsm;
   double *Ri = tsm + CQ_PK_INV;
   double *Xs = tsm + CQ_PK_DOUBLES;
   const int tid = threadIdx.x, lane = tid & 31, wid = tid >> 5, g = lane >> 2, q = lane & 3;
-  cq_fetch_factor<NH1 + NH2, CQ_TRSM_T>(Lt, Ri, Lpk, (nt + 7) >> 3);
+  unsigned cbar = 0;
+  if constexpr (STREAM) {
+    asm volatile("griddepcontrol.launch_dependents;" ::: "memory");
+    __shared__ __align__(8) unsigned long long bars[CQ_MAXB + 1];
+    cq_stream_init<NH1 + NH2, CQ_TRSM_T>(bars, Lt, Ri, (nt + 7) >> 3);
+    if (wid == CQ_TRSM_T / 32 - 1) {
+      if (lane == 0)
+        cq_stream_fetch(bars, Lt, Ri, Lpk, (nt + 7) >> 3, NH1 + NH2, pub_ctr, epoch);
+      return;
+    }
+    cq_mbar_wait(s_u32(bars));
+    cbar = s_u32(bars + 1);
+  } else {
+    OVB_PDL_ENTER();
+    cq_fetch_factor<NH1 + NH2, CQ_TRSM_T>(Lt, Ri, Lpk, (nt + 7) >> 3);
+  }
   double *xs = Xs + (size_t)wid * (CQ_TRSM_NH * 2 * 32);
   const int ngroups = (m + 7) >> 3;
-  for (int rg = blockIdx.x + gridDim.x * wid; rg < ngroups; rg += gridDim.x * (CQ_TRSM_T / 32)) {
+  constexpr int NSW = CQ_TRSM_T / 32 - (STREAM ? 1 : 0);
+  for (int rg = blockIdx.x + gridDim.x * wid; rg < ngroups; rg += gridDim.x * NSW) {
     const int row = 8 * rg + g;
     const bool row_ok = row < m;
     double *arow = A + (size_t)row * ldA;
@@ -538,7 +670,7 @@
 #ifdef CQ_PROBE
       t1 = clock64();
 #endif
-      cq_trsm_half<NH1>(acc, 0, Lt, Ri, NH2 > 0 ? xs : nullptr, lane);
+      cq_trsm_half<NH1, STREAM>(acc, 0, Lt, Ri, NH2 > 0 ? xs : nullptr, lane, cbar);
 #ifdef CQ_PROBE
       t2 = clock64();
 #endif
@@ -561,7 +693,7 @@
 #ifdef CQ_PROBE
       t3 = clock64();
 #endif
-      cq_trsm_half<NH2>(acc, NH1, Lt, Ri, nullptr, lane);
+      cq_trsm_half<NH2, STREAM>(acc, NH1, Lt, Ri, nullptr, lane, cbar);
 #ifdef CQ_PROBE
       t4 = clock64();
 #endif
@@ -574,18 +706,45 @@
 #endif
   }
 }
-
-static void cq_launch_trsm(ovb_ctx *ctx, int ctas, double *A, int ldA, int m, int nt, const double *Lpk) {
+template <int NH1, int NH2>
+__global__ void __launch_bounds__(CQ_TRSM_T) k_cq_trsm(double *__restrict__ A, int ldA, int m, int nt, const double *__restrict__ Lpk) {
+  cq_trsm_rows<NH1, NH2, false>(A, ldA, m, nt, Lpk, nullptr, 0);
+}
+template <int NH1, int NH2>
+__global__ void __launch_bounds__(CQ_TRSM_T) k_cq_trsm(double *__restrict__ A, int ldA, int m, int nt, const double *__restrict__ Lpk,
+                                                      const unsigned long long *__restrict__ pub_ctr, unsigned long long epoch) {
+  cq_trsm_rows<NH1, NH2, true>(A, ldA, m, nt, Lpk, pub_ctr, epoch);
+}
+using CqTrsmKernel = void (*)(double *, int, int, int, const double *);
+using CqTrsmStreamKernel = void (*)(double *, int, int, int, const double *, const unsigned long long *, unsigned long long);
+
+template <bool STREAM>
+static void cq_launch_trsm_t(ovb_ctx *ctx, int ctas, double *A, int ldA, int m, int nt, const double *Lpk, const unsigned long long *pub_ctr,
+                             unsigned long long epoch) {
   const int NB = (nt + 7) / 8;
   const size_t smem = CQ_TRSM_SMEM;
+  const dim3 grid(ctas), block(CQ_TRSM_T);
+  auto go = [&](auto plain, auto streaming) {
+    if constexpr (STREAM)
+      ovb_launch(ctx, streaming, grid, block, smem, A, ldA, m, nt, Lpk, pub_ctr, epoch);
+    else
+      ovb_launch(ctx, plain, grid, block, smem, A, ldA, m, nt, Lpk);
+  };
   if (NB <= 5)
-    ovb_launch(ctx, k_cq_trsm<5, 0>, dim3(ctas), dim3(CQ_TRSM_T), smem, A, ldA, m, nt, Lpk);
+    go((CqTrsmKernel)k_cq_trsm<5, 0>, (CqTrsmStreamKernel)k_cq_trsm<5, 0>);
   else if (NB <= 10)
-    ovb_launch(ctx, k_cq_trsm<10, 0>, dim3(ctas), dim3(CQ_TRSM_T), smem, A, ldA, m, nt, Lpk);
+    go((CqTrsmKernel)k_cq_trsm<10, 0>, (CqTrsmStreamKernel)k_cq_trsm<10, 0>);
   else if (NB <= 15)
-    ovb_launch(ctx, k_cq_trsm<10, 5>, dim3(ctas), dim3(CQ_TRSM_T), smem, A, ldA, m, nt, Lpk);
+    go((CqTrsmKernel)k_cq_trsm<10, 5>, (CqTrsmStreamKernel)k_cq_trsm<10, 5>);
   else
-    ovb_launch(ctx, k_cq_trsm<10, 10>, dim3(ctas), dim3(CQ_TRSM_T), smem, A, ldA, m, nt, Lpk);
+    go((CqTrsmKernel)k_cq_trsm<10, 10>, (CqTrsmStreamKernel)k_cq_trsm<10, 10>);
+}
+static void cq_launch_trsm(ovb_ctx *ctx, int ctas, double *A, int ldA, int m, int nt, const double *Lpk, const unsigned long long *pub_ctr = nullptr,
+                           unsigned long long epoch = 0) {
+  if (pub_ctr != nullptr)
+    cq_launch_trsm_t<true>(ctx, ctas, A, ldA, m, nt, Lpk, pub_ctr, epoch);
+  else
+    cq_launch_trsm_t<false>(ctx, ctas, A, ldA, m, nt, Lpk, pub_ctr, epoch);
 }
 
 #define CQ_SG_SMEM (226 * 1024)
@@ -596,13 +755,13 @@
 }
 
 template <int NH1, int NH2>
-__device__ __forceinline__ void cq_solve_group(double *xrow, bool row_ok, const double *Lt, const double *Ri, int lane) {
+__device__ __forceinline__ void cq_solve_group(double *xrow, bool row_ok, const double *Lt, const double *Ri, int lane, unsigned cbar) {
   constexpr int NBP = NH1 + NH2;
   const int g = lane >> 2, q = lane & 3;
   {
     double acc[NH1][2];
     cq_trsm_load<NH1>(acc, xrow, row_ok, 0, 8 * NBP, q);
-    cq_trsm_half<NH1>(acc, 0, Lt, Ri, nullptr, lane);
+    cq_trsm_half<NH1, true>(acc, 0, Lt, Ri, nullptr, lane, cbar);
     cq_trsm_store<NH1>(acc, xrow, row_ok, 0, 8 * NBP, q);
   }
   if constexpr (NH2 > 0) {
@@ -619,15 +778,16 @@
         dmma(acc[j][0], acc[j][1], af1, lf[4]);
       }
     }
-    cq_trsm_half<NH2>(acc, NH1, Lt, Ri, nullptr, lane);
+    cq_trsm_half<NH2, true>(acc, NH1, Lt, Ri, nullptr, lane, cbar);
     cq_trsm_store<NH2>(acc, xrow, row_ok, NH1, 8 * NBP, q);
   }
 }
 
 template <int NH1, int NH2>
 __global__ void __launch_bounds__(CQ_GRAM_T) k_cq_solve_gram(const double *__restrict__ A, int ldA, int m, int nt, const double *__restrict__ Lpk, int slab_rows,
-                                                            int cb, int ntail_max, int BW, double *__restrict__ Gpart, double *__restrict__ Qtail) {
-  OVB_PDL_ENTER();
+                                                          int cb, int ntail_max, int BW, double *__restrict__ Gpart, double *__restrict__ Qtail,
+                                                          const unsigned long long *__restrict__ pub_ctr, unsigned long long epoch) {
+  asm volatile("griddepcontrol.launch_dependents;" ::: "memory");
   extern __shared__ __align__(16) double ssm[];
   double *Lt = ssm;
   double *Ri = ssm + CQ_PK_INV;
@@ -638,26 +798,46 @@
   double *tail = Qtail + (size_t)blockIdx.x * ntail_max * pitch;
   auto split_at = [&](int rc) { return r1 - rc > cb && r1 - rc <= 8 * (CQ_GRAM_T / 32); };
   auto nbuf_at = [&](int rc) { return split_at(rc) ? cb & ~7 : min(cb, (r1 - rc + 3) & ~3); };
-  if (r0 < r1)
-    cq_issue_rows<CQ_GRAM_T>(X, pitch, A, ldA, r0, nbuf_at(r0), r1, nt, 0, 0, pitch - 4, 1);
-  cq_fetch_factor<NBP, CQ_GRAM_T>(Lt, Ri, Lpk, (nt + 7) >> 3);
+  constexpr int NF = CQ_GRAM_T - 32;
+  const int lane = threadIdx.x & 31, wid = threadIdx.x >> 5, g = lane >> 2, q = lane & 3, lr = 8 * wid + g;
+  const bool fetcher = threadIdx.x >= NF;
+  __shared__ __align__(8) unsigned long long bars[CQ_MAXB + 1];
+  cq_stream_init<NBP, CQ_GRAM_T>(bars, Lt, Ri, (nt + 7) >> 3);
+  const unsigned cbar = s_u32(bars + 1);
+  if (fetcher) {
+    if (lane == 0)
+      cq_stream_fetch(bars, Lt, Ri, Lpk, (nt + 7) >> 3, NBP, pub_ctr, epoch);
+    __syncwarp();
+  } else {
+    cq_mbar_wait(s_u32(bars));
+    if (r0 < r1)
+      cq_issue_rows<NF>(X, pitch, A, ldA, r0, nbuf_at(r0), r1, nt, 0, 0, pitch - 4, 1);
+  }
   for (int rc = r0, nbuf = nbuf_at(r0), ntail = 0; rc < r1; rc += nbuf + ntail, nbuf = nbuf_at(rc)) {
     ntail = split_at(rc) ? (r1 - rc - nbuf + 3) & ~3 : 0;
     const int nact = nbuf + ntail;
-    if (rc > r0)
+    const bool first = rc == r0;
+    if (!first)
       cq_issue_rows<CQ_GRAM_T>(X, pitch, A, ldA, rc, nbuf, r1, nt, 0, 0, pitch - 4, 1);
-    for (int e = threadIdx.x; e < ntail * (pitch - 4); e += CQ_GRAM_T) {
-      const int k = e / (pitch - 4), col = e - k * (pitch - 4), r = rc + nbuf + k;
-      tail[(size_t)k * pitch + col] = (r < r1 && col < nt) ? A[(size_t)r * ldA + col] : 0.0;
-    }
+    if (!(first && fetcher))
+      for (int e = threadIdx.x; e < ntail * (pitch - 4); e += first ? NF : CQ_GRAM_T) {
+        const int k = e / (pitch - 4), col = e - k * (pitch - 4), r = rc + nbuf + k;
+        tail[(size_t)k * pitch + col] = (r < r1 && col < nt) ? A[(size_t)r * ldA + col] : 0.0;
+      }
     cpa_wait<0>();
-    __syncthreads();
-    const int lane = threadIdx.x & 31, wid = threadIdx.x >> 5, g = lane >> 2, q = lane & 3, lr = 8 * wid + g;
+    if (!first) {
+      bar_group(1, CQ_GRAM_T);
+    } else if (fetcher) {
+      asm volatile("bar.sync 3, %0;" ::"n"(CQ_GRAM_T) : "memory");
+    } else {
+      asm volatile("bar.arrive 3, %0;" ::"n"(CQ_GRAM_T) : "memory");
+      bar_group(2, NF);
+    }
     if (8 * wid < nbuf)
-      cq_solve_group<NH1, NH2>(X + (size_t)min(lr, nbuf - 1) * pitch, lr < nbuf, Lt, Ri, lane);
+      cq_solve_group<NH1, NH2>(X + (size_t)min(lr, nbuf - 1) * pitch, lr < nbuf, Lt, Ri, lane, cbar);
     else if (8 * wid < nact)
-      cq_solve_group<NH1, NH2>(tail + (size_t)min(lr - nbuf, ntail - 1) * pitch, lr < nact, Lt, Ri, lane);
-    __syncthreads();
+      cq_solve_group<NH1, NH2>(tail + (size_t)min(lr - nbuf, ntail - 1) * pitch, lr < nact, Lt, Ri, lane, cbar);
+    bar_group(1, CQ_GRAM_T);
     int ci, cj, offI, offJ;
     bool diag;
     const bool active = cq_tile_origin(0, wid, BW, 1, ci, cj, offI, offJ, diag);
@@ -681,7 +861,7 @@
         for (int b = 0; b < 4; b++)
           *reinterpret_cast<double2 *>(part + a * 256 + 8 * b) = make_double2(acc[a][b][0], acc[a][b][1]);
     }
-    __syncthreads();
+    bar_group(1, CQ_GRAM_T);
   }
 }
 
@@ -705,22 +885,22 @@
 
 template <int NH1, int NH2>
 static void cq_launch_solve_gram_t(ovb_ctx *ctx, int nslab, const double *A, int ldA, int m, int nt, const double *Lpk, int slab_rows, int BW, double *Gpart,
-                                   double *Qtail) {
+                                   double *Qtail, const unsigned long long *pub_ctr, unsigned long long epoch) {
   const CqSgShape s = cq_sg_shape(nt, BW, slab_rows);
   const size_t smem = sizeof(double) * (CQ_PK_DOUBLES + (size_t)s.cb * s.pitch);
-  ovb_launch(ctx, k_cq_solve_gram<NH1, NH2>, dim3(nslab), dim3(CQ_GRAM_T), smem, A, ldA, m, nt, Lpk, slab_rows, s.cb, s.ntail, BW, Gpart, Qtail);
+  ovb_launch(ctx, k_cq_solve_gram<NH1, NH2>, dim3(nslab), dim3(CQ_GRAM_T), smem, A, ldA, m, nt, Lpk, slab_rows, s.cb, s.ntail, BW, Gpart, Qtail, pub_ctr, epoch);
 }
 static void cq_launch_solve_gram(ovb_ctx *ctx, int nslab, const double *A, int ldA, int m, int nt, const double *Lpk, int slab_rows, int BW, double *Gpart,
-                                 double *Qtail) {
+                                 double *Qtail, const unsigned long long *pub_ctr, unsigned long long epoch) {
   const int NB = (nt + 7) / 8;
   if (NB <= 5)
-    cq_launch_solve_gram_t<5, 0>(ctx, nslab, A, ldA, m, nt, Lpk, slab_rows, BW, Gpart, Qtail);
+    cq_launch_solve_gram_t<5, 0>(ctx, nslab, A, ldA, m, nt, Lpk, slab_rows, BW, Gpart, Qtail, pub_ctr, epoch);
   else if (NB <= 10)
-    cq_launch_solve_gram_t<10, 0>(ctx, nslab, A, ldA, m, nt, Lpk, slab_rows, BW, Gpart, Qtail);
+    cq_launch_solve_gram_t<10, 0>(ctx, nslab, A, ldA, m, nt, Lpk, slab_rows, BW, Gpart, Qtail, pub_ctr, epoch);
   else if (NB <= 15)
-    cq_launch_solve_gram_t<10, 5>(ctx, nslab, A, ldA, m, nt, Lpk, slab_rows, BW, Gpart, Qtail);
+    cq_launch_solve_gram_t<10, 5>(ctx, nslab, A, ldA, m, nt, Lpk, slab_rows, BW, Gpart, Qtail, pub_ctr, epoch);
   else
-    cq_launch_solve_gram_t<10, 10>(ctx, nslab, A, ldA, m, nt, Lpk, slab_rows, BW, Gpart, Qtail);
+    cq_launch_solve_gram_t<10, 10>(ctx, nslab, A, ldA, m, nt, Lpk, slab_rows, BW, Gpart, Qtail, pub_ctr, epoch);
 }
 
 __global__ void __launch_bounds__(256) k_cq_trmm(const double *__restrict__ L2, const double *__restrict__ L1, int nt, double *__restrict__ Rout, int ldR) {
@@ -931,10 +1111,14 @@
     cudaFuncSetAttribute(k_cq_gram, cudaFuncAttributeMaxDynamicSharedMemorySize, 160 * 1024);
     cudaFuncSetAttribute(k_cq_chol_gram, cudaFuncAttributeMaxDynamicSharedMemorySize, (int)sizeof(CqCholSmem));
     cudaFuncSetAttribute(k_cq_chol_ekf, cudaFuncAttributeMaxDynamicSharedMemorySize, (int)sizeof(CqCholSmem));
-    cudaFuncSetAttribute(k_cq_trsm<5, 0>, cudaFuncAttributeMaxDynamicSharedMemorySize, (int)CQ_TRSM_SMEM);
-    cudaFuncSetAttribute(k_cq_trsm<10, 0>, cudaFuncAttributeMaxDynamicSharedMemorySize, (int)CQ_TRSM_SMEM);
-    cudaFuncSetAttribute(k_cq_trsm<10, 5>, cudaFuncAttributeMaxDynamicSharedMemorySize, (int)CQ_TRSM_SMEM);
-    cudaFuncSetAttribute(k_cq_trsm<10, 10>, cudaFuncAttributeMaxDynamicSharedMemorySize, (int)CQ_TRSM_SMEM);
+    cudaFuncSetAttribute((CqTrsmKernel)k_cq_trsm<5, 0>, cudaFuncAttributeMaxDynamicSharedMemorySize, (int)CQ_TRSM_SMEM);
+    cudaFuncSetAttribute((CqTrsmStreamKernel)k_cq_trsm<5, 0>, cudaFuncAttributeMaxDynamicSharedMemorySize, (int)CQ_TRSM_SMEM);
+    cudaFuncSetAttribute((CqTrsmKernel)k_cq_trsm<10, 0>, cudaFuncAttributeMaxDynamicSharedMemorySize, (int)CQ_TRSM_SMEM);
+    cudaFuncSetAttribute((CqTrsmStreamKernel)k_cq_trsm<10, 0>, cudaFuncAttributeMaxDynamicSharedMemorySize, (int)CQ_TRSM_SMEM);
+    cudaFuncSetAttribute((CqTrsmKernel)k_cq_trsm<10, 5>, cudaFuncAttributeMaxDynamicSharedMemorySize, (int)CQ_TRSM_SMEM);
+    cudaFuncSetAttribute((CqTrsmStreamKernel)k_cq_trsm<10, 5>, cudaFuncAttributeMaxDynamicSharedMemorySize, (int)CQ_TRSM_SMEM);
+    cudaFuncSetAttribute((CqTrsmKernel)k_cq_trsm<10, 10>, cudaFuncAttributeMaxDynamicSharedMemorySize, (int)CQ_TRSM_SMEM);
+    cudaFuncSetAttribute((CqTrsmStreamKernel)k_cq_trsm<10, 10>, cudaFuncAttributeMaxDynamicSharedMemorySize, (int)CQ_TRSM_SMEM);
     cudaFuncSetAttribute(k_cq_solve_gram<5, 0>, cudaFuncAttributeMaxDynamicSharedMemorySize, CQ_SG_SMEM);
     cudaFuncSetAttribute(k_cq_solve_gram<10, 0>, cudaFuncAttributeMaxDynamicSharedMemorySize, CQ_SG_SMEM);
     cudaFuncSetAttribute(k_cq_solve_gram<10, 5>, cudaFuncAttributeMaxDynamicSharedMemorySize, CQ_SG_SMEM);
@@ -961,9 +1145,12 @@
   return true;
 }
 
-bool launch_chol_ekf_dmma(ovb_ctx *ctx, double *S, int ldS, int r, const double *res, double *w, double *invdiag, double **Lpk_out) {
+bool launch_chol_ekf_dmma(ovb_ctx *ctx, double *S, int ldS, int r, const double *res, double *w, double *invdiag, double **Lpk_out,
+                          unsigned long long *epoch_out) {
   if (Lpk_out)
     *Lpk_out = nullptr;
+  if (epoch_out)
+    *epoch_out = 0;
   if (r + 1 > CQ_MAXRB * 8 || r > CQ_MAXN || (ldS & 1))
     return false;
   cq_attrs(ctx);
@@ -972,13 +1159,17 @@
     const int ldW = CQ_MAXN + 8;
     Lpk = ctx->d_G + (size_t)3 * ldW * ldW;
   }
-  ovb_launch(ctx, k_cq_chol_ekf, dim3(1), dim3(CQ_CHOL_T), sizeof(CqCholSmem), S, ldS, r, res, w, invdiag, ctx->d_info, Lpk, (const double *)nullptr);
+  const unsigned long long epoch = (epoch_out != nullptr && Lpk != nullptr) ? ++ctx->pub_epoch : 0;
+  ovb_launch(ctx, k_cq_chol_ekf, dim3(1), dim3(CQ_CHOL_T), sizeof(CqCholSmem), S, ldS, r, res, w, invdiag, ctx->d_info, Lpk, (const double *)nullptr,
+             epoch ? ctx->d_pub : (unsigned long long *)nullptr, epoch);
   if (Lpk_out)
     *Lpk_out = Lpk;
+  if (epoch_out)
+    *epoch_out = epoch;
   return true;
 }
 
-bool launch_trsm_rows(ovb_ctx *ctx, double *A, int ldA, int m, int nt, const double *Lpk) {
+bool launch_trsm_rows(ovb_ctx *ctx, double *A, int ldA, int m, int nt, const double *Lpk, unsigned long long epoch) {
   if (nt > CQ_MAXN || (ldA & 1) || m < 1 || Lpk == nullptr)
     return false;
   cq_attrs(ctx);
@@ -986,7 +1177,7 @@
   int ctas = ngroups;
   if (ctas > ctx->sm_count)
     ctas = ctx->sm_count;
-  cq_launch_trsm(ctx, ctas, A, ldA, m, nt, Lpk);
+  cq_launch_trsm(ctx, ctas, A, ldA, m, nt, Lpk, epoch ? ctx->d_pub : nullptr, epoch);
   return true;
 }
 
@@ -1024,7 +1215,7 @@
     const int nb = (n - J < CQ_WB) ? n - J : CQ_WB;
     double *Lb = Lpk + (size_t)b * CQ_PK_DOUBLES;
     ovb_launch(ctx, k_cq_chol_ekf, dim3(1), dim3(CQ_CHOL_T), sizeof(CqCholSmem), S + (size_t)J * ld + J, ld, nb, (const double *)nullptr, (double *)nullptr,
-               (double *)nullptr, info, Lb, floor_dev);
+               (double *)nullptr, info, Lb, floor_dev, (unsigned long long *)nullptr, 0ull);
     const int mrem = n + extra - (J + nb);
     if (mrem > 0) {
       double *panel = S + (size_t)(J + nb) * ld + J;
@@ -1156,10 +1347,11 @@
     gram_smem = sizeof(double) * 16 * 1024;
   cq_launch_gram(ctx, nblk, nslab_pad, gram_smem, (const double *)A, ldA, m, nt, slab_rows, BW, nblk_side, ctx->d_Gpart, cs);
   ovb_launch(ctx, k_cq_reduce, dim3(CQ_RED_GX, nblk), dim3(CQ_RED_T), (size_t)0, (const double *)ctx->d_Gpart, npart, nblk, BW, nblk_side, nt, G, ldW, 1);
-  ovb_launch(ctx, k_cq_chol_gram, dim3(1), dim3(CQ_CHOL_T), sizeof(CqCholSmem), (const double *)G, ldW, nt, 1e-11, L1, 1);
-  cq_launch_solve_gram(ctx, nslab, (const double *)A, ldA, m, nt, (const double *)L1, slab_rows, BW, ctx->d_Gpart, ctx->d_Gpart + part_doubles);
+  const unsigned long long epoch = ++ctx->pub_epoch;
+  ovb_launch(ctx, k_cq_chol_gram, dim3(1), dim3(CQ_CHOL_T), sizeof(CqCholSmem), (const double *)G, ldW, nt, 1e-11, L1, 1, ctx->d_pub, epoch);
+  cq_launch_solve_gram(ctx, nslab, (const double *)A, ldA, m, nt, (const double *)L1, slab_rows, BW, ctx->d_Gpart, ctx->d_Gpart + part_doubles, ctx->d_pub, epoch);
   ovb_launch(ctx, k_cq_reduce, dim3(CQ_RED_GX, nblk), dim3(CQ_RED_T), (size_t)0, (const double *)ctx->d_Gpart, nslab, nblk, BW, nblk_side, nt, G, ldW, 1);
-  ovb_launch(ctx, k_cq_chol_gram, dim3(1), dim3(CQ_CHOL_T), sizeof(CqCholSmem), (const double *)G, ldW, nt, 1e-13, L2, 1);
+  ovb_launch(ctx, k_cq_chol_gram, dim3(1), dim3(CQ_CHOL_T), sizeof(CqCholSmem), (const double *)G, ldW, nt, 1e-13, L2, 1, (unsigned long long *)nullptr, 0ull);
   const int nT16 = (nt + 15) / 16;
   ovb_launch(ctx, k_cq_trmm, dim3(nT16, nT16), dim3(256), (size_t)0, (const double *)L2, (const double *)L1, nt, Rout, ldR);
   ctx->n_launch += 7;
diff --git a/open_vins_b200/csrc/k_ekf.cu b/open_vins_b200/csrc/k_ekf.cu
--- a/open_vins_b200/csrc/k_ekf.cu
+++ b/open_vins_b200/csrc/k_ekf.cu
@@ -405,7 +405,8 @@
   int use_smem = chol_bytes <= 200 * 1024;
   double *invdiag = ctx->d_w + ctx->cfg.max_state;
   double *Lpk = nullptr;
-  const bool dmma_chol = ctx->ekf_chol_dmma && launch_chol_ekf_dmma(ctx, ctx->d_S, ld, r, ctx->d_w, ctx->d_w, invdiag, &Lpk);
+  unsigned long long epoch = 0;
+  const bool dmma_chol = ctx->ekf_chol_dmma && launch_chol_ekf_dmma(ctx, ctx->d_S, ld, r, ctx->d_w, ctx->d_w, invdiag, &Lpk, gate_only ? nullptr : &epoch);
   const bool wide = !dmma_chol && ctx->ekf_chol_dmma && r < ld && launch_chol_solve_wide(ctx, ctx->d_S, ld, r, ctx->d_w, invdiag, ctx->d_M, ld, N, gate_only);
   if (wide) {
     if (gate_only)
@@ -419,7 +420,7 @@
   if (gate_only)
     return;
   const double *Yd = ctx->d_Y;
-  if (dmma_chol && Lpk != nullptr && launch_trsm_rows(ctx, ctx->d_M, ld, N, r, Lpk)) {
+  if (dmma_chol && Lpk != nullptr && launch_trsm_rows(ctx, ctx->d_M, ld, N, r, Lpk, epoch)) {
     Yd = ctx->d_M;
   } else {
     size_t trsm_small = sizeof(double) * ((size_t)TR_ROWS * r + r);
diff --git a/open_vins_b200/csrc/ovb_api.cu b/open_vins_b200/csrc/ovb_api.cu
--- a/open_vins_b200/csrc/ovb_api.cu
+++ b/open_vins_b200/csrc/ovb_api.cu
@@ -161,6 +161,8 @@
   CK(cudaMalloc(&ctx->d_S, sizeof(double) * (size_t)(ms + 1) * ms));
   CK(cudaMalloc(&ctx->d_Y, sizeof(double) * (size_t)ms * ms));
   CK(cudaMalloc(&ctx->d_w, sizeof(double) * (size_t)ms * 4));
+  CK(cudaMalloc(&ctx->d_pub, sizeof(unsigned long long)));
+  CK(cudaMemset(ctx->d_pub, 0, sizeof(unsigned long long)));
   ctx->scratch_per_cta = (size_t)(2 * OVB_BIG_MAX_MEAS + 1) * (2 * OVB_BIG_MAX_MEAS + 1);
   ctx->scratch_ctas = 2 * ctx->sm_count;
   CK(cudaMalloc(&ctx->d_scratch, sizeof(double) * ctx->scratch_per_cta * ctx->scratch_ctas));
@@ -186,7 +188,7 @@
     cudaStreamSynchronize(ctx->stream);
   void *dev[] = {ctx->P[0],   ctx->P[1], ctx->d_arena, ctx->d_cc, ctx->d_feat_order, ctx->d_info, ctx->d_chi2_table, ctx->d_Hs, ctx->d_W[0],
                  ctx->d_W[1], ctx->d_R,  ctx->d_R2,    ctx->d_M,  ctx->d_S,          ctx->d_Y,    ctx->d_w,          ctx->d_scratch,
-                 ctx->d_long, ctx->d_dump, ctx->P_snap, ctx->d_flush, ctx->d_Gpart, ctx->d_G, ctx->d_cqw, ctx->d_grp, ctx->d_grp_acc, ctx->d_init, ctx->d_imu};
+                 ctx->d_long, ctx->d_dump, ctx->P_snap, ctx->d_flush, ctx->d_Gpart, ctx->d_G, ctx->d_cqw, ctx->d_grp, ctx->d_grp_acc, ctx->d_init, ctx->d_imu, ctx->d_pub};
   for (void *p : dev)
     if (p)
       cudaFree(p);
diff --git a/open_vins_b200/csrc/ovb_internal.cuh b/open_vins_b200/csrc/ovb_internal.cuh
--- a/open_vins_b200/csrc/ovb_internal.cuh
+++ b/open_vins_b200/csrc/ovb_internal.cuh
@@ -184,6 +184,8 @@
   size_t Gpart_cap, G_cap;
   double *d_cqw;
   size_t cqw_cap;
+  unsigned long long *d_pub;
+  unsigned long long pub_epoch;
   size_t last_h2d_bytes, last_d2h_bytes;
   DevInitSys *d_init, *h_init;
   int64_t init_counters[4];
@@ -214,8 +216,9 @@
 void launch_tsqr(ovb_ctx *ctx, double *A, int m, int n, int ldA, double *Rout, int ldR);
 int launch_compress_gram(ovb_ctx *ctx, const double *A, int m, int n, int ldA, double *Rout, int ldR);
 int launch_compress_cholqr2(ovb_ctx *ctx, double *A, int m, int n, int ldA, double *Rout, int ldR);
-bool launch_chol_ekf_dmma(ovb_ctx *ctx, double *S, int ldS, int r, const double *res, double *w, double *invdiag, double **Lpk_out);
-bool launch_trsm_rows(ovb_ctx *ctx, double *A, int ldA, int m, int nt, const double *Lpk);
+bool launch_chol_ekf_dmma(ovb_ctx *ctx, double *S, int ldS, int r, const double *res, double *w, double *invdiag, double **Lpk_out,
+                          unsigned long long *epoch_out);
+bool launch_trsm_rows(ovb_ctx *ctx, double *A, int ldA, int m, int nt, const double *Lpk, unsigned long long epoch);
 bool launch_chol_solve_wide(ovb_ctx *ctx, double *S, int ldS, int r, double *w, double *invdiag, double *M, int ldM, int N, bool gate_only);
 void launch_reorder_R(ovb_ctx *ctx, const double *Rin, int n_all, int ldRin, double *Rout, int ldRout);
 void launch_ekf_update(ovb_ctx *ctx, const double *H, int ldHm, int r, int n, bool gate_only, double sigma2, const double *Rdiag_dev,
```

New measurement: 2573, median of 6. 10.5% higher.
